# fgvieira/ngsF-HMM

Hardware: AMD Instinct MI355X
Metric: site-ind updates/sec (EM iterations x individuals x sites / s), 1M sites x 1k ind (higher is better)
Workload: dtype f64

## Files before the change

### include/nghmm_debug.h

```cpp
#ifndef NGHMM_DEBUG_H
#define NGHMM_DEBUG_H

#include "nghmm.h"

#ifdef __cplusplus
extern "C" {
#endif

int nghmm_set_switch(nghmm_t* h, const char* name, long value);

int nghmm_fast_layout(nghmm_t* h, uint32_t* waves_per_individual, uint64_t* sites_per_lane);

int nghmm_get_emissions(nghmm_t* h, double* e_prob);

int nghmm_kernel_ms(nghmm_t* h, int slot, double* ms, uint32_t* launches);

typedef struct {
  uint32_t mode;
  uint64_t ind_rounds;
} nghmm_mode_count;
int nghmm_debug_mode_counts(nghmm_t* h, nghmm_mode_count* out, uint32_t cap, uint32_t* n, int reset);
int nghmm_debug_estmaf_counts(nghmm_t* h, uint64_t out[5], int reset);

#ifdef __cplusplus
}
#endif
#endif
```

### ngsf-hmm_amd/csrc/capi_internal.hpp

```cpp
#pragma once
#include <hip/hip_runtime.h>

#include <atomic>
#include <cmath>
#include <cstdarg>
#include <cstdio>
#include <cstdlib>
#include <chrono>
#include <cstring>
#include <new>
#include <functional>
#include <condition_variable>
#include <map>
#include <mutex>
#include <string>
#include <thread>
#include <vector>

#include "../../include/nghmm.h"
#include "../../include/nghmm_debug.h"
#include "bfgs_batch.hpp"
#include "capi_owners.hpp"
#include "kernels.hpp"
#include "kernels_fast.hpp"
#include "kernels_summary.hpp"

using namespace nghmm;

namespace capi {

extern thread_local std::string g_last_error;

#define HIP_TRY(expr)                                                              \
  do {                                                                             \
    hipError_t e__ = (expr);                                                       \
    if (e__ != hipSuccess) {                                                       \
      set_error("%s failed: %s (%s:%d)", #expr, hipGetErrorString(e__), __FILE__,  \
                __LINE__);                                                         \
      return NGHMM_ERR_HIP;                                                        \
    }                                                                              \
  } while (0)

enum Slot { SLOT_EMISSION = 0, SLOT_FORWARD = 1, SLOT_BACKWARD = 2, SLOT_LKL = 3, SLOT_ESTMAF = 4,
            SLOT_VITERBI = 5, SLOT_LKL_FIRST = 6, SLOT_BFGS = 7, NSLOTS = 8 };

}

using namespace capi;

struct ChainCtx;
struct nghmm_handle {
  ~nghmm_handle();
  uint64_t I = 0, S = 0;
  int device = 0, mode = NGHMM_MODE_EXACT;
  Stream stream;
  Event ev0, ev1, ev_sync;
  Stream aux_stream;
  Stream g_xstream;
  Event aux_ev0, aux_ev1, aux_go, aux_done;
  static constexpr uint32_t kAuxPieces = 16;
  Event aux_piece_ev[kAuxPieces];
  Event aux_estep_ev[3];
  DevBuf<double> d_aux_params;
  PinBuf<int> h_flags_pin;
  PinBuf<double> h_lkl_pin;
  hipEvent_t param_snapshot_ev = nullptr;
  bool blocking_sync = false;
  bool loaded = false;
  bool warmed = false;

  DevBuf<double> d_gl, d_pos;
  DevBuf<double> d_freq, d_eprob, d_fw, d_marg, d_indF, d_alpha, d_ind_lkl;
  DevBuf<int> d_flags;

  DevScratch<uint32_t> d_pt_ind;
  DevScratch<double> d_pt_F, d_pt_A, d_pt_lkl;

  DevBuf<uint8_t> d_bp, d_path_sites, d_path;
  DevBuf<double> d_vit;
  DevBuf<double> d_tmp;
  DevScratch<double> d_geno;
  DevScratch<char> d_text;
  bool tmp_is_posteriors = false;
  bool path_decoded = false;
  DevScratch<uint8_t> d_tseg, d_trec;
  DevScratch<uint8_t> d_samp;
  DevScratch<uint8_t> d_info;
  DevScratch<uint8_t> d_summ;
  DevBuf<double> d_freq_new, d_hap;

  uint64_t I_tot = 0, ind_begin = 0, site_begin = 0, S_own = 0;
  DevBuf<double> d_gl_shard;

  bool packed = false;
  DevBuf<uint32_t> d_codes;
  DevBuf<uint32_t> d_codes_shard;
  DevBuf<double> d_cls_log;
  double h_cls_proto[12] = {0};
  DevBuf<unsigned long long> d_uniform;
  uint64_t lkl_redone = 0;
  struct LklAsync {
    Event ev0, ev1, ev_done;
    DevScratch<double> d_lkl;
    PinScratch<double> h_lkl;
    DevBuf<int> d_flags;
    PinBuf<int> h_flags;
    std::vector<uint32_t> ind;
    std::vector<double> F, A;
    uint64_t lo = 0, hi = 0;
    bool pending = false;
  } lane[2];
  struct BgSpan {
    Event ev0, ev1;
    int slot = 0;
  };
  DevBuf<int> d_flags_bg;
  bool flags_bg_clear = false;
  std::vector<BgSpan> bg_spans;
  size_t bg_used = 0;
  nghmm_handle* parent = nullptr;
  std::atomic<int> n_replicas{0};
  int g_n = 0, g_rank = 0;
  DevBuf<double> g_send, g_recv, g_freq_own, g_freq_all;
  struct ChainCtx* chain = nullptr;
  DevBuf<double> c_send, c_recv;
  bool loading = false;
  std::map<uint64_t, uint64_t> load_cover;
  DevScratch<double> d_stage;
  DevScratch<int8_t> d_stage8;

  FastState fast;
  BfgsBatch batch;
  bool marg_valid = false;

  std::vector<double> h_indF, h_alpha;
  double ms[NSLOTS] = {0, 0, 0, 0, 0, 0, 0, 0};
  uint32_t launches[NSLOTS] = {0, 0, 0, 0, 0, 0, 0, 0};
};

namespace capi {

hipError_t sync_stream(nghmm_t* h);
int use_device(nghmm_t* h);
void tic(nghmm_t* h);
int toc(nghmm_t* h, int slot, bool accumulate);
int clear_flags(nghmm_t* h);
int check_flags(nghmm_t* h, const int* d_flags = nullptr);
int ensure_points(nghmm_t* h, size_t n);
GlView own_gl(const nghmm_t* h);
int ensure_tmp(nghmm_t* h);
int ensure_marg(nghmm_t* h);
int viterbi_scratch(nghmm_t* h, uint64_t* chunk, double** state = nullptr);
int fast_estep_impl(nghmm_t* h, double* ind_lkl, bool have_walk);
int redo_nonfinite(nghmm_t* h, uint32_t n_pts, const uint32_t* ind, const double* F,
                   const double* alpha, double* lkl);
int lkl_batch_impl(nghmm_t* h, uint32_t n_pts, const uint32_t* ind, const double* F,
                   const double* alpha, double* lkl, bool accumulate, bool* emit_estep = nullptr);
int lane_setup(nghmm_t* h, int k, size_t n);
int lkl_submit(nghmm_t* h, int k);
int lkl_wait(nghmm_t* h, int k);
int emission_impl(nghmm_t* h);
int bg_begin(nghmm_t* h);
int bg_open(nghmm_t* h, int slot, hipStream_t st = nullptr);
int bg_close(nghmm_t* h, hipStream_t st = nullptr);
int bg_finish(nghmm_t* h);
int ensure_emissions(nghmm_t* h);

int estmaf_and_refresh(nghmm_t* h, bool shard, const double* d_marg_blocks, uint64_t S_own,
                       uint64_t I_tot, uint64_t I_blk, double* d_freq_out);
void chain_release(nghmm_t* h);
int tracts_to_host(nghmm_t* h, int source, double threshold, uint64_t min_sites,
                   std::vector<nghmm_tract>& out);
int tracts_check_args(nghmm_t* h, int source, double threshold, const char* who);
int summary_check_source(nghmm_t* h, int what, double threshold, const char* who);
int summary_check_regions(uint64_t S, uint64_t I, uint64_t n_regions, const uint64_t* begin,
                          const uint64_t* end, const void* regions, const void* sites,
                          const char* who);
struct SummaryRegion {
  uint64_t begin, end;
  bool first;
};
int summary_to_host(nghmm_t* h, int what, double thr, const std::vector<SummaryRegion>& regs,
                    const uint8_t* prev_state, nghmm_region_stat* regions, nghmm_site_stat* sites);
int summary_last_state(nghmm_t* h, uint8_t* out);

}
```

### ngsf-hmm_amd/csrc/capi_multi.hip

```cpp
#include "capi_internal.hpp"


int nghmm_shard_config(nghmm_t* h, uint64_t n_ind_total, uint64_t ind_begin, uint64_t site_begin,
                       uint64_t n_sites_own) {
  g_last_error.clear();
  if (h && h->fast.shard.world > 1) {
    set_error("nghmm_shard_config: the handle is a site shard (one layout at a time)");
    return NGHMM_ERR_ARG;
  }
  if (!h || n_ind_total < h->I || ind_begin + h->I > n_ind_total ||
      site_begin + n_sites_own > h->S || n_ind_total % h->I != 0) {
    set_error("nghmm_shard_config: inconsistent shard (equal individuals per rank required)");
    return NGHMM_ERR_ARG;
  }
  h->I_tot = n_ind_total;
  h->ind_begin = ind_begin;
  h->site_begin = site_begin;
  h->S_own = n_sites_own;
  return NGHMM_OK;
}

uint64_t nghmm_site_shard_bytes(nghmm_t* h) {
  return h ? (uint64_t)(h->I * 30 + 64) * sizeof(double) : 0;
}
// ... 95 lines not shown
  if ((rc = use_device(h))) return rc;
  const size_t n = (size_t)h->S_own * h->I_tot * 3;
  if ((rc = h->d_gl_shard.alloc(n))) return rc;
  HIP_TRY(hipMemcpyAsync(h->d_gl_shard, gl_site_shard, n * sizeof(double), hipMemcpyHostToDevice,
                         h->stream));
  if (h->mode == NGHMM_MODE_FAST) fast_exp(h->stream, h->d_gl_shard, h->d_gl_shard, n);
  HIP_TRY(sync_stream(h));
  return NGHMM_OK;
}

int nghmm_get_geno_codes_dev(nghmm_t* h, uint64_t site_lo, uint64_t site_hi, uint8_t* d_out) {
  g_last_error.clear();
  if (!h || !h->packed || !h->loaded || !d_out || site_lo > site_hi || site_hi > h->S)
    return NGHMM_ERR_ARG;
  int rc;
  if ((rc = use_device(h))) return rc;
  launch_codes_to_bytes(h->stream, h->d_codes, site_lo * h->I, (site_hi - site_lo) * h->I, d_out);
  HIP_TRY(hipGetLastError());
  HIP_TRY(sync_stream(h));
  return NGHMM_OK;
}

int nghmm_load_geno_site_shard_dev(nghmm_t* h, const uint8_t* d_codes_bytes) {
  g_last_error.clear();
  if (!h || !h->packed || !d_codes_bytes) return NGHMM_ERR_ARG;
  int rc;
  if ((rc = use_device(h))) return rc;
  const size_t n = (size_t)h->S_own * h->I_tot;
  if ((rc = h->d_codes_shard.alloc(n / 16 + 2))) return rc;
  HIP_TRY(hipDeviceSynchronize());
  launch_bytes_to_codes(h->stream, d_codes_bytes, n, h->d_codes_shard);
  HIP_TRY(hipGetLastError());
  HIP_TRY(sync_stream(h));
  return NGHMM_OK;
}

int nghmm_load_gl_site_shard_dev(nghmm_t* h, const double* d_gl_site_shard) {
  g_last_error.clear();
  if (!h || !d_gl_site_shard) return NGHMM_ERR_ARG;
  if (h->packed) {
    set_error("packed handle: use nghmm_load_geno_site_shard_dev");
    return NGHMM_ERR_ARG;
  }
  int rc;
  if ((rc = use_device(h))) return rc;
  const size_t n = (size_t)h->S_own * h->I_tot * 3;
  if ((rc = h->d_gl_shard.alloc(n))) return rc;
  HIP_TRY(hipDeviceSynchronize());
  HIP_TRY(hipMemcpyAsync(h->d_gl_shard, d_gl_site_shard, n * sizeof(double),
                         hipMemcpyDeviceToDevice, h->stream));
  if (h->mode == NGHMM_MODE_FAST) fast_exp(h->stream, h->d_gl_shard, h->d_gl_shard, n);
  HIP_TRY(sync_stream(h));
  return NGHMM_OK;
}

int nghmm_pack_posteriors_dev(nghmm_t* h, uint64_t site_lo, uint64_t site_hi, double* d_out) {
  g_last_error.clear();
  if (!h || !d_out || site_lo > site_hi || site_hi > h->S) return NGHMM_ERR_ARG;
  int rc;
  if ((rc = use_device(h))) return rc;
  if (h->mode == NGHMM_MODE_FAST && site_lo == 0 && site_hi == h->S) {
    if (!fast_post_to_site_major(h->fast, h->stream, d_out)) return NGHMM_ERR_HIP;
    HIP_TRY(hipGetLastError());
    HIP_TRY(sync_stream(h));
    return NGHMM_OK;
  }
  if ((rc = ensure_marg(h))) return rc;
  launch_copy_f64(h->stream, h->d_marg + site_lo * h->I, d_out, (site_hi - site_lo) * h->I);
  HIP_TRY(hipGetLastError());
  HIP_TRY(sync_stream(h));
  return NGHMM_OK;
}

int nghmm_mstep_freq_sites_dev(nghmm_t* h, const double* d_marg_blocks, double* d_freq_out) {
  g_last_error.clear();
  if (!h || !d_marg_blocks || !d_freq_out || !(h->packed ? (void*)h->d_codes_shard.p : (void*)h->d_gl_shard.p))
    return NGHMM_ERR_ARG;
  int rc;
  if ((rc = use_device(h))) return rc;
  if (h->mode != NGHMM_MODE_FAST && h->I_tot != h->I) {
    set_error("exact-mode sharded est_maf is not available; use NGHMM_MODE_FAST");
    return NGHMM_ERR_ARG;
  }
  if ((rc = estmaf_and_refresh(h, true, d_marg_blocks, h->S_own, h->I_tot, h->I, d_freq_out)))
    return rc;
  HIP_TRY(sync_stream(h));
  return NGHMM_OK;
}

int nghmm_set_freq_dev(nghmm_t* h, const double* d_freq_all) {
  g_last_error.clear();
  if (!h || !d_freq_all) return NGHMM_ERR_ARG;
  int rc;
  if ((rc = use_device(h))) return rc;
  HIP_TRY(hipMemcpyAsync(h->d_freq, d_freq_all, h->S * sizeof(double), hipMemcpyDeviceToDevice,
                         h->stream));
  return emission_impl(h);
}



namespace {

struct GroupHook {
  nghmm_t** hs;
  int n, r;
  int rc;
};

void group_after_estep(void* user) {
  GroupHook* g = static_cast<GroupHook*>(user);
  nghmm_t* h = g->hs[g->r];
  g->rc = nghmm_pack_posteriors_dev(h, 0, h->S, h->g_send);
  if (g->rc != NGHMM_OK) return;
  const size_t blk = (size_t)h->S_own * h->I;
  for (int q = 0; q < g->n; ++q) {
    if (hipMemcpyAsync(g->hs[q]->g_recv + (size_t)g->r * blk, h->g_send + (size_t)q * blk,
                       blk * sizeof(double), hipMemcpyDeviceToDevice, h->g_xstream) != hipSuccess) {
      g->rc = NGHMM_ERR_HIP;
      return;
    }
  }
}

int for_each_rank(int n, const std::function<int(int)>& fn) {
  std::vector<int> rcs(n, NGHMM_OK);
  std::vector<std::string> msgs(n);
  if (n == 1) {
    rcs[0] = fn(0);
  } else {
    std::vector<std::thread> th;
    for (int r = 0; r < n; ++r)
      th.emplace_back([&, r] {
        rcs[r] = fn(r);
        if (rcs[r] != NGHMM_OK) msgs[r] = g_last_error;
      });
    for (auto& t : th) t.join();
  }
  for (int r = 0; r < n; ++r)
    if (rcs[r] != NGHMM_OK) {
      if (!msgs[r].empty()) g_last_error = msgs[r];
      return rcs[r];
    }
  return NGHMM_OK;
}

int group_freq_phases(nghmm_t** hs, int n) {
  const uint64_t S_own = hs[0]->S / n;
  int rc = for_each_rank(n, [&](int r) -> int {
    nghmm_t* h = hs[r];
    int rr = nghmm_mstep_freq_sites_dev(h, h->g_recv, h->g_freq_own);
    if (rr != NGHMM_OK) return rr;
    for (int q = 0; q < n; ++q)
      if (hipMemcpyAsync(hs[q]->g_freq_all + (size_t)r * S_own, h->g_freq_own, S_own * sizeof(double),
                         hipMemcpyDeviceToDevice, h->g_xstream) != hipSuccess)
        return NGHMM_ERR_HIP;
    return hipStreamSynchronize(h->g_xstream) == hipSuccess ? NGHMM_OK : NGHMM_ERR_HIP;
  });
  if (rc != NGHMM_OK) return rc;
  return for_each_rank(n, [&](int r) -> int { return nghmm_set_freq_dev(hs[r], hs[r]->g_freq_all); });
}

}

int nghmm_group_setup(nghmm_t** hs, int n) {
  g_last_error.clear();
  if (!hs || n < 1) return NGHMM_ERR_ARG;
  for (int r = 0; r < n; ++r)
    if (hs[r]) hs[r]->batch.set_max_threads(n > 1 ? 1 : 64);
  nghmm_t* h0 = hs[0];
  for (int r = 0; r < n; ++r) {
    nghmm_t* h = hs[r];
    if (!h || !h->loaded || (n > 1 && (h->parent || h->n_replicas.load() > 0)) ||
        h->fast.shard.world > 1 || h->I != h0->I ||
        h->S != h0->S || h->mode != h0->mode ||
        h->packed != h0->packed) {
      set_error("nghmm_group_setup: the handles must be loaded and agree in size, mode and packing");
      return NGHMM_ERR_ARG;
    }
// ... 476 lines not shown
```

### ngsf-hmm_amd/csrc/kernels_fast.hip

```cpp
#include <hip/hip_runtime.h>

#include "fast_dev.hpp"

namespace nghmm {

namespace {


__global__ void __launch_bounds__(256)
k_fast_geno_interleave(const uint32_t* __restrict__ codes, uint64_t cell0, uint64_t I, uint64_t S,
                       uint64_t T, uint32_t C, uint32_t* __restrict__ geno_il) {
  const uint64_t TB = T >> 4;
  const uint64_t n = I * C * TB * 64;
  for (uint64_t k = (uint64_t)blockIdx.x * blockDim.x + threadIdx.x; k < n;
       k += (uint64_t)gridDim.x * blockDim.x) {
    const uint64_t lane = k & 63, r = k >> 6;
    const uint64_t tb = r % TB, wv = r / TB;
    const uint64_t c = wv % C, i = wv / C;
    const uint64_t s0 = (c * 64 + lane) * T + tb * 16;
    uint32_t w = 0;
#pragma unroll
    for (int j = 0; j < 16; ++j) {
      const uint64_t s = s0 + j;
      if (s < S) w |= gl_code(codes, cell0 + s * I + i) << (2 * j);
// ... 90 lines not shown
      }
      tq[tx][ll] = q;
    }
  }
  __syncthreads();
  {
    const int tx = threadIdx.x & 63, ty = threadIdx.x >> 6;
    for (int ii = ty; ii < 32; ii += 4) {
      const uint64_t i = i0 + ii;
      if (i < I) glq_il[((i * C + c) * T + t) * 64 + tx] = tq[ii][tx];
    }
  }
}

__global__ void __launch_bounds__(256)
k_fast_gl_scale(const GlView gl_log, uint64_t I, uint64_t S, uint64_t T, uint32_t C,
                double* __restrict__ scale_c) {
  __shared__ double part[8][33];
  const uint64_t n_it = (I + 31) / 32;
  const uint64_t c = blockIdx.x / n_it;
  const uint64_t i0 = (blockIdx.x % n_it) * 32;
  const int tx = threadIdx.x & 31, ty = threadIdx.x >> 5;
  const uint64_t i = i0 + tx;
  double acc = 0;
  if (i < I) {
    for (uint64_t j = c * 64 + ty; j < c * 64 + 64; j += 8) {
      for (uint64_t t = 0; t < T; ++t) {
        const uint64_t s = j * T + t;
        if (s >= S) break;
        double g0, g1, g2;
        gl_fetch(gl_log, s * I + i, g0, g1, g2);
        acc += fmax(g0, fmax(g1, g2));
      }
    }
  }
  part[ty][tx] = acc;
  __syncthreads();
  if (ty == 0 && i < I) {
    double sum = 0;
    for (int k = 0; k < 8; ++k) sum += part[k][tx];
    scale_c[i * C + c] = sum;
  }
}

__global__ void __launch_bounds__(256)
k_fast_export_e(LklArrays arr, bool packed, const double* __restrict__ gl_lin, uint64_t I,
                uint64_t S, uint64_t T, uint32_t C, double* __restrict__ out) {
  const uint64_t n = I * S;
  for (uint64_t k = (uint64_t)blockIdx.x * blockDim.x + threadIdx.x; k < n;
       k += (uint64_t)gridDim.x * blockDim.x) {
    const uint64_t i = k / S, s = k % S;
    const uint64_t j = s / T, t = s % T;
    const uint64_t c = j >> 6, lane = j & 63;
    const uint64_t wv = i * C + c;
    const double maf = arr.freq_il[(c * T + t) * 64 + lane], om = 1 - maf;
    const double bb = om * maf;
    const double h00 = om * om, h02 = maf * maf;
    double e0, e1;
    if (packed) {
      const uint32_t w = arr.geno_il[(wv * (T >> 4) + (t >> 4)) * 64 + lane];
      const uint32_t code = (w >> ((uint32_t)(t & 15) * 2)) & 3u;
      const double u = arr.u_lin;
      const double u0 = fma(u, h00, fma(u, 2 * bb, u * h02));
      const double u1 = fma(u, h00 + bb, u * (h02 + bb));
      e0 = code == 0 ? h00 : code == 1 ? 2 * bb : code == 2 ? h02 : u0;
      e1 = code == 0 ? h00 + bb : code == 1 ? 0.0 : code == 2 ? h02 + bb : u1;
    } else {
      const double* g = gl_lin + (s * I + i) * 3;
      e0 = fma(g[0], h00, fma(g[1], 2 * bb, g[2] * h02));
      e1 = fma(g[0], h00 + bb, g[2] * (h02 + bb));
    }
    out[k * 2] = log(e0);
    out[k * 2 + 1] = log(e1);
  }
}

struct SwitchName {
  const char* name;
  int Switches::*field;
};
const SwitchName kSwitches[] = {
    {"bg_parts", &Switches::bg_parts}, {"estmaf_interp", &Switches::estmaf_interp},
    {"estmaf_no_rows", &Switches::estmaf_no_rows}, {"estmaf_no_called", &Switches::estmaf_no_called},
    {"fast_c", &Switches::fast_c}, {"exact_serial", &Switches::exact_serial},
    {"dbg_abort_round", &Switches::dbg_abort_round}, {"no_dev_bfgs", &Switches::no_dev_bfgs},
    {"no_bg_stream", &Switches::no_bg_stream}, {"spans", &Switches::spans},
    {"viterbi_chunk", &Switches::viterbi_chunk}};

}

Switches Switches::from_env() {
  Switches sw;
  for (const auto& k : kSwitches) {
    std::string env = "NGHMM_";
    for (const char* c = k.name; *c; ++c) env += (char)std::toupper((unsigned char)*c);
    if (const char* v = std::getenv(env.c_str())) {
      char* end = nullptr;
      const long n = std::strtol(v, &end, 10);
      sw.*(k.field) = (end != v) ? (int)n : 1;
    }
  }
  return sw;
}

bool Switches::set(const char* name, long value) {
  for (const auto& k : kSwitches)
    if (std::strcmp(k.name, name) == 0) {
      this->*(k.field) = (int)value;
      return true;
    }
  return false;
}

static bool fast_alloc_run_state(FastState& fs) {
  const size_t cells = (size_t)fs.I * fs.Spad;
  const size_t slack = 8 * 64;
  if (!dalloc(&fs.e_il, cells + slack)) return false;
  if (hipMemset(fs.e_il + cells, 0, slack * sizeof(double)) != hipSuccess) return false;
  if (!dalloc(&fs.base_c, (size_t)fs.I * fs.C)) return false;
  if (!dalloc(&fs.freq_il, (size_t)fs.Spad + slack)) return false;
  if (hipMemset(fs.freq_il + fs.Spad, 0, slack * sizeof(double)) != hipSuccess) return false;
  const size_t post_cells = (size_t)fs.C * fs.T * post_tile_doubles(fs.I);
  if (!dalloc(&fs.post, post_cells)) return false;
  if (hipMemset(fs.post, 0, post_cells * sizeof(double)) != hipSuccess) return false;
  if (!dalloc(&fs.ckpt, cells / CK * 4 + 4 * 64)) return false;
  if (!dalloc(&fs.lane_ops, (size_t)fs.I * fs.J * 5)) return false;
  if (!dalloc(&fs.bound, (size_t)fs.I * fs.J * 4)) return false;
  fs.e_stale = true;
  return true;
}

bool fast_create(FastState& fs, uint64_t I, uint64_t S, bool packed) {
  fs.I = I;
  fs.S = S;
  fs.packed = packed;
  fs.owns_data = true;
  uint64_t C = (49152 + I - 1) / I;
  if (fs.sw.fast_c >= 1) C = (uint64_t)fs.sw.fast_c;
  if (C > 256) C = 256;
  while (C > 1 && (S + 64 * C - 1) / (64 * C) < (C > 64 ? 32u : 16u)) --C;
  if (C < 1) C = 1;
  if (fs.sw.fast_c < 1) {
    const uint64_t c64 = S / (64 * 64);
    if (c64 >= 1 && c64 < C && I * c64 >= 24576) C = c64;
  }
  if (fs.sw.fast_c < 1) {
    const uint64_t q = packed ? 16 : 8;
    auto padded = [&](uint64_t c) { return 64 * c * ((((S + 64 * c - 1) / (64 * c)) + q - 1) / q * q); };
    uint64_t best = C;
    for (uint64_t c = C; c >= 1 && 4 * c >= 3 * C; --c)
      if (padded(c) < padded(best)) best = c;
    C = best;
  }
  fs.C = (uint32_t)C;
  fs.J = 64 * C;
  fs.T = (S + fs.J - 1) / fs.J;
  fs.T = (fs.T + 7) & ~7ull;
  if (packed) fs.T = (fs.T + 15) & ~15ull;
  fs.Spad = fs.J * fs.T;
  const size_t cells = (size_t)I * fs.Spad;
  const size_t slack = 8 * 64;
  if (!dalloc(&fs.pos_il, (size_t)fs.Spad + slack)) return false;
  if (hipMemset(fs.pos_il + fs.Spad, 0, slack * sizeof(double)) != hipSuccess) return false;
  if (!dalloc(&fs.chunk_scale, (size_t)2 * fs.J)) return false;
  if (!dalloc(&fs.gl_scale_c, (size_t)I * C)) return false;
  if (packed) {
    const size_t words = cells / 16 + slack;
    if (!dalloc(&fs.geno_il, words)) return false;
    if (hipMemset(fs.geno_il, 0, words * sizeof(uint32_t)) != hipSuccess) return false;
    if (!dalloc(&fs.cls_lin, (size_t)12)) return false;
  } else {
    if (!dalloc(&fs.glq_il, (cells + slack) * 2)) return false;
    if (hipMemset(fs.glq_il + cells * 2, 0, slack * 2 * sizeof(double)) != hipSuccess) return false;
    if (!dalloc(&fs.gl_lin, (size_t)I * S * 3)) return false;
  }
  return fast_alloc_run_state(fs);
}

bool fast_create_replica(FastState& fs, const FastState& parent) {
  fs = FastState();
  fs.sw = parent.sw;
  fs.I = parent.I;
  fs.S = parent.S;
  fs.T = parent.T;
  fs.C = parent.C;
  fs.J = parent.J;
  fs.Spad = parent.Spad;
  fs.packed = parent.packed;
  fs.owns_data = false;
  fs.gl_log = parent.gl_log;
  fs.d_pos = parent.d_pos;
  fs.geno_il = parent.geno_il;
  fs.cls_lin = parent.cls_lin;
  fs.u_lin = parent.u_lin;
  fs.called_table = parent.called_table;
  fs.gl_lin = parent.gl_lin;
  fs.pos_il = parent.pos_il;
  fs.chunk_scale = parent.chunk_scale;
  fs.glq_il = parent.glq_il;
  fs.gl_scale_c = parent.gl_scale_c;
  fs.dmax_finite = parent.dmax_finite;
  fs.alpha_small_min = parent.alpha_small_min;
  return fast_alloc_run_state(fs);
}

void fast_destroy(FastState& fs) {
  dbfgs_destroy(fs);
  void* run[] = {fs.e_il, fs.base_c, fs.freq_il, fs.post, fs.ckpt, fs.lane_ops, fs.bound, fs.lanes[0].part,
                 fs.lanes[0].grp_dev, fs.lanes[1].part, fs.lanes[1].grp_dev, fs.redo, fs.est_status,
                 fs.est_state, fs.est_counts, fs.shard.edges};
  for (void* p : run)
    if (p) (void)hipFree(p);
  if (fs.owns_data) {
    void* data[] = {fs.pos_il, fs.chunk_scale, fs.glq_il, fs.gl_scale_c, fs.gl_lin, fs.geno_il, fs.cls_lin};
    for (void* p : data)
      if (p) (void)hipFree(p);
  }
  fs = FastState();
}

void fast_exp(hipStream_t st, const double* d_in, double* d_out, uint64_t n) {
  if (n) hipLaunchKernelGGL(k_fast_exp, dim3(16384), dim3(256), 0, st, d_in, d_out, n);
}

GlView fast_gl_lin(const FastState& fs) {
  return fs.packed ? gl_packed(fs.gl_log.codes, fs.cls_lin, fs.gl_log.cell0) : gl_dense(fs.gl_lin);
}

bool fast_load(FastState& fs, hipStream_t st, const GlView& gl_log, const double* d_pos) {
  dbfgs_invalidate(fs);
  fs.gl_log = gl_log;
  fs.d_pos = d_pos;
  fs.e_stale = true;
  if (fs.packed) {
    if (gl_log.dense) return false;
    fast_exp(st, gl_log.table, fs.cls_lin, 12);
    double t[12];
    if (hipMemcpyAsync(t, fs.cls_lin, sizeof t, hipMemcpyDeviceToHost, st) != hipSuccess) return false;
    if (hipStreamSynchronize(st) != hipSuccess) return false;
    fs.u_lin = t[9];
    fs.called_table = t[0] == 1 && t[1] == 0 && t[2] == 0 && t[3] == 0 && t[4] == 1 && t[5] == 0 &&
                      t[6] == 0 && t[7] == 0 && t[8] == 1 && t[9] > 0 && t[10] == t[9] && t[11] == t[9];
    hipLaunchKernelGGL(k_fast_geno_interleave, dim3(8192), dim3(256), 0, st, gl_log.codes,
                       gl_log.cell0, fs.I, fs.S, fs.T, fs.C, fs.geno_il);
  } else {
    if (!gl_log.dense) return false;
    const double* lg = gl_log.dense + gl_log.cell0 * 3;
    fast_exp(st, lg, fs.gl_lin, fs.I * fs.S * 3);
    const uint64_t n_it = (fs.I + 31) / 32;
    hipLaunchKernelGGL(k_fast_gl_interleave, dim3((unsigned)((uint64_t)fs.C * fs.T * n_it)),
                       dim3(256), 0, st, lg, fs.I, fs.S, fs.T, fs.C,
                       reinterpret_cast<double2*>(fs.glq_il));
  }
  hipLaunchKernelGGL(k_fast_gl_scale, dim3((unsigned)((uint64_t)fs.C * ((fs.I + 31) / 32))), dim3(256),
                     0, st, gl_log, fs.I, fs.S, fs.T, fs.C, fs.gl_scale_c);
  hipLaunchKernelGGL(k_fast_pos_interleave, dim3(1024), dim3(256), 0, st, d_pos, fs.S, fs.T, fs.C,
                     fs.pos_il);
  hipLaunchKernelGGL(k_fast_chunk_scale, dim3(fs.C), dim3(64), 0, st, fs.pos_il, fs.T,
                     reinterpret_cast<double2*>(fs.chunk_scale));
  unsigned long long* d_m = reinterpret_cast<unsigned long long*>(fs.bound);
  if (hipMemsetAsync(d_m, 0, sizeof(unsigned long long), st) != hipSuccess) return false;
  hipLaunchKernelGGL(k_fast_max_finite, dim3(256), dim3(256), 0, st, d_pos, fs.S, d_m);
  unsigned long long bits = 0;
  if (hipMemcpyAsync(&bits, d_m, sizeof bits, hipMemcpyDeviceToHost, st) != hipSuccess) return false;
  if (hipStreamSynchronize(st) != hipSuccess) return false;
  std::memcpy(&fs.dmax_finite, &bits, sizeof bits);
  {
    std::vector<double> cs((size_t)2 * fs.J);
    if (hipMemcpy(cs.data(), fs.chunk_scale, cs.size() * sizeof(double), hipMemcpyDeviceToHost) != hipSuccess)
      return false;
    double sum = 0, starts = 0;
    for (size_t k = 0; k < fs.J; ++k) {
      sum += cs[2 * k];
      starts += cs[2 * k + 1];
    }
    const double n_finite = (double)fs.S - starts;
    fs.alpha_small_min = (n_finite > 0 && sum > 0) ? 1e-6 / (sum / n_finite) : HUGE_VAL;
  }
  return hipGetLastError() == hipSuccess;
}

bool fast_refresh_freq_table(FastState& fs, hipStream_t st, const double* d_freq, int* d_flags) {
  hipLaunchKernelGGL(k_fast_freq_interleave, dim3(1024), dim3(256), 0, st, d_freq, fs.S, fs.T, fs.C,
                     fs.freq_il, d_flags);
  fs.e_stale = true;
  return hipGetLastError() == hipSuccess;
}


bool fast_viterbi(FastState& fs, hipStream_t st, const double* d_freq, const double* d_indF,
                  const double* d_alpha, uint8_t* d_bp, uint8_t* d_path_sites, int* d_flags,
                  double* d_scratch, uint64_t chunk_sites) {
  double* eprob_log = nullptr;
  if (!dalloc(&eprob_log, (size_t)fs.I * fs.S * 2)) return false;
  launch_emission_exact(st, fs.gl_log, d_freq, eprob_log, fs.S, fs.I, d_flags);
  launch_viterbi_exact(st, eprob_log, fs.d_pos, fs.S, fs.I, d_indF, d_alpha, d_bp, d_path_sites,
                       d_scratch, chunk_sites, fs.sw.exact_serial != 0);
  const bool ok = hipGetLastError() == hipSuccess && hipStreamSynchronize(st) == hipSuccess;
  (void)hipFree(eprob_log);
  return ok;
}

bool fast_viterbi_forward(FastState& fs, hipStream_t st, const double* d_freq, const double* d_indF,
                          const double* d_alpha, uint8_t* d_bp, int* d_flags, double* d_scratch,
                          uint64_t chunk_sites, bool chain_start) {
  double* eprob_log = nullptr;
  if (!dalloc(&eprob_log, (size_t)fs.I * fs.S * 2)) return false;
  launch_emission_exact(st, fs.gl_log, d_freq, eprob_log, fs.S, fs.I, d_flags);
  launch_viterbi_fwd_exact(st, eprob_log, fs.d_pos, fs.S, fs.I, d_indF, d_alpha, d_bp, d_scratch,
                           chunk_sites, chain_start, fs.sw.exact_serial != 0);
  const bool ok = hipGetLastError() == hipSuccess && hipStreamSynchronize(st) == hipSuccess;
  (void)hipFree(eprob_log);
  return ok;
// ... 10 lines not shown
```

### ngsf-hmm_amd/csrc/kernels_fast.hpp

```cpp
#pragma once

#include <hip/hip_runtime.h>

#include <cstdint>
#include <map>
#include <vector>

#include "glview.hpp"

namespace nghmm {

struct Switches {
  int bg_parts = 2;
  int estmaf_interp = 1;
  int estmaf_no_rows = 0;
  int estmaf_no_called = 0;
  int fast_c = 0;
  int exact_serial = 0;
  int dbg_abort_round = 0;
  int no_dev_bfgs = 0;
  int no_bg_stream = 0;
  int viterbi_chunk = 0;
  int spans = 0;
  static Switches from_env();
  bool set(const char* name, long value);
};

struct SiteShard {
  uint32_t rank = 0, world = 1;
  double* send = nullptr;
  double* recv = nullptr;
  uint64_t cap = 0;
  int (*allgather)(void* user, uint64_t n_bytes) = nullptr;
  void* user = nullptr;
  double* edges = nullptr;
  bool edges_from_round = false;
  uint64_t n_gathers = 0;
};

struct FastState {
  Switches sw;
  SiteShard shard;
  uint64_t I = 0, S = 0;
  uint64_t T = 0;
  uint32_t C = 0;
  uint64_t J = 0;
  uint64_t Spad = 0;
  GlView gl_log;
  const double* d_pos = nullptr;
  bool packed = false;
  bool owns_data = true;
  uint32_t* geno_il = nullptr;
  double* cls_lin = nullptr;
  double u_lin = 0;
  bool called_table = false;
  double* gl_lin = nullptr;
  double* e_il = nullptr;
  double* base_c = nullptr;
  double* pos_il = nullptr;
  double* chunk_scale = nullptr;
  double* glq_il = nullptr;
  double* gl_scale_c = nullptr;
  double* freq_il = nullptr;
  bool e_stale = true;
  double* post = nullptr;
  double* ckpt = nullptr;
  double* lane_ops = nullptr;
  double* bound = nullptr;
  struct ModeRange { uint32_t mode, begin, count; };
  struct LklLane {
    double* part = nullptr;
    size_t part_cap = 0;
    void* grp_dev = nullptr;
    size_t grp_cap = 0;
    std::vector<unsigned char> grp_host;
    uint32_t n_groups = 0;
    uint32_t n_pts = 0;
    std::vector<ModeRange> mode_ranges;
  };
  LklLane lanes[2];
  int cur_lane = 0;

  struct DevBfgs {
    static constexpr uint32_t kRing = 4;
    static constexpr uint32_t kTableWords = 4 + 2 * 129 + 12;
    uint64_t cap_I = 0;
    void* prob = nullptr;
    void* solver = nullptr;
    double* arrays = nullptr;
    void* groups = nullptr;
    uint32_t* last_mode = nullptr;
    uint32_t* worklists = nullptr;
    uint32_t* all = nullptr;
    uint32_t* counts = nullptr;
    double* lkl = nullptr;
    double* part = nullptr;
    double *d_F = nullptr, *d_A = nullptr;
    double *snap_F = nullptr, *snap_A = nullptr;
    uint32_t snap_set = 0;
    volatile uint32_t* h_table = nullptr;
    double *h_F = nullptr, *h_A = nullptr;
    unsigned long long stats_host[6] = {0, 0, 0, 0, 0, 0};
    uint32_t seq_base = 0;
    uint32_t mstep_no = 0;
    bool clean = true;
    bool preplanned = false;
    bool pre_F_fixed = false, pre_alpha_fixed = false;
    double* h_epi_lkl = nullptr;
    volatile uint32_t* h_epi = nullptr;
    uint32_t epi_seq = 0;
  } dev;

  double dmax_finite = 0;
  double alpha_small_min = 0;
  uint8_t* redo = nullptr;
  size_t redo_cap = 0;
  uint8_t* est_status = nullptr;
  double* est_state = nullptr;
  std::map<uint32_t, uint64_t> mode_ind_rounds;
  uint32_t* est_counts = nullptr;
};

enum EstCount {
  EST_CNT_CHECK_FAILED = 0,
  EST_CNT_RESUMED = 1,
  EST_CNT_RESUMED_AGAIN = 2,
  EST_CNT_LOGSPACE = 3,
  EST_CNT_EXACT_TAIL = 4,
  EST_COUNTS = 5
};

bool fast_create(FastState& fs, uint64_t I, uint64_t S, bool packed = false);
bool fast_create_replica(FastState& fs, const FastState& parent);
void fast_destroy(FastState& fs);
bool fast_load(FastState& fs, hipStream_t st, const GlView& gl_log, const double* d_pos);
bool fast_refresh_freq_table(FastState& fs, hipStream_t st, const double* d_freq, int* d_flags);
bool fast_refresh_emissions(FastState& fs, hipStream_t st, const double* d_freq, int* d_flags);
bool fast_lkl_prepare(FastState& fs, hipStream_t st, uint32_t n_pts, const uint32_t* h_ind,
                      const double* h_F, const double* h_A, bool force_general = false);
bool fast_lkl_launch(FastState& fs, hipStream_t st, double* d_lkl, int* d_flags,
                     bool emit_estep = false);
bool fast_lkl_covers_everyone(const FastState& fs);
bool dbfgs_available(const FastState& fs);
bool dbfgs_reserve(FastState& fs);
void dbfgs_destroy(FastState& fs);
void dbfgs_invalidate(FastState& fs);
constexpr uint32_t kEpiFlags = 8;
bool dbfgs_epilogue(FastState& fs, hipStream_t st, int* d_flags, uint32_t n_flags, const double* d_lkl);
bool dbfgs_wait_epilogue(FastState& fs, hipStream_t st, int* flags_out, uint32_t n_flags, bool yield);
bool dbfgs_begin(FastState& fs, hipStream_t st, double* d_indF, double* d_alpha, bool F_fixed,
                 bool alpha_fixed);
const double* dbfgs_start_F(const FastState& fs);
const double* dbfgs_start_A(const FastState& fs);
bool dbfgs_advance(FastState& fs, hipStream_t st, uint32_t round, uint32_t n_in);
bool dbfgs_wait_plan(FastState& fs, hipStream_t st, uint32_t round, uint32_t* n_active,
                     std::vector<FastState::ModeRange>* ranges, bool yield = false);
bool dbfgs_launch_round(FastState& fs, hipStream_t st, uint32_t round, uint32_t n_active,
                        const std::vector<FastState::ModeRange>& ranges, bool emit_estep);
void dbfgs_end(FastState& fs, uint32_t last_round);
bool dbfgs_preplan(FastState& fs, hipStream_t st, bool F_fixed, bool alpha_fixed);
bool fast_lkl_launch_planned(FastState& fs, hipStream_t st, const void* d_groups_by_ind,
                             const std::vector<FastState::ModeRange>& ranges, uint32_t n_active,
                             const uint32_t* d_worklists, const uint32_t* d_all, double* part,
                             double* d_lkl, bool emit_estep);
bool fast_estep(FastState& fs, hipStream_t st, const double* d_indF, const double* d_alpha,
                double* d_ind_lkl, int* d_flags, bool have_forward_walk);
bool fast_forward_ops(FastState& fs, hipStream_t st, const double* d_indF, const double* d_alpha);
bool fast_post_to_site_major(FastState& fs, hipStream_t st, double* d_marg);
void fast_exp(hipStream_t st, const double* d_in, double* d_out, uint64_t n);
GlView fast_gl_lin(const FastState& fs);
bool fast_estmaf_splittable(const FastState& fs, uint64_t I_tot, bool tile_major);
bool fast_estmaf_in_place(const FastState& fs, uint64_t I_tot);
bool fast_estmaf_reserve(FastState& fs, uint64_t S_own);
bool fast_estmaf_called(const FastState& fs, const GlView& gl);
bool fast_estmaf(FastState& fs, hipStream_t st, const GlView& d_gl_lin_sites,
                 const double* d_marg_blocks, uint64_t S_own, uint64_t I_tot, uint64_t I_blk,
                 double* d_freq_out, bool tile_major = false, uint32_t part = 0,
                 uint32_t n_parts = 1);
bool fast_viterbi(FastState& fs, hipStream_t st, const double* d_freq, const double* d_indF,
                  const double* d_alpha, uint8_t* d_bp, uint8_t* d_path_sites, int* d_flags,
                  double* d_scratch, uint64_t chunk_sites);
bool fast_viterbi_forward(FastState& fs, hipStream_t st, const double* d_freq, const double* d_indF,
                          const double* d_alpha, uint8_t* d_bp, int* d_flags, double* d_scratch,
                          uint64_t chunk_sites, bool chain_start);
bool fast_export_emissions(FastState& fs, hipStream_t st, double* d_out);

}
```

### ngsf-hmm_amd/csrc/kernels_fast_estmaf.hip

```cpp
#include "fast_dev.hpp"

#include <mutex>

namespace capi {
void set_error(const char* fmt, ...);
}

namespace nghmm {

namespace {



__device__ double2 estmaf_term_logspace(const double* g, double freq, double F) {
  double h[3];
  h[0] = (1 - freq) * (1 - freq) + (1 - freq) * freq * F;
  h[1] = 2 * (1 - freq) * freq - 2 * (1 - freq) * freq * F;
  h[2] = freq * freq + (1 - freq) * freq * F;
  double pp[3];
  for (int k = 0; k < 3; ++k) {
    double l = log(h[k]);
    if (l == -__builtin_huge_val()) l = -kINF;
    h[k] = l;
  }
  if (F == 1) h[1] = -kINF;
  double M = g[0] + h[0];
  for (int k = 0; k < 3; ++k) {
    pp[k] = g[k] + h[k];
    M = (pp[k] >= M) ? pp[k] : M;
  }
  double sum = 0;
  for (int k = 0; k < 3; ++k) sum += exp(pp[k] - M);
  const double norm = log(sum) + M;
  for (int k = 0; k < 3; ++k) pp[k] = exp(pp[k] - norm);
  return double2{pp[1] + pp[2] * (2 - F), 2 * pp[1] + (pp[0] + pp[2]) * (2 - F)};
}

template <int CTRL>
__device__ __forceinline__ double dpp_move(double v) {
  const uint64_t b = ngh_bits(v);
  const int lo = __builtin_amdgcn_mov_dpp((int)(uint32_t)b, CTRL, 0xf, 0xf, true);
  const int hi = __builtin_amdgcn_mov_dpp((int)(uint32_t)(b >> 32), CTRL, 0xf, 0xf, true);
  return ngh_from_bits(((uint64_t)(uint32_t)hi << 32) | (uint32_t)lo);
}

__device__ __forceinline__ double lane_value(double v, int lane) {
  const uint64_t b = ngh_bits(v);
  const uint32_t lo = __builtin_amdgcn_readlane((int)(uint32_t)b, lane);
  const uint32_t hi = __builtin_amdgcn_readlane((int)(uint32_t)(b >> 32), lane);
  return ngh_from_bits(((uint64_t)hi << 32) | lo);
}

__device__ __forceinline__ double wave_sum_lastrow(double v) {
  v += dpp_move<0xB1>(v);
  v += dpp_move<0x4E>(v);
  v += dpp_move<0x141>(v);
  v += dpp_move<0x140>(v);
  {
    const uint64_t b = ngh_bits(v);
    const int lo = __builtin_amdgcn_update_dpp(0, (int)(uint32_t)b, 0x142, 0xa, 0xf, false);
    const int hi = __builtin_amdgcn_update_dpp(0, (int)(uint32_t)(b >> 32), 0x142, 0xa, 0xf, false);
    v += ngh_from_bits(((uint64_t)(uint32_t)hi << 32) | (uint32_t)lo);
  }
  {
    const uint64_t b = ngh_bits(v);
    const int lo = __builtin_amdgcn_update_dpp(0, (int)(uint32_t)b, 0x143, 0xc, 0xf, false);
    const int hi = __builtin_amdgcn_update_dpp(0, (int)(uint32_t)(b >> 32), 0x143, 0xc, 0xf, false);
    v += ngh_from_bits(((uint64_t)(uint32_t)hi << 32) | (uint32_t)lo);
  }
  return v;
}

__device__ __forceinline__ double wave_sum_uniform(double v) {
  v += dpp_move<0xB1>(v);
  v += dpp_move<0x4E>(v);
  v += dpp_move<0x141>(v);
  v += dpp_move<0x140>(v);
  return ((lane_value(v, 0) + lane_value(v, 16)) + lane_value(v, 32)) + lane_value(v, 48);
}

__device__ __forceinline__ double wave_sum_pair(double pn, double pd) {
  const uint64_t bn = ngh_bits(pn), bd = ngh_bits(pd);
  const auto lo = __builtin_amdgcn_permlane32_swap((unsigned)bn, (unsigned)bd, false, false);
  const auto hi = __builtin_amdgcn_permlane32_swap((unsigned)(bn >> 32), (unsigned)(bd >> 32),
                                                   false, false);
  double v = ngh_from_bits(((uint64_t)hi[0] << 32) | lo[0]) +
             ngh_from_bits(((uint64_t)hi[1] << 32) | lo[1]);
  v += dpp_move<0xB1>(v);
  v += dpp_move<0x4E>(v);
  v += dpp_move<0x141>(v);
  v += dpp_move<0x140>(v);
  {
    const uint64_t b = ngh_bits(v);
    const int l = __builtin_amdgcn_update_dpp(0, (int)(uint32_t)b, 0x142, 0xa, 0xf, false);
    const int h = __builtin_amdgcn_update_dpp(0, (int)(uint32_t)(b >> 32), 0x142, 0xa, 0xf, false);
    v += ngh_from_bits(((uint64_t)(uint32_t)h << 32) | (uint32_t)l);
  }
  return v;
}

constexpr int EN = 12;
constexpr int EST_SCALARS = 8;
constexpr int EST_FIELDS = EST_SCALARS + 2 * EN;
enum : uint8_t { EST_DONE = 0, EST_INTERP = 1, EST_EXACT = 2 };
constexpr int EST_K0 = 2;
constexpr int EST_MIN_GAIN = 24;
constexpr double EST_DMAX = 0.85;
constexpr double EST_BACK = 0.1;
constexpr double EST_MULT = 32.0;
constexpr double EST_FIT = 0.72;
constexpr int EST_KMAX = 32;
constexpr double EST_TOL = 1e-11;
constexpr double EST_GUARD = 1e-9;
__constant__ double kChebC[EN] = {0.9914448613738104, 0.9238795325112867, 0.7933533402912352, 0.6087614290087207, 0.38268343236508984, 0.1305261922200517, -0.1305261922200516, -0.3826834323650895, -0.6087614290087207, -0.793353340291235, -0.9238795325112867, -0.9914448613738104};
__constant__ double kChebW[EN] = {0.13052619222005157, -0.3826834323650898, 0.6087614290087207, -0.7933533402912352, 0.9238795325112867, -0.9914448613738104, 0.9914448613738104, -0.9238795325112868, 0.7933533402912352, -0.6087614290087209, 0.3826834323650899, -0.130526192220052};

constexpr int ESTMAF_MAXW = 16;

__device__ __forceinline__ bool in_tile_rows(uint64_t site, uint64_t tile_T, uint64_t row0,
                                             uint64_t row1) {
  if (tile_T == 0) return true;
  const uint64_t j = site / tile_T, t = site - j * tile_T;
  const uint64_t row = (j >> 6) * tile_T + t;
  return row >= row0 && row < row1;
}
__host__ __device__ constexpr int estmaf_full_slots(int NI, int BLOCK) {
  return BLOCK == 64 ? (NI == 16 ? 12 : NI == 12 ? 8 : NI == 8 ? 4 : NI == 4 ? 2 : NI == 2 ? 1 : 0)
                     : (NI == 16 ? 8 : 0);
}

template <int NI, int BLOCK, bool TILE>
__device__ __forceinline__ void estmaf_site(
    const GlView& gl, const double* __restrict__ marg_blocks, uint64_t S_own, uint64_t I_tot,
    uint64_t I_blk, double* __restrict__ freq_out, uint8_t* __restrict__ redo,
    uint8_t* __restrict__ status, double* __restrict__ state, uint64_t state_stride, int fresh,
    int n_exact, int allow_build, uint64_t site, const double* __restrict__ tile_col,
    uint32_t* __restrict__ cnt, double (&xch)[2][ESTMAF_MAXW][2],
    double2 (&nodebuf)[(BLOCK == 64 && NI >= 8) ? EN : 1][(BLOCK == 64 && NI >= 8) ? 65 : 1],
    double2 (&xnode)[(BLOCK == 64 && NI >= 8) ? 1 : EN][(BLOCK == 64 && NI >= 8) ? 1 : BLOCK / 64],
    double2* park = nullptr) {
  constexpr int W = BLOCK / 64;
  constexpr bool PARK = (W == 1 && NI >= 8);
  const int lane = threadIdx.x & 63;
  const int wv = threadIdx.x >> 6;
  const uint32_t tix = threadIdx.x;
  constexpr uint64_t stride = BLOCK;
  const uint64_t cell_s = site * I_tot;

  double tF_lane_out;
  double sA[NI], sb[NI], sC[NI], u0[NI], nC[NI], fc[NI];
  {
    constexpr int NB = NI < 8 ? NI : (NI % 8 ? NI / 2 : 8);
    static_assert(NI % NB == 0, "whole batches");
    const bool one_block = (I_blk == I_tot);
    const uint32_t ib = (uint32_t)I_blk;
    double tF_acc = 0;
#pragma unroll
    for (int k0 = 0; k0 < NI; k0 += NB) {
      double r0[NB], r1[NB], r2[NB], rF[NB];
      uint64_t ic[NB];
#pragma unroll
      for (int j = 0; j < NB; ++j) {
        const uint64_t i = (uint64_t)tix + stride * (k0 + j);
        ic[j] = (k0 + j < estmaf_full_slots(NI, BLOCK) || i < I_tot) ? i : I_tot - 1;
        gl_fetch(gl, cell_s + ic[j], r0[j], r1[j], r2[j]);
      }
      if constexpr (TILE) {
#pragma unroll
        for (int j = 0; j < NB; ++j)
          rF[j] = tile_col[k0 + j < estmaf_full_slots(NI, BLOCK)
                               ? post_ind_off(tix) + (uint64_t)(k0 + j) * post_ind_off(stride)
                               : post_ind_off(ic[j])];
      } else if (one_block) {
#pragma unroll
        for (int j = 0; j < NB; ++j) rF[j] = marg_blocks[site * I_blk + ic[j]];
      } else {
#pragma unroll
        for (int j = 0; j < NB; ++j) {
          const uint32_t q = (uint32_t)ic[j] / ib;
          rF[j] = marg_blocks[((uint64_t)q * S_own + site) * I_blk + ((uint32_t)ic[j] - q * ib)];
        }
      }
#pragma unroll
      for (int j = 0; j < NB; ++j) {
        const int k = k0 + j;
        const bool valid = k < estmaf_full_slots(NI, BLOCK) || (uint64_t)tix + stride * k < I_tot;
        const double p0 = valid ? r0[j] : 1.0, p1 = valid ? r1[j] : 0.0;
        const double p2 = valid ? r2[j] : 0.0, F = valid ? rF[j] : 0.0;
        const double cc = p1 * fma(-2.0, F, 2.0);
        const double n2 = (2 - F) * p2;
        sA[k] = p0;
        sb[k] = fma(F, p0 + p2, cc);
        sC[k] = p2;
        u0[k] = fma(n2, F, cc);
        nC[k] = n2;
        fc[k] = F * cc;
        tF_acc += valid ? 2 - F : 0.0;
      }
      __builtin_amdgcn_sched_barrier(0);
    }
    tF_lane_out = tF_acc;
  }
  double tF_sum = wave_sum_uniform(tF_lane_out);
  if constexpr (W > 1) {
    if (lane == 0) xch[1][wv][0] = tF_sum;
    __syncthreads();
    tF_sum = xch[1][0][0];
#pragma unroll
    for (int w = 1; w < W; ++w) tF_sum += xch[1][w][0];
    __syncthreads();
  }

  int iters = 0;
  int buf = 0;
  double num = 0, den = 0;
  double pnum = 0.01, pden = 1.0;
  if (!fresh) {
    num = state[0 * state_stride + site];
    den = state[1 * state_stride + site];
    pnum = state[2 * state_stride + site];
    pden = state[3 * state_stride + site];
    iters = (int)state[4 * state_stride + site];
  }
  bool built = !allow_build;
  int n_before = n_exact;
  bool check = false, interp_ok = false;
  double mid = 0, half = 0, my_gn = 0, my_gd = 0, rprev = 0;
  auto lane_sums = [&](double r, double& pn, double& pd) {
    pn = 0;
    pd = 0;
    if constexpr (NI >= 4) {
#pragma unroll
      for (int k0 = 0; k0 + 4 <= NI; k0 += 4) {
        double sm[4];
#pragma unroll
        for (int j = 0; j < 4; ++j) sm[j] = fma(r, fma(r, sC[k0 + j], sb[k0 + j]), sA[k0 + j]);
        const double p01 = sm[0] * sm[1], p23 = sm[2] * sm[3];
        const double R = rcp_nr(p01 * p23);
        const double r01 = R * p23, r23 = R * p01;
        const double inv0 = r01 * sm[1], inv1 = r01 * sm[0];
        const double inv2 = r23 * sm[3], inv3 = r23 * sm[2];
        pn = fma(fma(nC[k0], r, u0[k0]), inv0, pn);
        pd = fma(fc[k0], inv0, pd);
        pn = fma(fma(nC[k0 + 1], r, u0[k0 + 1]), inv1, pn);
        pd = fma(fc[k0 + 1], inv1, pd);
        pn = fma(fma(nC[k0 + 2], r, u0[k0 + 2]), inv2, pn);
        pd = fma(fc[k0 + 2], inv2, pd);
        pn = fma(fma(nC[k0 + 3], r, u0[k0 + 3]), inv3, pn);
        pd = fma(fc[k0 + 3], inv3, pd);
      }
      if constexpr (NI % 4 == 2) {
        constexpr int k0 = NI - 2;
        const double s0 = fma(r, fma(r, sC[k0], sb[k0]), sA[k0]);
        const double s1 = fma(r, fma(r, sC[k0 + 1], sb[k0 + 1]), sA[k0 + 1]);
        const double R = rcp_nr(s0 * s1);
        const double inv0 = R * s1, inv1 = R * s0;
        pn = fma(fma(nC[k0], r, u0[k0]), inv0, pn);
        pd = fma(fc[k0], inv0, pd);
        pn = fma(fma(nC[k0 + 1], r, u0[k0 + 1]), inv1, pn);
        pd = fma(fc[k0 + 1], inv1, pd);
      }
    } else {
#pragma unroll
      for (int k = 0; k < NI; ++k) {
        const double inv = rcp_nr(fma(r, fma(r, sC[k], sb[k]), sA[k]));
        pn = fma(fma(nC[k], r, u0[k]), inv, pn);
        pd = fma(fc[k], inv, pd);
      }
    }
  };
  for (;;) {
    const double r = pnum * rcp_nr2(pden - pnum);
    double pn, pd;
    lane_sums(r, pn, pd);
    const double v = wave_sum_pair(pn, pd);
    double sn = lane_value(v, 31), sd = lane_value(v, 63);
    if constexpr (W > 1) {
      if (lane == 0) {
        xch[buf][wv][0] = sn;
        xch[buf][wv][1] = sd;
      }
      __syncthreads();
      sn = xch[buf][0][0];
      sd = xch[buf][0][1];
#pragma unroll
      for (int w = 1; w < W; ++w) {
        sn += xch[buf][w][0];
        sd += xch[buf][w][1];
      }
      buf ^= 1;
    }
    if (check) {
      const int nj = lane < EN ? lane : 0;
      const double t = (r - mid) / (r + mid) - half * kChebC[nj];
      const double q = (lane < EN) ? kChebW[nj] / t : 0.0;
      const double Sq = wave_sum_uniform(q);
      const double bn = wave_sum_uniform(q * my_gn) / Sq, bd = wave_sum_uniform(q * my_gd) / Sq;
      interp_ok = fabs(bn - sn) <= EST_TOL * fabs(sn) && fabs(bd - sd) <= EST_TOL * fabs(sd);
      check = false;
      if (!interp_ok && tix == 0) atomicAdd(cnt + EST_CNT_CHECK_FAILED, 1u);
    }
    num = fma(r, sn, num);
    den = fma(r, sd, den + tF_sum);
    const double lhs = fabs(fma(pnum, den, -(num * pden))), thr = kEPS * (den * pden);
    const bool again = (lhs > thr) && (iters++ < 100);
    rprev = r;
    pnum = num;
    pden = den;
    if (!again) break;
    if (interp_ok) {
      if (wv == 0) {
        if (lane < EN) {
          state[(EST_SCALARS + lane) * state_stride + site] = my_gn;
          state[(EST_SCALARS + EN + lane) * state_stride + site] = my_gd;
        }
        if (lane == 0) {
          state[0 * state_stride + site] = num;
          state[1 * state_stride + site] = den;
          state[2 * state_stride + site] = pnum;
          state[3 * state_stride + site] = pden;
          state[4 * state_stride + site] = (double)iters;
          state[5 * state_stride + site] = mid;
          state[6 * state_stride + site] = half;
          state[7 * state_stride + site] = tF_sum;
          status[site] = EST_INTERP;
        }
      }
      return;
    }
    if (!built && --n_before <= 0) {
      const double m_est = (double)iters * (sqrt(lhs / thr) - 1.0);
      const double rn = pnum * rcp_nr2(pden - pnum);
      const double step = fabs(rn - rprev);
      const double reach = (rn >= rprev) ? EST_DMAX * rn : EST_DMAX / (1 + EST_DMAX) * rn;
      const bool fits = (double)iters * step <= EST_FIT * reach;
      if (!fits && iters < EST_KMAX && m_est >= EST_MIN_GAIN) {
        n_before = 1;
      } else {
        built = true;
      }
      if (built && m_est >= EST_MIN_GAIN && 100 - iters >= EST_MIN_GAIN) {
        const double g = fmin(EST_DMAX, fmax(EST_MULT * step / rn, 1e-3));
        double lo, hi;
        if (rn >= rprev) {
          lo = rn * (1 - EST_BACK * g);
          hi = rn * (1 + g);
        } else {
          lo = rn / (1 + g);
          hi = rn * (1 + EST_BACK * g);
        }
        mid = sqrt(lo * hi);
        half = (hi - mid) / (hi + mid);
        if (half > 0 && lo > 0 && hi < 1e300) {
          if constexpr (PARK) {
            const double tnl = half * kChebC[lane < EN ? lane : 0];
            const double r_nodes = mid * (1 + tnl) * rcp_nr2(1 - tnl);
#pragma unroll 1
            for (int nd = 0; nd < EN; ++nd) {
              double pn, pd;
              lane_sums(lane_value(r_nodes, nd), pn, pd);
              nodebuf[nd][lane] = double2{pn, pd};
            }
            __syncthreads();
            const int j = lane & 15, q4 = lane >> 4;
            double an = 0, ad = 0;
            if (j < EN) {
#pragma unroll
              for (int l = 0; l < 16; ++l) {
                const double2 t2 = nodebuf[j][q4 * 16 + l];
                an += t2.x;
                ad += t2.y;
              }
            }
            an += __shfl_xor(an, 16);
            ad += __shfl_xor(ad, 16);
            an += __shfl_xor(an, 32);
            ad += __shfl_xor(ad, 32);
            my_gn = an;
            my_gd = ad;
            check = true;
          } else {
            const double tnl = half * kChebC[lane < EN ? lane : 0];
            const double r_nodes = mid * (1 + tnl) * rcp_nr2(1 - tnl);
            double an = 0, ad = 0;
            if constexpr (W > 1) {
#pragma unroll 1
              for (int nd = 0; nd < EN; ++nd) {
                double pn, pd;
                lane_sums(lane_value(r_nodes, nd), pn, pd);
                park[nd * BLOCK + (int)tix] = double2{pn, pd};
              }
              __syncthreads();
              for (int nd = wv; nd < EN; nd += W) {
                double sn = 0, sd = 0;
#pragma unroll
                for (int w = 0; w < W; ++w) {
                  const double2 t2 = park[nd * BLOCK + w * 64 + lane];
                  sn += t2.x;
                  sd += t2.y;
                }
                const double v = wave_sum_pair(sn, sd);
                const double tn = lane_value(v, 31), td = lane_value(v, 63);
                if (lane == 0) xnode[nd][0] = double2{tn, td};
              }
              __syncthreads();
              if (lane < EN) {
                an = xnode[lane][0].x;
                ad = xnode[lane][0].y;
              }
              __syncthreads();
            } else {
#pragma unroll 1
              for (int nd = 0; nd < EN; ++nd) {
                double pn, pd;
                lane_sums(lane_value(r_nodes, nd), pn, pd);
                const double v = wave_sum_pair(pn, pd);
                const double sn = lane_value(v, 31), sd = lane_value(v, 63);
                if (lane == nd) {
                  an = sn;
                  ad = sd;
                }
              }
            }
            my_gn = an;
            my_gd = ad;
            check = true;
          }
        }
      }
    }
  }
  if (tix == 0) {
    const double freq = num / den;
    const bool ok = freq >= 0 && freq < 1;
    freq_out[site] = freq;
    redo[site] = ok ? 0 : 1;
    status[site] = EST_DONE;
  }
}

__device__ __forceinline__ const double* estmaf_tile_col(const double* marg_blocks, uint64_t site,
                                                         uint64_t tile_T, uint64_t I_tot) {
  const uint64_t j = site / tile_T, t = site - j * tile_T;
  return marg_blocks + post_lane_off((j >> 6) * tile_T + t, j & 63, I_tot);
}

#define ESTMAF_SHARED(NI, BLOCK)                                                              \
  constexpr bool PARK_ = ((BLOCK) == 64 && (NI) >= 8);                                         \
  __shared__ double xch[2][ESTMAF_MAXW][2];                       \
  __shared__ double2 nodebuf[PARK_ ? EN : 1][PARK_ ? 65 : 1];                                  \
  __shared__ double2 xnode[PARK_ ? 1 : EN][PARK_ ? 1 : (BLOCK) / 64]

template <int NI, int BLOCK, bool TILE>
__global__ void __launch_bounds__(BLOCK) __attribute__((amdgpu_waves_per_eu(2)))
k_fast_estmaf(const GlView gl, const double* __restrict__ marg_blocks,
              uint64_t S_own, uint64_t I_tot, uint64_t I_blk, uint64_t tile_T,
              double* __restrict__ freq_out, uint8_t* __restrict__ redo,
              uint8_t* __restrict__ status, double* __restrict__ state, uint64_t state_stride,
              int n_exact, int allow_build, uint64_t blk0, uint32_t* __restrict__ cnt) {
  ESTMAF_SHARED(NI, BLOCK);
  uint64_t site;
  const double* tile_col = nullptr;
  if constexpr (TILE) {
    const uint64_t b = blockIdx.x + blk0, x = b & 7, k = b >> 3;
    const uint64_t q = ((k >> 3) << 6) + (x << 3) + (k & 7);
    const uint64_t tile_row = q >> 6, l = q & 63;
    const uint64_t c = tile_row / tile_T, t = tile_row - c * tile_T;
    site = (c * 64 + l) * tile_T + t;
    if (site >= S_own) return;
    tile_col = marg_blocks + post_lane_off(tile_row, l, I_tot);
  } else {
    site = blockIdx.x;
  }
  extern __shared__ double2 park_mem[];
  estmaf_site<NI, BLOCK, TILE>(gl, marg_blocks, S_own, I_tot, I_blk, freq_out, redo, status, state,
                               state_stride, 1, n_exact, allow_build, site, tile_col, cnt, xch, nodebuf,
                               xnode, park_mem);
}

template <int NI, int BLOCK, bool TILE>
__global__ void __launch_bounds__(BLOCK) __attribute__((amdgpu_waves_per_eu(2)))
k_fast_estmaf_resume(const GlView gl, const double* __restrict__ marg_blocks,
                     uint64_t S_own, uint64_t I_tot, uint64_t I_blk, uint64_t tile_T,
                     double* __restrict__ freq_out, uint8_t* __restrict__ redo,
                     uint8_t* __restrict__ status, double* __restrict__ state,
                     uint64_t state_stride, int n_exact, int allow_build, uint64_t row0,
                     uint64_t row1, uint32_t* __restrict__ cnt, int cnt_slot) {
  ESTMAF_SHARED(NI, BLOCK);
  extern __shared__ double2 park_mem[];
  const int lane = threadIdx.x & 63;
  for (uint64_t base = (uint64_t)blockIdx.x * 64; base < S_own; base += (uint64_t)gridDim.x * 64) {
    const uint64_t s = base + lane;
    const bool need = s < S_own && in_tile_rows(s, TILE ? tile_T : 0, row0, row1) &&
                      status[s] == EST_EXACT;
    uint64_t mask = __ballot(need);
    if (mask && threadIdx.x == 0) atomicAdd(cnt + cnt_slot, (uint32_t)__popcll(mask));
    if constexpr (BLOCK > 64) __syncthreads();
    while (mask) {
      const uint64_t site = base + (uint64_t)__builtin_ctzll(mask);
      mask &= mask - 1;
      const double* tile_col = TILE ? estmaf_tile_col(marg_blocks, site, tile_T, I_tot) : nullptr;
      estmaf_site<NI, BLOCK, TILE>(gl, marg_blocks, S_own, I_tot, I_blk, freq_out, redo, status,
                                   state, state_stride, 0, n_exact, allow_build, site, tile_col, cnt,
                                   xch, nodebuf, xnode, park_mem);
      if constexpr (BLOCK > 64) __syncthreads();
    }
  }
}

__device__ __forceinline__ double row_sum(double v) {
  v = __dadd_rn(v, dpp_move<0xB1>(v));
  v = __dadd_rn(v, dpp_move<0x4E>(v));
  v = __dadd_rn(v, dpp_move<0x141>(v));
  v = __dadd_rn(v, dpp_move<0x140>(v));
  return v;
}

template <int NI, bool TILE>
__device__ __forceinline__ void estmaf_rows_sites(
    const GlView& gl, const double* __restrict__ marg_blocks, uint64_t S_own, uint64_t I_tot,
    uint64_t I_blk, double* __restrict__ freq_out, uint8_t* __restrict__ redo,
    uint8_t* __restrict__ status, double* __restrict__ state, uint64_t state_stride, int fresh,
    int n_exact, int allow_build, uint64_t site, const double* __restrict__ tile_col, bool done,
    uint32_t* __restrict__ cnt) {
  static_assert(EN <= 16, "a row's lanes hold the interval's node sums");
  const int lane = threadIdx.x, j = lane & 15;
  const uint64_t cell_s = site * I_tot;

  double sA[NI], sb[NI], sC[NI], u0[NI], nC[NI], fc[NI];
  double tF_acc = 0;
  {
    const bool one_block = (I_blk == I_tot);
    const uint32_t ib = (uint32_t)I_blk;
    double r0[NI], r1[NI], r2[NI], rF[NI];
    uint64_t ic[NI];
#pragma unroll
    for (int k = 0; k < NI; ++k) {
      const uint64_t i = (uint64_t)j + 16 * k;
      ic[k] = i < I_tot ? i : I_tot - 1;
      gl_fetch(gl, cell_s + ic[k], r0[k], r1[k], r2[k]);
    }
#pragma unroll
    for (int k = 0; k < NI; ++k) {
      if constexpr (TILE) {
        rF[k] = tile_col[post_ind_off(ic[k])];
      } else if (one_block) {
        rF[k] = marg_blocks[site * I_blk + ic[k]];
      } else {
        const uint32_t q = (uint32_t)ic[k] / ib;
        rF[k] = marg_blocks[((uint64_t)q * S_own + site) * I_blk + ((uint32_t)ic[k] - q * ib)];
      }
    }
#pragma unroll
    for (int k = 0; k < NI; ++k) {
      const bool valid = (uint64_t)j + 16 * k < I_tot;
      const double p0 = valid ? r0[k] : 1.0, p1 = valid ? r1[k] : 0.0;
      const double p2 = valid ? r2[k] : 0.0, F = valid ? rF[k] : 0.0;
      const double cc = p1 * fma(-2.0, F, 2.0);
      const double n2 = (2 - F) * p2;
      sA[k] = p0;
      sb[k] = fma(F, p0 + p2, cc);
      sC[k] = p2;
      u0[k] = fma(n2, F, cc);
      nC[k] = n2;
      fc[k] = F * cc;
      tF_acc += valid ? 2 - F : 0.0;
    }
  }
  const double tF_sum = row_sum(tF_acc);

  int iters = 0;
  double num = 0, den = 0;
  double pnum = 0.01, pden = 1.0;
  if (!fresh && !done) {
    num = state[0 * state_stride + site];
    den = state[1 * state_stride + site];
    pnum = state[2 * state_stride + site];
    pden = state[3 * state_stride + site];
    iters = (int)state[4 * state_stride + site];
  }
  bool built = !allow_build;
  int n_before = n_exact;
  bool check = false;
  double mid = 1, half = 0.5, my_gn = 0, my_gd = 0, rprev = 0;
  auto lane_sums = [&](double r, double& pn, double& pd) {
    pn = 0;
    pd = 0;
    if constexpr (NI >= 4) {
#pragma unroll
      for (int k0 = 0; k0 < NI; k0 += 4) {
        double sm[4];
#pragma unroll
        for (int k = 0; k < 4; ++k) sm[k] = fma(r, fma(r, sC[k0 + k], sb[k0 + k]), sA[k0 + k]);
        const double p01 = sm[0] * sm[1], p23 = sm[2] * sm[3];
        const double R = rcp_nr(p01 * p23);
        const double r01 = R * p23, r23 = R * p01;
        const double inv0 = r01 * sm[1], inv1 = r01 * sm[0];
        const double inv2 = r23 * sm[3], inv3 = r23 * sm[2];
        pn = fma(fma(nC[k0], r, u0[k0]), inv0, pn);
        pd = fma(fc[k0], inv0, pd);
        pn = fma(fma(nC[k0 + 1], r, u0[k0 + 1]), inv1, pn);
        pd = fma(fc[k0 + 1], inv1, pd);
        pn = fma(fma(nC[k0 + 2], r, u0[k0 + 2]), inv2, pn);
        pd = fma(fc[k0 + 2], inv2, pd);
        pn = fma(fma(nC[k0 + 3], r, u0[k0 + 3]), inv3, pn);
        pd = fma(fc[k0 + 3], inv3, pd);
      }
    } else {
#pragma unroll
      for (int k = 0; k < NI; ++k) {
        const double inv = rcp_nr(fma(r, fma(r, sC[k], sb[k]), sA[k]));
        pn = fma(fma(nC[k], r, u0[k]), inv, pn);
        pd = fma(fc[k], inv, pd);
      }
    }
  };
  for (;;) {
    const double r = pnum * rcp_nr2(pden - pnum);
    double pn, pd;
    lane_sums(r, pn, pd);
    const double sn = row_sum(pn), sd = row_sum(pd);
    bool interp_ok = false;
    if (__builtin_amdgcn_ballot_w64(check && !done) != 0) {
      const int nj = j < EN ? j : 0;
      const double t = (r - mid) / (r + mid) - half * kChebC[nj];
      const double q = (j < EN) ? kChebW[nj] / t : 0.0;
      const double Sq = row_sum(q);
      const double bn = row_sum(q * my_gn) / Sq, bd = row_sum(q * my_gd) / Sq;
      if (check && !done) {
        interp_ok = fabs(bn - sn) <= EST_TOL * fabs(sn) && fabs(bd - sd) <= EST_TOL * fabs(sd);
        if (!interp_ok && j == 0) atomicAdd(cnt + EST_CNT_CHECK_FAILED, 1u);
      }
      check = false;
    }
    bool want_build = false;
    if (!done) {
      num = fma(r, sn, num);
      den = fma(r, sd, den + tF_sum);
      const double lhs = fabs(fma(pnum, den, -(num * pden))), thr = kEPS * (den * pden);
      const bool again = (lhs > thr) && (iters++ < 100);
      rprev = r;
      pnum = num;
      pden = den;
      if (!again) {
        if (j == 0) {
          const double freq = num / den;
          const bool ok = freq >= 0 && freq < 1;
          freq_out[site] = freq;
          redo[site] = ok ? 0 : 1;
          status[site] = EST_DONE;
        }
        done = true;
      } else if (interp_ok) {
        if (j < EN) {
          state[(EST_SCALARS + j) * state_stride + site] = my_gn;
          state[(EST_SCALARS + EN + j) * state_stride + site] = my_gd;
        }
        if (j == 0) {
          state[0 * state_stride + site] = num;
          state[1 * state_stride + site] = den;
          state[2 * state_stride + site] = pnum;
          state[3 * state_stride + site] = pden;
          state[4 * state_stride + site] = (double)iters;
          state[5 * state_stride + site] = mid;
          state[6 * state_stride + site] = half;
          state[7 * state_stride + site] = tF_sum;
          status[site] = EST_INTERP;
        }
        done = true;
      } else if (!built && --n_before <= 0) {
        const double m_est = (double)iters * (sqrt(lhs / thr) - 1.0);
        const double rn = pnum * rcp_nr2(pden - pnum);
        const double step = fabs(rn - rprev);
        const double reach = (rn >= rprev) ? EST_DMAX * rn : EST_DMAX / (1 + EST_DMAX) * rn;
        const bool fits = (double)iters * step <= EST_FIT * reach;
        if (!fits && iters < EST_KMAX && m_est >= EST_MIN_GAIN) {
          n_before = 1;
        } else {
          built = true;
        }
        if (built && m_est >= EST_MIN_GAIN && 100 - iters >= EST_MIN_GAIN) {
          const double g = fmin(EST_DMAX, fmax(EST_MULT * step / rn, 1e-3));
          double lo, hi;
          if (rn >= rprev) {
            lo = rn * (1 - EST_BACK * g);
            hi = rn * (1 + g);
          } else {
            lo = rn / (1 + g);
            hi = rn * (1 + EST_BACK * g);
          }
          const double a = sqrt(lo * hi), h = (hi - a) / (hi + a);
          if (h > 0 && lo > 0 && hi < 1e300) {
            mid = a;
            half = h;
            want_build = true;
          }
        }
      }
    }
    if (__builtin_amdgcn_ballot_w64(want_build) != 0) {
#pragma unroll 1
      for (int nd = 0; nd < EN; ++nd) {
        const double tn = half * kChebC[nd];
        double qn, qd;
        lane_sums(mid * (1 + tn) * rcp_nr2(1 - tn), qn, qd);
        const double gn = row_sum(qn), gd = row_sum(qd);
        if (want_build && j == nd) {
          my_gn = gn;
          my_gd = gd;
        }
      }
      if (want_build) check = true;
    }
    if (__builtin_amdgcn_ballot_w64(!done) == 0) break;
  }
}

template <int NI, bool TILE>
__global__ void __launch_bounds__(64)
k_fast_estmaf_rows(const GlView gl, const double* __restrict__ marg_blocks, uint64_t S_own,
                   uint64_t I_tot, uint64_t I_blk, uint64_t tile_T, double* __restrict__ freq_out,
                   uint8_t* __restrict__ redo, uint8_t* __restrict__ status,
                   double* __restrict__ state, uint64_t state_stride, int n_exact,
                   int allow_build, uint32_t* __restrict__ cnt) {
  const int lane = threadIdx.x, row = lane >> 4;
  uint64_t site;
  const double* tile_col = nullptr;
  if constexpr (TILE) {
    const uint64_t b = blockIdx.x, x = b & 7, k = b >> 3;
    const uint64_t q = ((k >> 1) << 6) + (x << 3) + ((k & 1) << 2) + row;
    const uint64_t tile_row = q >> 6, l = q & 63;
    const uint64_t c = tile_row / tile_T, t = tile_row - c * tile_T;
    site = (c * 64 + l) * tile_T + t;
    tile_col = marg_blocks + post_lane_off(tile_row, l, I_tot);
  } else {
    site = (uint64_t)blockIdx.x * 4 + row;
  }
  bool done = site >= S_own;
  if (done) {
    site = 0;
    if constexpr (TILE) tile_col = marg_blocks;
  }
  if (__builtin_amdgcn_ballot_w64(!done) == 0) return;
  estmaf_rows_sites<NI, TILE>(gl, marg_blocks, S_own, I_tot, I_blk, freq_out, redo, status, state,
                              state_stride, 1, n_exact, allow_build, site, tile_col, done, cnt);
}

template <int NI, bool TILE>
__global__ void __launch_bounds__(64)
k_fast_estmaf_rows_resume(const GlView gl, const double* __restrict__ marg_blocks, uint64_t S_own,
                          uint64_t I_tot, uint64_t I_blk, uint64_t tile_T,
                          double* __restrict__ freq_out, uint8_t* __restrict__ redo,
                          uint8_t* __restrict__ status, double* __restrict__ state,
                          uint64_t state_stride, int n_exact, int allow_build,
                          uint32_t* __restrict__ cnt, int cnt_slot) {
  const int lane = threadIdx.x, row = lane >> 4;
  for (uint64_t base = (uint64_t)blockIdx.x * 64; base < S_own; base += (uint64_t)gridDim.x * 64) {
    const uint64_t s = base + lane;
    uint64_t mask = __ballot(s < S_own && status[s] == EST_EXACT);
    if (mask && lane == 0) atomicAdd(cnt + cnt_slot, (uint32_t)__popcll(mask));
    while (mask) {
      uint64_t site = 0;
      bool done = true;
#pragma unroll
      for (int r = 0; r < 4; ++r) {
        if (mask) {
          const uint64_t cand = base + (uint64_t)__builtin_ctzll(mask);
          mask &= mask - 1;
          if (r == row) {
            site = cand;
            done = false;
          }
        }
      }
      const double* tile_col =
          TILE ? (done ? marg_blocks : estmaf_tile_col(marg_blocks, site, tile_T, I_tot)) : nullptr;
      estmaf_rows_sites<NI, TILE>(gl, marg_blocks, S_own, I_tot, I_blk, freq_out, redo, status,
                                  state, state_stride, 0, n_exact, allow_build, site, tile_col, done,
                                  cnt);
    }
  }
}

__global__ void __launch_bounds__(256)
k_fast_estmaf_interp(uint64_t S_own, double* __restrict__ freq_out, uint8_t* __restrict__ redo,
                     uint8_t* __restrict__ status, double* __restrict__ state,
                     uint64_t state_stride, uint64_t tile_T, uint64_t row0, uint64_t row1) {
  const uint64_t site = (uint64_t)blockIdx.x * blockDim.x + threadIdx.x;
  if (site >= S_own || !in_tile_rows(site, tile_T, row0, row1) || status[site] != EST_INTERP)
    return;
  double num = state[0 * state_stride + site], den = state[1 * state_stride + site];
  double pnum = state[2 * state_stride + site], pden = state[3 * state_stride + site];
  int iters = (int)state[4 * state_stride + site];
  const double mid = state[5 * state_stride + site], half = state[6 * state_stride + site];
  const double tF_sum = state[7 * state_stride + site];
  double gn[EN], gd[EN];
#pragma unroll
  for (int j = 0; j < EN; ++j) {
    gn[j] = state[(EST_SCALARS + j) * state_stride + site];
    gd[j] = state[(EST_SCALARS + EN + j) * state_stride + site];
  }
  double cn[EN], cd[EN];
#pragma unroll
  for (int k = 0; k < EN; ++k) cn[k] = cd[k] = 0;
#pragma unroll
  for (int j = 0; j < EN; ++j) {
    const double x = kChebC[j], fn = gn[j] * (2.0 / EN), fd = gd[j] * (2.0 / EN);
    double t0 = 1.0, t1 = x;
    cn[0] += fn;
    cd[0] += fd;
#pragma unroll
    for (int k = 1; k < EN; ++k) {
      cn[k] = fma(fn, t1, cn[k]);
      cd[k] = fma(fd, t1, cd[k]);
      const double t2 = fma(2 * x, t1, -t0);
      t0 = t1;
      t1 = t2;
    }
  }
  const double inv_half = 1.0 / half;
  uint8_t st = EST_EXACT;
  for (;;) {
    const double r = pnum * rcp_nr2(pden - pnum);
    const double tt = (r - mid) * rcp_nr2(r + mid);
    if (!(fabs(tt) <= half)) break;
    const double x2 = 2 * (tt * inv_half);
    double bn1 = 0, bn2 = 0, bd1 = 0, bd2 = 0;
#pragma unroll
    for (int k = EN - 1; k >= 1; --k) {
      const double bn0 = fma(x2, bn1, cn[k] - bn2), bd0 = fma(x2, bd1, cd[k] - bd2);
      bn2 = bn1;
      bn1 = bn0;
      bd2 = bd1;
      bd1 = bd0;
    }
    const double sn = fma(0.5 * x2, bn1, 0.5 * cn[0] - bn2);
    const double sd = fma(0.5 * x2, bd1, 0.5 * cd[0] - bd2);
    const double num2 = fma(r, sn, num), den2 = fma(r, sd, den + tF_sum);
    const double lhs = fabs(fma(pnum, den2, -(num2 * pden))), thr = kEPS * (den2 * pden);
    if (!(fabs(lhs - thr) >= EST_GUARD * thr)) break;
    num = num2;
    den = den2;
    const bool again = (lhs > thr) && (iters++ < 100);
    pnum = num;
    pden = den;
    if (!again) {
      st = EST_DONE;
      break;
    }
  }
  if (st == EST_DONE) {
    const double freq = num / den;
    const bool ok = freq >= 0 && freq < 1;
    freq_out[site] = freq;
    redo[site] = ok ? 0 : 1;
  } else {
    state[0 * state_stride + site] = num;
    state[1 * state_stride + site] = den;
    state[2 * state_stride + site] = pnum;
    state[3 * state_stride + site] = pden;
    state[4 * state_stride + site] = (double)iters;
  }
  status[site] = st;
}

constexpr int ESTC_A0 = 0, ESTC_B0 = 1, ESTC_M0 = 2, ESTC_M1 = 3, ESTC_M2 = 4;

template <bool TILE>
__global__ void __launch_bounds__(64)
k_fast_estmaf_called_sums(const GlView gl, const double* __restrict__ marg_blocks, uint64_t S_own,
                          uint64_t I_tot, uint64_t I_blk, uint64_t tile_T,
                          uint8_t* __restrict__ redo, double* __restrict__ state,
                          uint64_t state_stride, uint64_t blk0) {
  const int lane = threadIdx.x;
  uint64_t site;
  const double* tile_col = nullptr;
  if constexpr (TILE) {
    const uint64_t b = blockIdx.x + blk0, x = b & 7, k = b >> 3;
    const uint64_t q = ((k >> 3) << 6) + (x << 3) + (k & 7);
    const uint64_t tile_row = q >> 6, l = q & 63;
    const uint64_t c = tile_row / tile_T, t = tile_row - c * tile_T;
    site = (c * 64 + l) * tile_T + t;
    if (site >= S_own) return;
    tile_col = marg_blocks + post_lane_off(tile_row, l, I_tot);
  } else {
    site = blockIdx.x;
  }
  const uint64_t cell_s = gl.cell0 + site * I_tot;
  const bool one_block = (I_blk == I_tot);
  double n1 = 0, s2 = 0, s02 = 0, m0 = 0, m1 = 0, m2 = 0;
  bool bad = false;
  auto posterior = [&](uint64_t i) -> double {
    if constexpr (TILE) return tile_col[post_ind_off(i)];
    if (one_block) return marg_blocks[site * I_blk + i];
    const uint64_t q = i / I_blk;
    return marg_blocks[(q * S_own + site) * I_blk + (i - q * I_blk)];
  };
  auto take = [&](uint32_t code, double F) {
    const double tF = 2 - F;
    const bool g1 = code == 1, g2 = code == 2, g3 = code == 3;
    n1 += g1 ? 1.0 : 0.0;
    bad |= g1 && !(F < 1);
    s2 += g2 ? tF : 0.0;
    s02 += (code == 0 || g2) ? tF : 0.0;
    m0 += g3 ? 1 - F : 0.0;
    m1 += g3 ? tF : 0.0;
    m2 += g3 ? F * tF : 0.0;
  };
  uint64_t i = lane;
  for (; i + 192 < I_tot; i += 256) {
    double F[4];
    uint32_t cd[4];
#pragma unroll
    for (int j = 0; j < 4; ++j) {
      F[j] = posterior(i + 64 * j);
      cd[j] = gl_code(gl.codes, cell_s + i + 64 * j);
    }
#pragma unroll
    for (int j = 0; j < 4; ++j) take(cd[j], F[j]);
  }
  for (; i < I_tot; i += 64) take(gl_code(gl.codes, cell_s + i), posterior(i));
  const double A0 = wave_sum(n1 + s2), B0 = wave_sum(2 * n1 + s02);
  m0 = wave_sum(m0);
  m1 = wave_sum(m1);
  m2 = wave_sum(m2);
  const bool any_bad = __ballot(bad) != 0;
  if (lane == 0) {
    state[ESTC_A0 * state_stride + site] = A0;
    state[ESTC_B0 * state_stride + site] = B0;
    state[ESTC_M0 * state_stride + site] = m0;
    state[ESTC_M1 * state_stride + site] = m1;
    state[ESTC_M2 * state_stride + site] = m2;
    redo[site] = any_bad ? 1 : 0;
  }
}

__global__ void __launch_bounds__(256)
k_fast_estmaf_called_passes(uint64_t S_own, double* __restrict__ freq_out, uint8_t* __restrict__ redo,
                            uint8_t* __restrict__ status, const double* __restrict__ state,
                            uint64_t state_stride, uint64_t tile_T, uint64_t row0, uint64_t row1) {
  const uint64_t site = (uint64_t)blockIdx.x * blockDim.x + threadIdx.x;
  if (site >= S_own || !in_tile_rows(site, tile_T, row0, row1)) return;
  status[site] = EST_DONE;
  if (redo[site]) return;
  const double A0 = state[ESTC_A0 * state_stride + site], B0 = state[ESTC_B0 * state_stride + site];
  const double m0 = state[ESTC_M0 * state_stride + site], m1 = state[ESTC_M1 * state_stride + site];
  const double m2 = state[ESTC_M2 * state_stride + site];
  int iters = 0;
  double num = 0, den = 0, pnum = 0.01, pden = 1.0;
  for (;;) {
    const double f = pnum / pden, om = 1 - f;
    const double b = f * om, ff = f * f;
    const double miss_n = fma(2 * b, m0, fma(ff, m1, b * m2));
    const double miss_d = fma(4 * b, m0, fma(fma(om, om, ff), m1, 2 * b * m2));
    num += A0 + miss_n;
    den += B0 + miss_d;
    const double lhs = fabs(fma(pnum, den, -(num * pden))), thr = kEPS * (den * pden);
    const bool again = (lhs > thr) && (iters++ < 100);
    pnum = num;
    pden = den;
    if (!again) break;
  }
  const double freq = num / den;
  const bool ok = freq >= 0 && freq < 1;
  freq_out[site] = freq;
  redo[site] = ok ? 0 : 1;
}

__device__ void estmaf_stream_site(const GlView& gl, const double* __restrict__ marg_blocks,
                                   uint64_t S_own, uint64_t I_tot, uint64_t I_blk, uint64_t tile_T,
                                   double* __restrict__ freq_out, uint64_t site, int lane) {
  const uint64_t cell_s = site * I_tot;
  const uint64_t tj = tile_T ? site / tile_T : 0;
  const double* trow =
      tile_T ? marg_blocks + post_lane_off((tj >> 6) * tile_T + (site - tj * tile_T), tj & 63, I_tot)
             : nullptr;
  int iters = 0;
  double num = 0, den = 0, freq = 0.01, prev;
  bool again;
  do {
    prev = freq;
    const double om = 1 - freq;
    const double b = om * freq;
    const double A = om * om, Cq = freq * freq;
    double pn = 0, pd = 0;
    for (uint64_t i = lane; i < I_tot; i += 64) {
      const double F = trow ? trow[post_ind_off(i)]
                            : marg_blocks[((i / I_blk) * S_own + site) * I_blk + (i % I_blk)];
      const double bF = b * F;
      const double h0 = A + bF, h2 = Cq + bF;
      const double h1 = (F == 1) ? 0.0 : (2 * b) * (1 - F);
      double p0, p1, p2;
      gl_fetch(gl, cell_s + i, p0, p1, p2);
      const double w0 = p0 * h0, w1 = p1 * h1, w2 = p2 * h2;
      const double sum = w0 + w1 + w2;
      const double tF = 2 - F;
      if (sum > 0) {
        const double inv = 1.0 / sum;
        pn += fma(w2, tF, w1) * inv;
        pd += fma(w0 + w2, tF, 2 * w1) * inv;
      } else {
        double lg[3] = {log(p0), log(p1), log(p2)};
        for (int k = 0; k < 3; ++k)
          if (lg[k] == -__builtin_huge_val()) lg[k] = -kINF;
        const double2 tt = estmaf_term_logspace(lg, freq, F);
        pn += tt.x;
        pd += tt.y;
      }
    }
    num += wave_sum(pn);
    den += wave_sum(pd);
    freq = num / den;
    again = (fabs(prev - freq) > kEPS) && (iters++ < 100);
  } while (again);
  if (lane == 0) freq_out[site] = freq;
}

__global__ void __launch_bounds__(256)
k_fast_estmaf_stream(const GlView gl, const double* __restrict__ marg_blocks,
                     uint64_t S_own, uint64_t I_tot, uint64_t I_blk, uint64_t tile_T,
                     double* __restrict__ freq_out, const uint8_t* __restrict__ redo,
                     uint64_t row0, uint64_t row1, uint32_t* __restrict__ cnt) {
  const int lane = threadIdx.x & 63;
  const uint64_t wave = (uint64_t)blockIdx.x * (blockDim.x >> 6) + (threadIdx.x >> 6);
  const uint64_t n_waves = (uint64_t)gridDim.x * (blockDim.x >> 6);
  if (!redo) {
    for (uint64_t site = wave; site < S_own; site += n_waves)
      if (in_tile_rows(site, tile_T, row0, row1))
        estmaf_stream_site(gl, marg_blocks, S_own, I_tot, I_blk, tile_T, freq_out, site, lane);
    return;
  }
  for (uint64_t base = wave * 64; base < S_own; base += n_waves * 64) {
    const uint64_t s = base + lane;
    const bool need = s < S_own && in_tile_rows(s, tile_T, row0, row1) && redo[s];
    uint64_t mask = __ballot(need);
    if (mask && lane == 0) atomicAdd(cnt + EST_CNT_LOGSPACE, (uint32_t)__popcll(mask));
    while (mask) {
      const int b = __builtin_ctzll(mask);
      mask &= mask - 1;
      estmaf_stream_site(gl, marg_blocks, S_own, I_tot, I_blk, tile_T, freq_out, base + b, lane);
    }
  }
}

}


bool fast_estmaf_called(const FastState& fs, const GlView& gl) {
  return !gl.dense && gl.codes && fs.called_table && !fs.sw.estmaf_no_called;
}

bool fast_estmaf_in_place(const FastState& fs, uint64_t I_tot) {
  return I_tot <= 8192 || (fs.packed && fs.called_table && !fs.sw.estmaf_no_called);
}

bool fast_estmaf_splittable(const FastState& fs, uint64_t I_tot, bool tile_major) {
  if (tile_major && fs.packed && fs.called_table && !fs.sw.estmaf_no_called) return true;
  return tile_major && I_tot > 128 && I_tot <= 8192;
}

bool fast_estmaf_reserve(FastState& fs, uint64_t S_own) {
  if (!fs.est_counts) {
    if (hipMalloc((void**)&fs.est_counts, EST_COUNTS * sizeof(uint32_t)) != hipSuccess) return false;
    if (hipMemset(fs.est_counts, 0, EST_COUNTS * sizeof(uint32_t)) != hipSuccess) return false;
    if (hipDeviceSynchronize() != hipSuccess) return false;
  }
  if (S_own <= fs.redo_cap) return true;
  if (fs.redo) (void)hipFree(fs.redo);
  if (fs.est_status) (void)hipFree(fs.est_status);
  if (fs.est_state) (void)hipFree(fs.est_state);
  fs.redo = fs.est_status = nullptr;
  fs.est_state = nullptr;
  fs.redo_cap = 0;
  if (hipMalloc((void**)&fs.redo, S_own) != hipSuccess) return false;
  if (hipMalloc((void**)&fs.est_status, S_own) != hipSuccess) return false;
  if (hipMalloc((void**)&fs.est_state, S_own * EST_FIELDS * sizeof(double)) != hipSuccess) return false;
  fs.redo_cap = S_own;
  return true;
}

static bool estmaf_dyn_lds(const void* kernel, size_t bytes) {
  if (bytes <= 65536) return true;
  static std::vector<std::pair<const void*, int>> told;
  static std::mutex mu;
  int dev = 0;
  (void)hipGetDevice(&dev);
  std::lock_guard<std::mutex> lock(mu);
  const std::pair<const void*, int> key{kernel, dev};
  if (std::find(told.begin(), told.end(), key) != told.end()) return true;
  const hipError_t e =
      hipFuncSetAttribute(kernel, hipFuncAttributeMaxDynamicSharedMemorySize, (int)bytes);
  if (e != hipSuccess) {
    (void)hipGetLastError();
    capi::set_error("est_maf: the kernel needs %zu bytes of dynamic LDS per workgroup and the "
                    "device refuses them (hipFuncSetAttribute: %s)", bytes, hipGetErrorString(e));
    return false;
  }
  told.push_back(key);
  return true;
}

bool fast_estmaf(FastState& fs, hipStream_t st, const GlView& d_gl_sites,
                 const double* d_marg_blocks, uint64_t S_own, uint64_t I_tot, uint64_t I_blk,
                 double* d_freq_out, bool tile_major, uint32_t part, uint32_t n_parts) {
  if (S_own == 0) return true;
  if (n_parts == 0 || part >= n_parts) return false;
  if (n_parts > 1 && !fast_estmaf_splittable(fs, I_tot, tile_major)) return false;
  const uint64_t n_rows = (uint64_t)fs.C * fs.T;
  const uint64_t row0 = n_parts > 1 ? n_rows * part / n_parts : 0;
  const uint64_t row1 = n_parts > 1 ? n_rows * (part + 1) / n_parts : n_rows;
  const uint64_t blk0 = row0 * 64, nblk = (row1 - row0) * 64;
  if (nblk == 0) return true;
  if (tile_major && !((I_tot <= 8192 || fast_estmaf_called(fs, d_gl_sites)) && I_blk == I_tot &&
                      S_own == fs.S))
    return false;
  const uint64_t tile_T = tile_major ? fs.T : 0;
  const bool stream_all = I_tot > 8192 && !tile_major;
  const uint64_t stream_wgs = stream_all ? (S_own + 3) / 4 : (S_own + 255) / 256;
  const dim3 grid((unsigned)(stream_wgs < 65536 ? stream_wgs : 65536)), block(256);
  if (!fast_estmaf_reserve(fs, S_own)) return false;
  if (fast_estmaf_called(fs, d_gl_sites)) {
    if (tile_major)
      hipLaunchKernelGGL((k_fast_estmaf_called_sums<true>), dim3((unsigned)nblk), dim3(64), 0, st,
                         d_gl_sites, d_marg_blocks, S_own, I_tot, I_blk, tile_T, fs.redo, fs.est_state,
                         fs.redo_cap, blk0);
    else
      hipLaunchKernelGGL((k_fast_estmaf_called_sums<false>), dim3((unsigned)S_own), dim3(64), 0, st,
                         d_gl_sites, d_marg_blocks, S_own, I_tot, I_blk, tile_T, fs.redo, fs.est_state,
                         fs.redo_cap, (uint64_t)0);
    hipLaunchKernelGGL(k_fast_estmaf_called_passes, dim3((unsigned)((S_own + 255) / 256)), dim3(256), 0,
                       st, S_own, d_freq_out, fs.redo, fs.est_status, fs.est_state, fs.redo_cap, tile_T,
                       row0, row1);
    hipLaunchKernelGGL(k_fast_estmaf_stream, grid, block, 0, st, d_gl_sites, d_marg_blocks, S_own,
                       I_tot, I_blk, tile_T, d_freq_out, fs.redo, row0, row1, fs.est_counts);
    return hipGetLastError() == hipSuccess;
  }
  bool interp = true;
  interp = fs.sw.estmaf_interp != 0;
  const uint64_t scan_wgs_all = (S_own + 63) / 64;
  const unsigned scan_wgs = (unsigned)(scan_wgs_all < 16384 ? scan_wgs_all : 16384);
#define ESTMAF_DYN(B) ((B) > 64 ? (size_t)EN * (B) * sizeof(double2) : (size_t)0)
#define ESTMAF_TELL(K, B) estmaf_dyn_lds(reinterpret_cast<const void*>(K), ESTMAF_DYN(B))
#define LAUNCH_NI(N, B)                                                                         \
  do {                                                                                          \
    if (fresh) {                                                                                \
      if (!ESTMAF_TELL((k_fast_estmaf<N, B, false>), B)) return false;                          \
      hipLaunchKernelGGL((k_fast_estmaf<N, B, false>), dim3((unsigned)S_own), dim3(B),          \
                         ESTMAF_DYN(B), st, d_gl_sites, d_marg_blocks, S_own, I_tot, I_blk,     \
                         (uint64_t)0, d_freq_out, fs.redo, fs.est_status, fs.est_state,         \
                         fs.redo_cap, n_exact, allow_build, (uint64_t)0, fs.est_counts);        \
    } else {                                                                                    \
      if (!ESTMAF_TELL((k_fast_estmaf_resume<N, B, false>), B)) return false;                   \
      hipLaunchKernelGGL((k_fast_estmaf_resume<N, B, false>), dim3(scan_wgs), dim3(B),          \
                         ESTMAF_DYN(B), st, d_gl_sites, d_marg_blocks, S_own, I_tot, I_blk,     \
                         (uint64_t)0, d_freq_out, fs.redo, fs.est_status, fs.est_state,         \
                         fs.redo_cap, n_exact, allow_build, row0, row1, fs.est_counts,          \
                         cnt_slot);                                                             \
    }                                                                                           \
  } while (0)
#define LAUNCH_TILE(N, B)                                                                       \
  do {                                                                                          \
    if (fresh) {                                                                                \
      if (!ESTMAF_TELL((k_fast_estmaf<N, B, true>), B)) return false;                           \
      hipLaunchKernelGGL((k_fast_estmaf<N, B, true>), dim3((unsigned)nblk), dim3(B),            \
                         ESTMAF_DYN(B), st, d_gl_sites, d_marg_blocks, S_own, I_tot, I_blk,     \
                         tile_T, d_freq_out, fs.redo, fs.est_status, fs.est_state, fs.redo_cap, \
                         n_exact, allow_build, blk0, fs.est_counts);                            \
    } else {                                                                                    \
      if (!ESTMAF_TELL((k_fast_estmaf_resume<N, B, true>), B)) return false;                    \
      hipLaunchKernelGGL((k_fast_estmaf_resume<N, B, true>), dim3(scan_wgs), dim3(B),           \
                         ESTMAF_DYN(B), st, d_gl_sites, d_marg_blocks, S_own, I_tot, I_blk,     \
                         tile_T, d_freq_out, fs.redo, fs.est_status, fs.est_state, fs.redo_cap, \
                         n_exact, allow_build, row0, row1, fs.est_counts, cnt_slot);            \
    }                                                                                           \
  } while (0)
#define LAUNCH_ROWS(N, TL)                                                                      \
  do {                                                                                          \
    if (fresh)                                                                                  \
      hipLaunchKernelGGL((k_fast_estmaf_rows<N, TL>),                                            \
                         dim3((unsigned)((TL) ? fs.Spad / 4 : (S_own + 3) / 4)), dim3(64), 0,   \
                         st, d_gl_sites, d_marg_blocks, S_own, I_tot, I_blk, tile_T, d_freq_out, \
                         fs.redo, fs.est_status, fs.est_state, fs.redo_cap, n_exact,            \
                         allow_build, fs.est_counts);                                           \
    else                                                                                        \
      hipLaunchKernelGGL((k_fast_estmaf_rows_resume<N, TL>), dim3(scan_wgs), dim3(64), 0, st,    \
                         d_gl_sites, d_marg_blocks, S_own, I_tot, I_blk, tile_T, d_freq_out,    \
                         fs.redo, fs.est_status, fs.est_state, fs.redo_cap, n_exact,            \
                         allow_build, fs.est_counts, cnt_slot);                                 \
  } while (0)
  const bool rows = I_tot <= 128 && !fs.sw.estmaf_no_rows;
  auto launch = [&](int fresh, int n_exact, int allow_build, int cnt_slot = 0) -> bool {
    if (rows) {
      if (tile_major) {
        if (I_tot <= 16) LAUNCH_ROWS(1, true);
        else if (I_tot <= 32) LAUNCH_ROWS(2, true);
        else if (I_tot <= 64) LAUNCH_ROWS(4, true);
        else LAUNCH_ROWS(8, true);
      } else {
        if (I_tot <= 16) LAUNCH_ROWS(1, false);
        else if (I_tot <= 32) LAUNCH_ROWS(2, false);
        else if (I_tot <= 64) LAUNCH_ROWS(4, false);
        else LAUNCH_ROWS(8, false);
      }
      return true;
    }
    if (tile_major) {
      if (I_tot <= 64) LAUNCH_TILE(1, 64);
      else if (I_tot <= 128) LAUNCH_TILE(2, 64);
      else if (I_tot <= 256) LAUNCH_TILE(4, 64);
      else if (I_tot <= 512) LAUNCH_TILE(8, 64);
      else if (I_tot <= 768) LAUNCH_TILE(12, 64);
      else if (I_tot <= 1024) LAUNCH_TILE(16, 64);
      else if (I_tot <= 1536) LAUNCH_TILE(12, 128);
      else if (I_tot <= 2048) LAUNCH_TILE(16, 128);
      else if (I_tot <= 3072) LAUNCH_TILE(12, 256);
      else if (I_tot <= 4096) LAUNCH_TILE(16, 256);
      else if (I_tot <= 5120) LAUNCH_TILE(10, 512);
      else if (I_tot <= 6144) LAUNCH_TILE(12, 512);
      else if (I_tot <= 7168) LAUNCH_TILE(14, 512);
      else LAUNCH_TILE(16, 512);
    } else if (I_tot <= 64) LAUNCH_NI(1, 64);
    else if (I_tot <= 128) LAUNCH_NI(2, 64);
    else if (I_tot <= 256) LAUNCH_NI(4, 64);
    else if (I_tot <= 512) LAUNCH_NI(8, 64);
    else if (I_tot <= 768) LAUNCH_NI(12, 64);
    else if (I_tot <= 1024) LAUNCH_NI(16, 64);
    else if (I_tot <= 1536) LAUNCH_NI(12, 128);
    else if (I_tot <= 2048) LAUNCH_NI(16, 128);
    else if (I_tot <= 3072) LAUNCH_NI(12, 256);
    else if (I_tot <= 4096) LAUNCH_NI(16, 256);
    else if (I_tot <= 5120) LAUNCH_NI(10, 512);
    else if (I_tot <= 6144) LAUNCH_NI(12, 512);
    else if (I_tot <= 7168) LAUNCH_NI(14, 512);
    else LAUNCH_NI(16, 512);
    return true;
  };
  const uint8_t* redo = fs.redo;
  if (I_tot > 8192 && !tile_major) {
    redo = nullptr;
  } else if (!interp) {
    if (!launch(1, 0, 0)) return false;
  } else {
    const dim3 igrid((unsigned)((S_own + 255) / 256));
    if (!launch(1, EST_K0, 1)) return false;
    hipLaunchKernelGGL(k_fast_estmaf_interp, igrid, dim3(256), 0, st, S_own, d_freq_out, fs.redo,
                       fs.est_status, fs.est_state, fs.redo_cap, tile_T, row0, row1);
    for (int again = 0; again < 2; ++again) {
      if (!launch(0, 1, 1, again ? EST_CNT_RESUMED_AGAIN : EST_CNT_RESUMED)) return false;
      hipLaunchKernelGGL(k_fast_estmaf_interp, igrid, dim3(256), 0, st, S_own, d_freq_out, fs.redo,
                         fs.est_status, fs.est_state, fs.redo_cap, tile_T, row0, row1);
    }
    if (!launch(0, 0, 0, EST_CNT_EXACT_TAIL)) return false;
  }
  hipLaunchKernelGGL(k_fast_estmaf_stream, grid, block, 0, st, d_gl_sites, d_marg_blocks, S_own,
                     I_tot, I_blk, tile_T, d_freq_out, redo, row0, row1, fs.est_counts);
#undef LAUNCH_NI
#undef ESTMAF_DYN
#undef ESTMAF_TELL
#undef LAUNCH_TILE
#undef LAUNCH_ROWS
  return hipGetLastError() == hipSuccess;
}

}
```

### ngsf-hmm_amd/csrc/nghmm_capi.hip

```cpp
#include "capi_internal.hpp"

namespace capi {

thread_local std::string g_last_error;

void set_error(const char* fmt, ...) {
  char buf[512];
  va_list ap;
  va_start(ap, fmt);
  vsnprintf(buf, sizeof buf, fmt, ap);
  va_end(ap);
  g_last_error = buf;
}


hipError_t sync_stream(nghmm_t* h) {
  if (!h->blocking_sync) return hipStreamSynchronize(h->stream);
  hipError_t e = hipEventRecord(h->ev_sync, h->stream);
  return e != hipSuccess ? e : hipEventSynchronize(h->ev_sync);
}

int use_device(nghmm_t* h) {
  HIP_TRY(hipSetDevice(h->device));
  return NGHMM_OK;
// ... 448 lines not shown
      launch_prepare_gl(h->stream, h->d_cls_log, 4, NGHMM_GL_LOG, 0, h->d_flags);
      if (hipMemcpyAsync(h->h_cls_proto, h->d_cls_log, sizeof h->h_cls_proto, hipMemcpyDeviceToHost,
                         h->stream) != hipSuccess ||
          sync_stream(h) != hipSuccess) { rc = NGHMM_ERR_HIP; break; }
    } else {
      if ((rc = h->d_gl.alloc(cells * 3))) break;
    }
    if ((rc = h->d_pos.alloc(n_sites))) break;
    if (mode == NGHMM_MODE_FAST && !fast_create(h->fast, n_ind, n_sites, packed)) { rc = NGHMM_ERR_NOMEM; break; }
  } while (0);
  if (rc != NGHMM_OK) {
    if (g_last_error.empty()) set_error("nghmm_create failed (%d)", rc);
    delete h;
    return rc;
  }
  *out = h;
  return NGHMM_OK;
}

int nghmm_destroy(nghmm_t* h) {
  if (!h) return NGHMM_OK;
  if (h->n_replicas.load() > 0) {
    set_error("nghmm_destroy: %d replica(s) of this handle are still alive", h->n_replicas.load());
    return NGHMM_ERR_ARG;
  }
  (void)hipSetDevice(h->device);
  if (h->stream) (void)hipStreamSynchronize(h->stream);
  chain_release(h);
  if (h->parent) h->parent->n_replicas.fetch_sub(1);
  delete h;
  return NGHMM_OK;
}

int nghmm_create_replica(nghmm_t** out, nghmm_t* parent) {
  g_last_error.clear();
  if (!out || !parent || !parent->loaded || parent->parent) {
    set_error("nghmm_create_replica: the parent must be a loaded handle that is not itself a replica");
    return NGHMM_ERR_ARG;
  }
  if (parent->I_tot != parent->I || parent->fast.shard.world > 1) {
    set_error("nghmm_create_replica: sharded handles have no replicas");
    return NGHMM_ERR_ARG;
  }
  int rc;
  if ((rc = use_device(parent))) return rc;
  nghmm_t* h = new (std::nothrow) nghmm_handle;
  if (!h) return NGHMM_ERR_NOMEM;
  h->I = parent->I;
  h->S = parent->S;
  h->device = parent->device;
  h->mode = parent->mode;
  h->packed = parent->packed;
  h->fast.sw = parent->fast.sw;
  h->I_tot = h->I;
  h->S_own = h->S;
  h->parent = parent;
  parent->batch.set_max_threads(1);
  h->batch.set_max_threads(1);
  h->d_gl.borrow(parent->d_gl);
  h->d_pos.borrow(parent->d_pos);
  h->d_codes.borrow(parent->d_codes);
  h->d_cls_log.borrow(parent->d_cls_log);
  h->blocking_sync = true;
  if ((rc = alloc_own_state(h)) == NGHMM_OK && h->mode == NGHMM_MODE_FAST &&
      !fast_create_replica(h->fast, parent->fast))
    rc = NGHMM_ERR_NOMEM;
  if (rc != NGHMM_OK) {
    if (g_last_error.empty()) set_error("nghmm_create_replica failed (%d)", rc);
    delete h;
    return rc;
  }
  h->loaded = true;
  parent->n_replicas.fetch_add(1);
  *out = h;
  return NGHMM_OK;
}

int nghmm_set_params(nghmm_t* h, const double* indF, const double* alpha, const double* freq) {
  g_last_error.clear();
  if (!h) return NGHMM_ERR_ARG;
  int rc;
  if ((rc = use_device(h))) return rc;
  if (indF || alpha) dbfgs_invalidate(h->fast);
  if (indF) {
    std::memcpy(h->h_indF.data(), indF, h->I * sizeof(double));
    HIP_TRY(hipMemcpyAsync(h->d_indF, indF, h->I * sizeof(double), hipMemcpyHostToDevice, h->stream));
  }
  if (alpha) {
    std::memcpy(h->h_alpha.data(), alpha, h->I * sizeof(double));
    HIP_TRY(hipMemcpyAsync(h->d_alpha, alpha, h->I * sizeof(double), hipMemcpyHostToDevice,
                           h->stream));
  }
  if (freq)
    HIP_TRY(hipMemcpyAsync(h->d_freq, freq, h->S * sizeof(double), hipMemcpyHostToDevice, h->stream));
  HIP_TRY(sync_stream(h));
  return NGHMM_OK;
}

int nghmm_get_params(nghmm_t* h, double* indF, double* alpha, double* freq) {
  g_last_error.clear();
  if (!h) return NGHMM_ERR_ARG;
  int rc;
  if ((rc = use_device(h))) return rc;
  if (indF) std::memcpy(indF, h->h_indF.data(), h->I * sizeof(double));
  if (alpha) std::memcpy(alpha, h->h_alpha.data(), h->I * sizeof(double));
  if (freq) {
    HIP_TRY(hipMemcpyAsync(freq, h->d_freq, h->S * sizeof(double), hipMemcpyDeviceToHost, h->stream));
    HIP_TRY(sync_stream(h));
  }
  return NGHMM_OK;
}

int nghmm_emission(nghmm_t* h) {
  g_last_error.clear();
  if (!h || !h->loaded) return NGHMM_ERR_ARG;
  int rc;
  if ((rc = use_device(h))) return rc;
  if (!h->warmed) {
    h->warmed = true;
    h->batch.reserve(h->I);
    if (h->mode == NGHMM_MODE_FAST) {
      if ((rc = lane_setup(h, 0, (size_t)h->I * 5)) || (rc = lane_setup(h, 1, (size_t)h->I * 5))) return rc;
      if (h->I_tot == h->I && !fast_estmaf_reserve(h->fast, h->S)) return NGHMM_ERR_NOMEM;
      if (!h->fast.sw.no_dev_bfgs && dbfgs_available(h->fast) && !dbfgs_reserve(h->fast)) return NGHMM_ERR_NOMEM;
    }
  }
  return emission_impl(h);
}

int nghmm_estep(nghmm_t* h, double* ind_lkl) {
  g_last_error.clear();
  if (!h || !h->loaded) return NGHMM_ERR_ARG;
  int rc;
  if ((rc = use_device(h))) return rc;
  if (h->mode == NGHMM_MODE_FAST) return fast_estep_impl(h, ind_lkl, false);
  if ((rc = clear_flags(h))) return rc;
  {
    tic(h);
    (h->fast.sw.exact_serial ? launch_forward_exact : launch_forward_exact_pc)(
        h->stream, h->d_eprob, h->d_pos, h->S, h->I, (uint32_t)h->I, nullptr, h->d_indF,
        h->d_alpha, h->d_ind_lkl, h->d_fw, h->d_flags);
    if ((rc = toc(h, SLOT_FORWARD, false))) return rc;
    tic(h);
    h->tmp_is_posteriors = false;
    (h->fast.sw.exact_serial ? launch_backward_exact : launch_backward_exact_pc)(
        h->stream, h->d_eprob, h->d_pos, h->d_fw, h->S, h->I, h->d_indF, h->d_alpha,
        h->d_ind_lkl, h->d_marg, h->d_flags);
    if ((rc = toc(h, SLOT_BACKWARD, false))) return rc;
  }
  HIP_TRY(hipGetLastError());
  if (ind_lkl)
    HIP_TRY(hipMemcpyAsync(ind_lkl, h->d_ind_lkl, h->I * sizeof(double), hipMemcpyDeviceToHost,
                           h->stream));
  return check_flags(h);
}

int nghmm_lkl_batch(nghmm_t* h, uint32_t n_pts, const uint32_t* ind, const double* F,
                    const double* alpha, double* lkl) {
  g_last_error.clear();
  if (!h || !h->loaded || (n_pts && (!ind || !F || !alpha || !lkl))) return NGHMM_ERR_ARG;
  int rc;
  if ((rc = use_device(h))) return rc;
  return lkl_batch_impl(h, n_pts, ind, F, alpha, lkl, false);
}

namespace {

struct MstepRun {
  nghmm_t* h;
  int indF_fixed, alpha_fixed;
  bool fuse_estep, fuse_freq;
  double* ind_lkl;
  nghmm_hook_fn after_estep;
  void* user;

  BfgsBatch& batch;
  std::function<int()> before_round;
  bool estep_pending = false;
  bool bg_active = false;
  bool bg_begun = false;
  hipStream_t bg_stream = nullptr;
  const double *estep_F = nullptr, *estep_A = nullptr;
  bool tile_major = false;
  uint32_t bg_parts = 0, bg_next = 0;
  double t_gather = 0, t_lkl = 0, t_estep = 0, t_scatter = 0;
  std::vector<uint32_t> ind;
  std::vector<double> F, A, lkl;

  using clock = std::chrono::steady_clock;
  static double since(clock::time_point t0) {
    return std::chrono::duration<double, std::milli>(clock::now() - t0).count();
  }

  MstepRun(nghmm_t* h_, int f, int a, bool fe, double* il, nghmm_hook_fn hook, void* u, bool ff)
      : h(h_), indF_fixed(f), alpha_fixed(a), fuse_estep(fe), fuse_freq(ff), ind_lkl(il),
        after_estep(hook), user(u), batch(h_->batch) {}

  int estep_then_hook(bool have_walk) {
    const int r = fast_estep_impl(h, ind_lkl, have_walk);
    if (r == NGHMM_OK && after_estep) after_estep(user);
    return r;
  }

  bool wants_background() const {
    return fuse_freq && fuse_estep && !after_estep && h->mode == NGHMM_MODE_FAST &&
           h->I_tot == h->I && h->fast.sw.bg_parts != 0;
  }

  bool wants_two_lanes() const {
    if (h->fast.shard.world > 1) return false;
    return h->mode == NGHMM_MODE_FAST && h->I >= 2 && (uint64_t)h->I * h->fast.C < 16384;
  }

  int start_background(bool have_walk) {
    int r;
    if (!have_walk && (r = ensure_emissions(h))) return r;
    if (!bg_begun && (r = bg_begin(h))) return r;
    bg_begun = true;
    hipStream_t bs = bg_stream ? bg_stream : h->stream;
    if ((r = bg_open(h, SLOT_FORWARD, bs))) return r;
    if (!fast_estep(h->fast, bs, estep_F ? estep_F : h->d_indF, estep_A ? estep_A : h->d_alpha,
                    h->d_ind_lkl, h->d_flags_bg, have_walk))
      return NGHMM_ERR_HIP;
    if ((r = bg_close(h, bs))) return r;
    h->ms[SLOT_BACKWARD] = 0;
    h->launches[SLOT_BACKWARD] = 0;
    h->marg_valid = false;
    h->tmp_is_posteriors = false;
    tile_major = fast_estmaf_in_place(h->fast, h->I);
    bg_parts = 1;
    if (fast_estmaf_splittable(h->fast, h->I, tile_major)) {
      bg_parts = h->fast.sw.bg_parts >= 1 ? (uint32_t)h->fast.sw.bg_parts : 1;
    }
    bg_next = 0;
    bg_active = true;
    return NGHMM_OK;
  }

  int push_background_piece() {
    if (bg_next >= bg_parts) return NGHMM_OK;
    const uint32_t part = bg_next++;
    int q;
    hipStream_t bs = bg_stream ? bg_stream : h->stream;
    if ((q = bg_open(h, SLOT_ESTMAF, bs))) return q;
    if (!tile_major && (q = ensure_marg(h))) return q;
    if (!fast_estmaf(h->fast, bs, fast_gl_lin(h->fast),
                     tile_major ? h->fast.post : h->d_marg, h->S, h->I, h->I, h->d_freq,
                     tile_major, part, bg_parts))
      return NGHMM_ERR_HIP;
    return bg_close(h, bs);
  }

  int first_or_plain_round() {
    int rc;
    if (before_round && (rc = before_round())) return rc;
    auto t0 = clock::now();
    const size_t n = batch.gather(ind, F, A);
    lkl.resize(n);
    t_gather += since(t0);
    bool emit = estep_pending;
    t0 = clock::now();
    if (n) {
      if ((rc = lkl_batch_impl(h, (uint32_t)n, ind.data(), F.data(), A.data(), lkl.data(), true,
                               &emit)))
        return rc;
    } else {
      emit = false;
    }
    t_lkl += since(t0);
    if (estep_pending) {
      t0 = clock::now();
      if ((rc = wants_background() ? start_background(emit) : estep_then_hook(emit))) return rc;
      estep_pending = false;
      t_estep += since(t0);
    }
    t0 = clock::now();
    batch.scatter(lkl.data());
    t_scatter += since(t0);
    return NGHMM_OK;
  }

  int round_with_background() {
    int rc;
    auto& L = h->lane[0];
    auto t0 = clock::now();
    const size_t n = batch.gather(L.ind, L.F, L.A, 0, h->I);
    t_gather += since(t0);
    if (n) {
      t0 = clock::now();
      if ((rc = lkl_submit(h, 0))) return rc;
      if ((rc = push_background_piece())) return rc;
      if ((rc = lkl_wait(h, 0))) return rc;
      t_lkl += since(t0);
    }
    t0 = clock::now();
    batch.scatter(L.h_lkl, 0, h->I);
    t_scatter += since(t0);
    return NGHMM_OK;
  }

  int feed_lane(int k) {
    auto& L = h->lane[k];
    for (;;) {
      auto t1 = clock::now();
      const size_t n = batch.gather(L.ind, L.F, L.A, L.lo, L.hi);
      t_gather += since(t1);
      if (n) {
        t1 = clock::now();
        const int r = lkl_submit(h, k);
        t_lkl += since(t1);
        return r;
      }
      if (batch.active_in(L.lo, L.hi) == 0) return NGHMM_OK;
      batch.scatter(L.h_lkl, L.lo, L.hi);
    }
  }

  int two_lane_rounds() {
    int rc;
    const uint64_t half = (h->I + 1) / 2;
    h->lane[0].lo = 0;
    h->lane[0].hi = half;
    h->lane[1].lo = half;
    h->lane[1].hi = h->I;
    if ((rc = ensure_emissions(h))) return rc;
    for (int k = 0; k < 2; ++k)
      if ((rc = feed_lane(k))) return rc;
    while (bg_active && bg_next < bg_parts)
// ... 294 lines not shown
    for (size_t p = 0; p < n; ++p) lkl[p] = fn(ind[p], F[p], A[p], user);
    batch.scatter(lkl.data());
  }
  batch.result(indF, alpha);
  if (stats) {
    stats->rounds = batch.rounds();
    stats->points = batch.points();
    stats->ref_forward_calls = batch.ref_forward_calls();
    stats->ind_rounds = batch.ind_rounds();
  }
  return NGHMM_OK;
}

int nghmm_bfgs_batch_host2(uint64_t n_ind, double* indF, double* alpha, int indF_fixed,
                           int alpha_fixed, nghmm_objective_fn fn, void* user,
                           nghmm_mstep_stats* stats, int flags) {
  g_last_error.clear();
  if (!indF || !alpha || !fn) return NGHMM_ERR_ARG;
  if (stats) std::memset(stats, 0, sizeof *stats);
  if (indF_fixed && alpha_fixed) return NGHMM_OK;
  const bool det = (flags & 1) != 0;
  if (!(flags & 2)) {
    BfgsBatch batch;
    batch.set_det_pow(det);
    batch.set_max_threads(1);
    batch.begin(n_ind, indF, alpha, indF_fixed != 0, alpha_fixed != 0);
    std::vector<uint32_t> ind;
    std::vector<double> F, A, lkl;
    while (!batch.done()) {
      const size_t n = batch.gather(ind, F, A);
      lkl.resize(n);
      for (size_t p = 0; p < n; ++p) lkl[p] = fn(ind[p], F[p], A[p], user);
      batch.scatter(lkl.data());
    }
    batch.result(indF, alpha);
    if (stats) {
      stats->rounds = batch.rounds();
      stats->points = batch.points();
      stats->ref_forward_calls = batch.ref_forward_calls();
      stats->ind_rounds = batch.ind_rounds();
    }
    return NGHMM_OK;
  }
  std::vector<double> block(LbfgsbPtrs::doubles(2, 10));
  uint64_t points = 0, ref_calls = 0, ind_rounds = 0;
  uint32_t rounds = 0;
  for (uint64_t i = 0; i < n_ind; ++i) {
    BfgsProblem p;
    bfgs_problem_begin(p, indF[i], alpha[i], indF_fixed != 0, alpha_fixed != 0);
    LbfgsbT<PtrStore> solver;
    solver.st_.bind(block.data(), 2, 10);
    for (;;) {
      if (det) bfgs_plan<DetPow>(p);
      else bfgs_plan<LibmPow>(p);
      ++p.n_rounds;
      ++ind_rounds;
      double lklv[5] = {0, 0, 0, 0, 0};
      for (int k = 0; k < 5; ++k)
        if (p.slot_used[k] && !p.slot_nonfinite[k]) {
          lklv[k] = fn((uint32_t)i, p.pt[k][0], p.pt[k][1], user);
          ++points;
        }
      const bool again = bfgs_consume(p, solver, lklv, ref_calls, [&](BfgsProblem& q) {
        const int nbd[2] = {2, 2};
        solver.start_bound(2, 10, q.x, q.lb, q.ub, nbd, 1.0e6, 1.0e-3);
      });
      if (!again) break;
    }
    if (p.n_rounds > rounds) rounds = p.n_rounds;
    indF[i] = p.x[0];
    alpha[i] = p.x[1];
  }
  if (stats) {
    stats->rounds = rounds;
    stats->points = points;
    stats->ref_forward_calls = ref_calls;
    stats->ind_rounds = ind_rounds;
  }
  return NGHMM_OK;
}

}

int capi::estmaf_and_refresh(nghmm_t* h, bool shard, const double* d_marg_blocks, uint64_t S_own,
                              uint64_t I_tot, uint64_t I_blk, double* d_freq_out) {
  int rc;
  tic(h);
  if (h->mode == NGHMM_MODE_FAST) {
    const GlView lin = !shard ? fast_gl_lin(h->fast)
                       : h->packed ? gl_packed(h->d_codes_shard, h->fast.cls_lin)
                                   : gl_dense(h->d_gl_shard);
    bool tile_major = false;
    if (!d_marg_blocks) {
      tile_major = fast_estmaf_in_place(h->fast, I_tot);
      if (tile_major) {
        d_marg_blocks = h->fast.post;
      } else {
        if ((rc = ensure_marg(h))) return rc;
        d_marg_blocks = h->d_marg;
      }
    }
    if (!fast_estmaf(h->fast, h->stream, lin, d_marg_blocks, S_own, I_tot, I_blk, d_freq_out,
                     tile_major))
      return NGHMM_ERR_HIP;
  } else {
    if (I_blk != I_tot) {
      set_error("exact-mode est_maf expects one posterior block");
      return NGHMM_ERR_ARG;
    }
    const GlView lg = !shard ? own_gl(h)
                      : h->packed ? gl_packed(h->d_codes_shard, h->d_cls_log)
                                  : gl_dense(h->d_gl_shard);
    launch_estmaf_exact(h->stream, lg, d_marg_blocks, S_own, I_tot, d_freq_out, nullptr, 0);
  }
  if ((rc = toc(h, SLOT_ESTMAF, false))) return rc;
  HIP_TRY(hipGetLastError());
  return NGHMM_OK;
}

extern "C" {

static int mstep_freq_ld_impl(nghmm_t* h, int freq_est, int e_prob) {
  const bool exact = h->mode == NGHMM_MODE_EXACT;
  if (h->I_tot != h->I || h->fast.shard.world > 1 || h->chain || h->g_n > 1) {
    set_error("the intended --freq_est 2 walks the sites in order on ONE handle: not available "
              "for a sharded cohort");
    return NGHMM_ERR_ARG;
  }
  if (e_prob == 2 && !exact) {
    set_error("the intended --e_prob 2 needs materialised emissions: NGHMM_MODE_EXACT only");
    return NGHMM_ERR_ARG;
  }
  if (h->I > 8192) {
    set_error("the intended --freq_est 2 holds a site pair's cohort in one workgroup: at most "
              "8192 individuals");
    return NGHMM_ERR_ARG;
  }
  int rc;
  if (!h->d_freq_new && (rc = h->d_freq_new.alloc(h->S))) return rc;
  if (!h->d_hap && (rc = h->d_hap.alloc((size_t)h->S * 4))) return rc;
  if ((rc = clear_flags(h))) return rc;
  if (!exact && (rc = ensure_marg(h))) return rc;
  const uint64_t n_est = freq_est == 1 ? h->S : 1;
  tic(h);
  if (exact) {
    launch_estmaf_exact(h->stream, own_gl(h), h->d_marg, n_est, h->I, h->d_freq_new, nullptr, 0);
  } else if (!fast_estmaf(h->fast, h->stream, fast_gl_lin(h->fast), h->d_marg, n_est, h->I, h->I,
                          h->d_freq_new, false)) {
    return NGHMM_ERR_HIP;
  }
  if (!launch_freq_ld_chain(h->stream, exact, exact ? own_gl(h) : fast_gl_lin(h->fast), h->d_marg,
                            h->d_freq, h->d_freq_new, h->d_hap, h->S, h->I, freq_est, h->d_flags))
    return NGHMM_ERR_ARG;
  HIP_TRY(hipMemcpyAsync(h->d_freq, h->d_freq_new, h->S * sizeof(double), hipMemcpyDeviceToDevice,
                         h->stream));
  if ((rc = toc(h, SLOT_ESTMAF, false))) return rc;
  HIP_TRY(hipGetLastError());
  int f[NFLAGS];
  HIP_TRY(hipMemcpyAsync(f, h->d_flags, sizeof f, hipMemcpyDeviceToHost, h->stream));
  HIP_TRY(sync_stream(h));
  if (f[FLAG_LD_FREQ]) {
    set_error("invalid allele frequencies");
    return NGHMM_ERR_FREQ_EST2;
  }
  if ((rc = emission_impl(h))) return rc;
  if (e_prob == 2) {
    if ((rc = clear_flags(h))) return rc;
    launch_emission_ld_exact(h->stream, own_gl(h), h->d_freq, h->d_hap, h->d_eprob, h->S, h->I,
                             h->d_flags);
    HIP_TRY(hipGetLastError());
    if ((rc = check_flags(h))) return rc;
  }
  return NGHMM_OK;
}

int nghmm_mstep_freq(nghmm_t* h, int freq_est) {
  g_last_error.clear();
  if (!h || !h->loaded) return NGHMM_ERR_ARG;
  int rc;
  if ((rc = use_device(h))) return rc;
  if (freq_est & NGHMM_LD_INTENDED) {
    const int fe = freq_est & 3, ep = (freq_est & NGHMM_EPROB_LD) ? 2 : 1;
    if ((freq_est & ~(NGHMM_LD_INTENDED | NGHMM_EPROB_LD | 3)) || (fe != 1 && fe != 2)) {
      set_error("wrong MAF estimation method!");
      return NGHMM_ERR_ARG;
    }
    if (fe == 1 && ep == 1) freq_est = 1;
    else return mstep_freq_ld_impl(h, fe, ep);
  }
  if (freq_est == 0) return NGHMM_OK;
  if (freq_est == 2) {
    set_error("invalid allele frequencies");
    return NGHMM_ERR_FREQ_EST2;
  }
  if (freq_est != 1) {
    set_error("wrong MAF estimation method!");
    return NGHMM_ERR_ARG;
  }
  if (h->I_tot != h->I) {
    set_error("sharded handle: use nghmm_mstep_freq_sites_dev");
    return NGHMM_ERR_ARG;
  }
  if ((rc = estmaf_and_refresh(h, false, h->mode == NGHMM_MODE_FAST ? nullptr : h->d_marg, h->S,
                               h->I, h->I, h->d_freq)))
    return rc;
  return emission_impl(h);
}

int nghmm_estep_mstep(nghmm_t* h, int indF_fixed, int alpha_fixed, double* ind_lkl,
                      nghmm_mstep_stats* stats, nghmm_hook_fn after_estep, void* user) {
  g_last_error.clear();
  if (!h || !h->loaded) return NGHMM_ERR_ARG;
  int rc;
  if ((rc = use_device(h))) return rc;
  if (h->mode == NGHMM_MODE_FAST)
    return mstep_indf_impl(h, indF_fixed, alpha_fixed, stats, true, ind_lkl, after_estep, user);
  if ((rc = nghmm_estep(h, ind_lkl))) return rc;
  if (after_estep) after_estep(user);
  return nghmm_mstep_indf(h, indF_fixed, alpha_fixed, stats);
}

int nghmm_iter_em(nghmm_t* h, int freq_est, int indF_fixed, int alpha_fixed, double* ind_lkl,
                  nghmm_mstep_stats* stats) {
  g_last_error.clear();
  if (!h || !h->loaded) return NGHMM_ERR_ARG;
  int rc;
  if ((rc = use_device(h))) return rc;
  if (h->mode == NGHMM_MODE_FAST) {
    bool freq_done = false;
    if ((rc = mstep_indf_impl(h, indF_fixed, alpha_fixed, stats, true, ind_lkl, nullptr, nullptr,
                              freq_est == 1, &freq_done)))
      return rc;
// ... 125 lines not shown
  PinBuf<uint8_t> b;
  if (bytes == 0 || b.alloc(bytes) != NGHMM_OK) {
    (void)hipGetLastError();
    return nullptr;
  }
  return b.release();
}

void nghmm_free_host(void* p) {
  PinBuf<uint8_t> b;
  b.adopt(static_cast<uint8_t*>(p));
}

int nghmm_set_switch(nghmm_t* h, const char* name, long value) {
  g_last_error.clear();
  if (!h || !name) return NGHMM_ERR_ARG;
  if (std::strcmp(name, "fast_c") == 0) {
    set_error("nghmm_set_switch: fast_c is fixed when the handle is created (NGHMM_FAST_C in the environment)");
    return NGHMM_ERR_ARG;
  }
  if (!h->fast.sw.set(name, value)) {
    set_error("nghmm_set_switch: no switch named %s", name);
    return NGHMM_ERR_ARG;
  }
  return NGHMM_OK;
}

int nghmm_fast_layout(nghmm_t* h, uint32_t* waves_per_individual, uint64_t* sites_per_lane) {
  if (!h) return NGHMM_ERR_ARG;
  const bool fast = h->mode == NGHMM_MODE_FAST;
  if (waves_per_individual) *waves_per_individual = fast ? h->fast.C : 0;
  if (sites_per_lane) *sites_per_lane = fast ? h->fast.T : 0;
  return NGHMM_OK;
}

void* nghmm_stream(nghmm_t* h) { return h ? (void*)h->stream : nullptr; }

int nghmm_synchronize(nghmm_t* h) {
  g_last_error.clear();
  if (!h) return NGHMM_ERR_ARG;
  HIP_TRY(hipSetDevice(h->device));
  HIP_TRY(sync_stream(h));
  return NGHMM_OK;
}

int nghmm_kernel_ms(nghmm_t* h, int slot, double* ms, uint32_t* launches) {
  if (!h || slot < 0 || slot >= NSLOTS) return NGHMM_ERR_ARG;
  if (ms) *ms = h->ms[slot];
  if (launches) *launches = h->launches[slot];
  return NGHMM_OK;
}

int nghmm_debug_mode_counts(nghmm_t* h, nghmm_mode_count* out, uint32_t cap, uint32_t* n, int reset) {
  g_last_error.clear();
  if (!h || (!out && cap)) return NGHMM_ERR_ARG;
  uint32_t k = 0;
  for (const auto& kv : h->fast.mode_ind_rounds) {
    if (k < cap) out[k] = nghmm_mode_count{kv.first, kv.second};
    ++k;
  }
  if (n) *n = k;
  if (reset) h->fast.mode_ind_rounds.clear();
  return NGHMM_OK;
}

int nghmm_debug_estmaf_counts(nghmm_t* h, uint64_t out[5], int reset) {
  g_last_error.clear();
  if (!h || !out) return NGHMM_ERR_ARG;
  for (int k = 0; k < 5; ++k) out[k] = 0;
  if (!h->fast.est_counts) return NGHMM_OK;
  int rc;
  if ((rc = use_device(h))) return rc;
  uint32_t v[EST_COUNTS];
  HIP_TRY(sync_stream(h));
  HIP_TRY(hipMemcpy(v, h->fast.est_counts, sizeof v, hipMemcpyDeviceToHost));
  for (int k = 0; k < 5; ++k) out[k] = v[k];
  if (reset) {
    HIP_TRY(hipMemset(h->fast.est_counts, 0, sizeof v));
    HIP_TRY(hipDeviceSynchronize());
  }
  return NGHMM_OK;
}

}
```

### ngsf-hmm_amd/hmm.py

```python
from __future__ import annotations

import ctypes as C
import weakref
import math
import os
import subprocess

import numpy as np

MODE_EXACT = 0
MODE_FAST = 1
GENO_PACKED = 0x10
LD_INTENDED = 0x20
EPROB_LD = 0x40

_HERE = os.path.dirname(os.path.abspath(__file__))
_LIB = None

c_double_p = C.POINTER(C.c_double)
HOOK_FN = C.CFUNCTYPE(None, C.c_void_p)
ALLGATHER_FN = C.CFUNCTYPE(C.c_int, C.c_void_p, C.c_uint64)


class NgsFHMMError(RuntimeError):
# ... 7 lines not shown
class ModeCount(C.Structure):
    _fields_ = [("mode", C.c_uint32), ("ind_rounds", C.c_uint64)]


class MstepStats(C.Structure):
    _fields_ = [("rounds", C.c_uint32), ("points", C.c_uint64),
                ("ref_forward_calls", C.c_uint64), ("ind_rounds", C.c_uint64)]


def library_path():
    return os.environ.get("NGHMM_LIB") or os.path.join(_HERE, "libnghmm.so")


def build_library(verbose=False):
    out = None if verbose else subprocess.DEVNULL
    subprocess.run(["make", "-C", os.path.join(_HERE, "csrc"), "-j4"], check=True, stdout=out)
    return library_path()


def load_library():
    global _LIB
    if _LIB is not None:
        return _LIB
    path = library_path()
    if not os.path.exists(path):
        raise NgsFHMMError(-11, f"{path} is missing: build it with "
                                "`python -c 'import __graft_entry__ as g; g.build()'` "
                                "(the hot path has no CPU fallback)")
    L = C.CDLL(path)
    vp, u64, u32, i32, d = C.c_void_p, C.c_uint64, C.c_uint32, C.c_int, C.c_double
    dp = c_double_p
    sig = {
        "nghmm_last_error": (C.c_char_p, []),
        "nghmm_strerror": (C.c_char_p, [i32]),
        "nghmm_has_hip": (i32, []),
        "nghmm_create": (i32, [C.POINTER(vp), u64, u64, i32, i32]),
        "nghmm_destroy": (i32, [vp]),
        "nghmm_create_replica": (i32, [C.POINTER(vp), vp]),
        "nghmm_load_gl": (i32, [vp, dp, dp]),
        "nghmm_load_gl_raw": (i32, [vp, dp, i32, i32, i32, dp]),
        "nghmm_get_gl": (i32, [vp, dp]),
        "nghmm_geno_posteriors": (i32, [vp, u64, u64, dp]),
        "nghmm_format_posteriors": (i32, [vp, u64, u64, C.c_char_p]),
        "nghmm_format_fixed6": (i32, [vp, dp, u64, u64, C.c_char_p]),
        "nghmm_load_gl_device": (i32, [vp, vp, vp]),
        "nghmm_load_begin": (i32, [vp, dp]),
        "nghmm_load_begin_dev": (i32, [vp, vp]),
        "nghmm_load_gl_raw_sites": (i32, [vp, u64, u64, dp, i32, i32, i32]),
        "nghmm_load_gl_raw_sites_dev": (i32, [vp, u64, u64, vp, i32, i32, i32]),
        "nghmm_load_geno_sites": (i32, [vp, u64, u64, C.POINTER(C.c_int8)]),
        "nghmm_load_end": (i32, [vp]),
        "nghmm_get_geno_codes_dev": (i32, [vp, u64, u64, vp]),
        "nghmm_load_geno_site_shard_dev": (i32, [vp, vp]),
        "nghmm_set_params": (i32, [vp, dp, dp, dp]),
        "nghmm_get_params": (i32, [vp, dp, dp, dp]),
        "nghmm_emission": (i32, [vp]),
        "nghmm_estep": (i32, [vp, dp]),
        "nghmm_lkl_batch": (i32, [vp, u32, C.POINTER(u32), dp, dp, dp]),
        "nghmm_mstep_indf": (i32, [vp, i32, i32, C.POINTER(MstepStats)]),
        "nghmm_bfgs_batch_host": (i32, [u64, dp, dp, i32, i32, vp, vp, C.POINTER(MstepStats)]),
        "nghmm_bfgs_batch_host2": (i32, [u64, dp, dp, i32, i32, vp, vp, C.POINTER(MstepStats), i32]),
        "nghmm_mstep_freq": (i32, [vp, i32]),
        "nghmm_estep_mstep": (i32, [vp, i32, i32, dp, C.POINTER(MstepStats), HOOK_FN, vp]),
        "nghmm_iter_em": (i32, [vp, i32, i32, i32, dp, C.POINTER(MstepStats)]),
        "nghmm_viterbi": (i32, [vp, C.POINTER(C.c_uint8)]),
        "nghmm_get_posteriors": (i32, [vp, dp]),
        "nghmm_get_emissions": (i32, [vp, dp]),
        "nghmm_shard_config": (i32, [vp, u64, u64, u64, u64]),
        "nghmm_load_gl_site_shard": (i32, [vp, dp]),
        "nghmm_load_gl_site_shard_dev": (i32, [vp, vp]),
        "nghmm_pack_posteriors_dev": (i32, [vp, u64, u64, vp]),
        "nghmm_mstep_freq_sites_dev": (i32, [vp, vp, vp]),
        "nghmm_set_freq_dev": (i32, [vp, vp]),
        "nghmm_group_setup": (i32, [C.POINTER(vp), i32]),
        "nghmm_group_iter_em": (i32, [C.POINTER(vp), i32, i32, i32, i32, dp, C.POINTER(MstepStats)]),
        "nghmm_group_mstep_freq": (i32, [C.POINTER(vp), i32, i32]),
        "nghmm_fast_layout": (i32, [vp, C.POINTER(u32), C.POINTER(u64)]),
        "nghmm_stream": (vp, [vp]),
        "nghmm_synchronize": (i32, [vp]),
        "nghmm_kernel_ms": (i32, [vp, i32, dp, C.POINTER(u32)]),
        "nghmm_set_switch": (i32, [vp, C.c_char_p, C.c_long]),
        "nghmm_debug_mode_counts": (i32, [vp, C.POINTER(ModeCount), u32, C.POINTER(u32), i32]),
        "nghmm_debug_estmaf_counts": (i32, [vp, C.POINTER(u64), i32]),
        "nghmm_alloc_host": (vp, [u64]),
        "nghmm_free_host": (None, [vp]),
        "nghmm_site_shard_bytes": (u64, [vp]),
        "nghmm_site_shard_setup": (i32, [vp, i32, i32, vp, vp, u64, ALLGATHER_FN, vp]),
        "nghmm_chain_setup": (i32, [C.POINTER(vp), i32]),
        "nghmm_chain_iter_em": (i32, [C.POINTER(vp), i32, i32, i32, i32, dp, C.POINTER(MstepStats)]),
        "nghmm_chain_mstep_freq": (i32, [C.POINTER(vp), i32, i32]),
        "nghmm_chain_viterbi": (i32, [C.POINTER(vp), i32, C.POINTER(C.c_uint8)]),
        "nghmm_viterbi_shard_forward": (i32, [vp, dp, dp]),
        "nghmm_viterbi_shard_back": (i32, [vp, C.POINTER(C.c_uint8), C.POINTER(C.c_uint8),
                                           C.POINTER(C.c_uint8)]),
        "nghmm_ibd_tracts": (i32, [vp, i32, d, u64, vp, u64, C.POINTER(u64)]),
        "nghmm_chain_ibd_tracts": (i32, [C.POINTER(vp), i32, i32, d, u64, vp, u64, C.POINTER(u64)]),
        "nghmm_sample_paths": (i32, [vp, u64, u32, vp, u32, C.POINTER(C.c_uint8)]),
        "nghmm_chain_sample_paths": (i32, [C.POINTER(vp), i32, u64, u32, vp, u32,
                                           C.POINTER(C.c_uint8)]),
        "nghmm_obs_info": (i32, [vp, dp, dp, vp]),
        "nghmm_chain_obs_info": (i32, [C.POINTER(vp), i32, dp, dp, vp]),
        "nghmm_ibd_summary": (i32, [vp, i32, d, u64, C.POINTER(u64), C.POINTER(u64), vp, vp]),
        "nghmm_chain_ibd_summary": (i32, [C.POINTER(vp), i32, i32, d, u64, C.POINTER(u64),
                                          C.POINTER(u64), vp, vp]),
    }
    for name, (res, args) in sig.items():
        fn = getattr(L, name)
        fn.restype = res
        fn.argtypes = args
    _LIB = L
    return L


def _dp(a):
    return a.ctypes.data_as(c_double_p)


EXPORTED_SYMBOLS = [
    "nghmm_last_error", "nghmm_strerror", "nghmm_has_hip", "nghmm_create", "nghmm_destroy",
    "nghmm_create_replica",
    "nghmm_load_gl", "nghmm_load_gl_raw", "nghmm_get_gl", "nghmm_geno_posteriors",
    "nghmm_format_posteriors", "nghmm_format_fixed6",
    "nghmm_load_gl_device", "nghmm_load_begin", "nghmm_load_begin_dev", "nghmm_load_gl_raw_sites",
    "nghmm_load_gl_raw_sites_dev", "nghmm_load_geno_sites", "nghmm_load_end",
    "nghmm_get_geno_codes_dev", "nghmm_load_geno_site_shard_dev",
    "nghmm_set_params", "nghmm_get_params",
    "nghmm_emission", "nghmm_estep", "nghmm_lkl_batch", "nghmm_mstep_indf",
    "nghmm_bfgs_batch_host", "nghmm_bfgs_batch_host2", "nghmm_mstep_freq", "nghmm_estep_mstep",
    "nghmm_iter_em", "nghmm_viterbi", "nghmm_get_posteriors", "nghmm_get_emissions",
    "nghmm_shard_config", "nghmm_load_gl_site_shard", "nghmm_load_gl_site_shard_dev",
    "nghmm_pack_posteriors_dev",
    "nghmm_mstep_freq_sites_dev", "nghmm_set_freq_dev", "nghmm_group_setup", "nghmm_group_iter_em",
    "nghmm_group_mstep_freq",
    "nghmm_fast_layout", "nghmm_stream",
    "nghmm_synchronize",
    "nghmm_kernel_ms", "nghmm_set_switch", "nghmm_debug_mode_counts", "nghmm_debug_estmaf_counts",
    "nghmm_site_shard_bytes", "nghmm_site_shard_setup", "nghmm_viterbi_shard_forward",
    "nghmm_viterbi_shard_back", "nghmm_chain_setup", "nghmm_chain_iter_em", "nghmm_chain_mstep_freq",
    "nghmm_chain_viterbi", "nghmm_alloc_host", "nghmm_free_host",
    "nghmm_ibd_tracts", "nghmm_chain_ibd_tracts",
    "nghmm_sample_paths", "nghmm_chain_sample_paths",
    "nghmm_obs_info", "nghmm_chain_obs_info",
    "nghmm_ibd_summary", "nghmm_chain_ibd_summary",
]

OBJECTIVE_FN = C.CFUNCTYPE(C.c_double, C.c_uint32, C.c_double, C.c_double, C.c_void_p)


def bfgs_batch_host(indF, alpha, objective, indF_fixed=False, alpha_fixed=False, det_pow=None,
                    device_solver=False):
    L = load_library()
    F = np.array(indF, dtype=np.float64)
    A = np.array(alpha, dtype=np.float64)
    st = MstepStats()
    cb = OBJECTIVE_FN(lambda i, f, a, _u: float(objective(i, f, a)))
    if det_pow is None and not device_solver:
        rc = L.nghmm_bfgs_batch_host(len(F), _dp(F), _dp(A), int(indF_fixed), int(alpha_fixed),
                                     C.cast(cb, C.c_void_p), None, C.byref(st))
    else:
        rc = L.nghmm_bfgs_batch_host2(len(F), _dp(F), _dp(A), int(indF_fixed), int(alpha_fixed),
                                      C.cast(cb, C.c_void_p), None, C.byref(st),
                                      (1 if det_pow else 0) | (2 if device_solver else 0))
    if rc != 0:
        raise NgsFHMMError(rc, L.nghmm_strerror(rc).decode())
    return F, A, st


TRACTS_VITERBI = 0
TRACTS_POSTERIOR = 1


class Tract(C.Structure):
    _fields_ = [("first_site", C.c_uint64), ("n_sites", C.c_uint64), ("ind", C.c_uint32),
                ("reserved", C.c_uint32), ("post_sum", C.c_double)]


TRACT_DTYPE = np.dtype([("ind", np.uint32), ("first_site", np.uint64), ("n_sites", np.uint64),
                        ("post_sum", np.float64), ("post_mean", np.float64)])


def _tract_source(source):
    src = {"viterbi": TRACTS_VITERBI, "posterior": TRACTS_POSTERIOR}.get(source, source)
    if src not in (TRACTS_VITERBI, TRACTS_POSTERIOR):
        raise NgsFHMMError(-10, f"ibd_tracts: unknown source {source!r} ('viterbi' or 'posterior')")
    return src


def _tracts(call, check, source, threshold, min_sites):
    src = _tract_source(source)
    n = C.c_uint64(0)
    check(call(src, float(threshold), int(min_sites), None, 0, C.byref(n)))
    buf = (Tract * max(n.value, 1))()
    if n.value:
        got = C.c_uint64(0)
        check(call(src, float(threshold), int(min_sites), C.cast(buf, C.c_void_p), n.value,
                   C.byref(got)))
        assert got.value == n.value
    raw = np.frombuffer(buf, dtype=np.dtype([("first_site", np.uint64), ("n_sites", np.uint64),
                                             ("ind", np.uint32), ("reserved", np.uint32),
                                             ("post_sum", np.float64)]), count=n.value)
    out = np.empty(n.value, dtype=TRACT_DTYPE)
    for f in ("ind", "first_site", "n_sites", "post_sum"):
        out[f] = raw[f]
    out["post_mean"] = out["post_sum"] / np.maximum(out["n_sites"], 1)
    return out


def bed_lines(tracts, chrom_names, positions, ind_names):
    lines = []
    for t in tracts:
        a = int(t["first_site"])
        b = a + int(t["n_sites"]) - 1
        start, end = int(positions[a]) - 1, int(positions[b])
        lines.append(f"{chrom_names[a]}\t{start}\t{end}\t{ind_names[int(t['ind'])]}\t{end - start}\n")
    return "".join(lines)


PATH_STATS_DTYPE = np.dtype([("ibd_sites", np.uint64), ("n_tracts", np.uint64),
                             ("longest_sites", np.uint64), ("ibd_mb", np.float64)])
# ... 406 lines not shown
        def _cb(_user, n):
            try:
                allgather(int(n))
                return 0
            except BaseException as e:
                self._shard_err.append(e)
                return 1

        self._shard_cb = ALLGATHER_FN(_cb) if world > 1 else C.cast(None, ALLGATHER_FN)
        self._check(self.lib.nghmm_site_shard_setup(self._h, int(rank), int(world), C.c_void_p(send_ptr),
                                                    C.c_void_p(recv_ptr), int(nbytes), self._shard_cb,
                                                    None))

    def viterbi_shard_forward(self, scores_in=None):
        out = np.empty((self.n_ind, 2))
        if scores_in is not None:
            scores_in = np.ascontiguousarray(scores_in, dtype=np.float64).reshape(self.n_ind, 2)
        self._check(self.lib.nghmm_viterbi_shard_forward(
            self._h, _dp(scores_in) if scores_in is not None else None, _dp(out)))
        return out

    def viterbi_shard_back(self, state_after=None):
        u8p = C.POINTER(C.c_uint8)
        before = np.empty(self.n_ind, dtype=np.uint8)
        path = np.empty((self.n_ind, self.n_sites), dtype=np.uint8)
        if state_after is not None:
            state_after = np.ascontiguousarray(state_after, dtype=np.uint8).reshape(self.n_ind)
        self._check(self.lib.nghmm_viterbi_shard_back(
            self._h, state_after.ctypes.data_as(u8p) if state_after is not None else None,
            before.ctypes.data_as(u8p), path.ctypes.data_as(u8p)))
        return before, path

    def viterbi(self):
        path = np.empty((self.n_ind, self.n_sites), dtype=np.uint8)
        self._check(self.lib.nghmm_viterbi(self._h, path.ctypes.data_as(C.POINTER(C.c_uint8))))
        return path

    def ibd_tracts(self, source="viterbi", threshold=0.5, min_sites=1):
        return _tracts(lambda *a: self.lib.nghmm_ibd_tracts(self._h, *a), self._check, source,
                       threshold, min_sites)

    def sample_paths(self, n_draws, seed=0, keep=0):
        return _sample_paths(lambda *a: self.lib.nghmm_sample_paths(self._h, *a), self._check,
                             self.n_ind, self.n_sites, n_draws, seed, keep)

    def obs_info(self, indF=None, alpha=None):
        return _obs_info(lambda *a: self.lib.nghmm_obs_info(self._h, *a), self._check, self.n_ind,
                         indF, alpha)

    def ibd_summary(self, regions=None, what=("viterbi", "posterior"), threshold=0.5, sites=True):
        return _ibd_summary(lambda *a: self.lib.nghmm_ibd_summary(self._h, *a), self._check,
                            self.n_ind, self.n_sites, regions, what, threshold, sites)

    def kernel_ms(self, name):
        ms = C.c_double(0)
        n = C.c_uint32(0)
        self._check(self.lib.nghmm_kernel_ms(self._h, KERNEL_SLOTS[name], C.byref(ms), C.byref(n)))
        return ms.value, n.value

    def synchronize(self):
        self._check(self.lib.nghmm_synchronize(self._h))

    @staticmethod
    def mode_name(mode):
        if mode == 0xffffffff:
            return "rounds_of_mixed_versions"
        if mode == 0:
            return "general"
        return (f"{(mode >> 2) & 3}F{mode & 3}A" + ("s" if mode & 0x200 else "") +
                ("2" if mode & 0x400 else "") + ("e" if mode & 0x800 else ""))

    def mode_counts(self, reset=False):
        buf = (ModeCount * 160)()
        n = C.c_uint32(0)
        self._check(self.lib.nghmm_debug_mode_counts(self._h, buf, 160, C.byref(n), int(reset)))
        return {self.mode_name(buf[k].mode): int(buf[k].ind_rounds) for k in range(min(n.value, 160))}

    def estmaf_counts(self, reset=False):
        v = (C.c_uint64 * 5)()
        self._check(self.lib.nghmm_debug_estmaf_counts(self._h, v, int(reset)))
        return {"check_failed": int(v[0]), "second_interval": int(v[1]), "third_interval": int(v[2]),
                "log_space": int(v[3]), "exact_tail": int(v[4])}


class Group:

    def __init__(self, handles):
        self.handles = list(handles)
        self.lib = self.handles[0].lib
        n = len(self.handles)
        self._arr = (C.c_void_p * n)(*[h._h for h in self.handles])
        self.handles[0]._check(self.lib.nghmm_group_setup(self._arr, n))
        self.ind_lkl = np.full(n * self.handles[0].n_ind, -math.inf)

    def _members_open(self):
        if any(h.closed for h in self.handles):
            raise NgsFHMMError(-10, "a member of this group has been closed")

    def mstep_freq(self, freq_est=1):
        self._members_open()
        self.handles[0]._check(self.lib.nghmm_group_mstep_freq(self._arr, len(self.handles),
                                                               int(freq_est)))

    def iter_EM(self, freq_est=1, indF_fixed=False, alpha_fixed=False):
        self._members_open()
        st = MstepStats()
        self.handles[0]._check(self.lib.nghmm_group_iter_em(
            self._arr, len(self.handles), int(freq_est), int(indF_fixed), int(alpha_fixed),
            _dp(self.ind_lkl), C.byref(st)))
        return st


class Chain:

    def __init__(self, handles):
        self.handles = list(handles)
        self.lib = self.handles[0].lib
        n = len(self.handles)
        self._arr = (C.c_void_p * n)(*[h._h for h in self.handles])
        self.handles[0]._check(self.lib.nghmm_chain_setup(self._arr, n))
        self.n_ind = self.handles[0].n_ind
        self.n_sites = sum(h.n_sites for h in self.handles)
        self.ind_lkl = np.full(self.n_ind, -math.inf)

    def _members_open(self):
        if any(h.closed for h in self.handles):
            raise NgsFHMMError(-10, "a member of this chain has been closed")

    def mstep_freq(self, freq_est=1):
        self._members_open()
        self.handles[0]._check(self.lib.nghmm_chain_mstep_freq(self._arr, len(self.handles),
                                                               int(freq_est)))

    def iter_EM(self, freq_est=1, indF_fixed=False, alpha_fixed=False):
        self._members_open()
        st = MstepStats()
        self.handles[0]._check(self.lib.nghmm_chain_iter_em(
            self._arr, len(self.handles), int(freq_est), int(indF_fixed), int(alpha_fixed),
            _dp(self.ind_lkl), C.byref(st)))
        return st

    def viterbi(self):
        self._members_open()
        path = np.empty((self.n_ind, self.n_sites), dtype=np.uint8)
        self.handles[0]._check(self.lib.nghmm_chain_viterbi(
            self._arr, len(self.handles), path.ctypes.data_as(C.POINTER(C.c_uint8))))
        return path

    def ibd_tracts(self, source="viterbi", threshold=0.5, min_sites=1):
        self._members_open()
        return _tracts(lambda *a: self.lib.nghmm_chain_ibd_tracts(self._arr, len(self.handles), *a),
                       self.handles[0]._check, source, threshold, min_sites)

    def sample_paths(self, n_draws, seed=0, keep=0):
        self._members_open()
        return _sample_paths(
            lambda *a: self.lib.nghmm_chain_sample_paths(self._arr, len(self.handles), *a),
            self.handles[0]._check, self.n_ind, self.n_sites, n_draws, seed, keep)

    def obs_info(self, indF=None, alpha=None):
        self._members_open()
        return _obs_info(lambda *a: self.lib.nghmm_chain_obs_info(self._arr, len(self.handles), *a),
                         self.handles[0]._check, self.n_ind, indF, alpha)

    def ibd_summary(self, regions=None, what=("viterbi", "posterior"), threshold=0.5, sites=True):
        self._members_open()
# ... 12 lines not shown
```

Baseline: 42.81 billion.

## Warm-start est_maf interpolation interval from previous EM iteration's converged ratio

Stores each site's final fixed-point ratio from the frequency M-step and, on the next call, uses it to predict the interpolation interval right after the first iteration instead of waiting for several fixed-point steps. When the predicted interval is narrow it also picks fewer Chebyshev nodes (6, 8 or 10 instead of 12), which cuts the per-site node evaluations over all individuals. It adds a per-site buffer, extra state fields, striped debug counters and cache invalidation on parameter and data changes. The risk is more failed interpolation checks that fall back to exact iteration, plus extra atomics and memory traffic.

```diff
diff --git a/include/nghmm_debug.h b/include/nghmm_debug.h
--- a/include/nghmm_debug.h
+++ b/include/nghmm_debug.h
@@ -22,6 +22,12 @@
 int nghmm_debug_mode_counts(nghmm_t* h, nghmm_mode_count* out, uint32_t cap, uint32_t* n, int reset);
 int nghmm_debug_estmaf_counts(nghmm_t* h, uint64_t out[5], int reset);
 
+int nghmm_debug_estmaf_predict_counts(nghmm_t* h, uint64_t out[7], int reset);
+
+int nghmm_debug_estmaf_r_end(nghmm_t* h, double* r_end, uint64_t n, int set);
+
+int nghmm_debug_estmaf_state(nghmm_t* h, int field, double* out, uint64_t n);
+
 #ifdef __cplusplus
 }
 #endif
diff --git a/ngsf-hmm_amd/csrc/capi_internal.hpp b/ngsf-hmm_amd/csrc/capi_internal.hpp
--- a/ngsf-hmm_amd/csrc/capi_internal.hpp
+++ b/ngsf-hmm_amd/csrc/capi_internal.hpp
@@ -88,6 +88,7 @@
   DevScratch<uint8_t> d_info;
   DevScratch<uint8_t> d_summ;
   DevBuf<double> d_freq_new, d_hap;
+  DevScratch<double> d_est_rend;
 
   uint64_t I_tot = 0, ind_begin = 0, site_begin = 0, S_own = 0;
   DevBuf<double> d_gl_shard;
@@ -166,6 +167,7 @@
 int bg_finish(nghmm_t* h);
 int ensure_emissions(nghmm_t* h);
 
+int estmaf_carry(nghmm_t* h, uint64_t n_sites);
 int estmaf_and_refresh(nghmm_t* h, bool shard, const double* d_marg_blocks, uint64_t S_own,
                        uint64_t I_tot, uint64_t I_blk, double* d_freq_out);
 void chain_release(nghmm_t* h);
diff --git a/ngsf-hmm_amd/csrc/capi_multi.hip b/ngsf-hmm_amd/csrc/capi_multi.hip
--- a/ngsf-hmm_amd/csrc/capi_multi.hip
+++ b/ngsf-hmm_amd/csrc/capi_multi.hip
@@ -201,8 +201,10 @@
     set_error("exact-mode sharded est_maf is not available; use NGHMM_MODE_FAST");
     return NGHMM_ERR_ARG;
   }
-  if ((rc = estmaf_and_refresh(h, true, d_marg_blocks, h->S_own, h->I_tot, h->I, d_freq_out)))
-    return rc;
+  fast_estmaf_forget(h->fast);
+  rc = estmaf_and_refresh(h, true, d_marg_blocks, h->S_own, h->I_tot, h->I, d_freq_out);
+  fast_estmaf_forget(h->fast);
+  if (rc) return rc;
   HIP_TRY(sync_stream(h));
   return NGHMM_OK;
 }
@@ -214,6 +216,7 @@
   if ((rc = use_device(h))) return rc;
   HIP_TRY(hipMemcpyAsync(h->d_freq, d_freq_all, h->S * sizeof(double), hipMemcpyDeviceToDevice,
                          h->stream));
+  fast_estmaf_forget(h->fast);
   return emission_impl(h);
 }
 
diff --git a/ngsf-hmm_amd/csrc/kernels_fast.hip b/ngsf-hmm_amd/csrc/kernels_fast.hip
--- a/ngsf-hmm_amd/csrc/kernels_fast.hip
+++ b/ngsf-hmm_amd/csrc/kernels_fast.hip
@@ -196,6 +196,7 @@
 const SwitchName kSwitches[] = {
     {"bg_parts", &Switches::bg_parts}, {"estmaf_interp", &Switches::estmaf_interp},
     {"estmaf_no_rows", &Switches::estmaf_no_rows}, {"estmaf_no_called", &Switches::estmaf_no_called},
+    {"estmaf_no_predict", &Switches::estmaf_no_predict},
     {"fast_c", &Switches::fast_c}, {"exact_serial", &Switches::exact_serial},
     {"dbg_abort_round", &Switches::dbg_abort_round}, {"no_dev_bfgs", &Switches::no_dev_bfgs},
     {"no_bg_stream", &Switches::no_bg_stream}, {"spans", &Switches::spans},
@@ -343,6 +344,7 @@
 
 bool fast_load(FastState& fs, hipStream_t st, const GlView& gl_log, const double* d_pos) {
   dbfgs_invalidate(fs);
+  fast_estmaf_forget(fs);
   fs.gl_log = gl_log;
   fs.d_pos = d_pos;
   fs.e_stale = true;
diff --git a/ngsf-hmm_amd/csrc/kernels_fast.hpp b/ngsf-hmm_amd/csrc/kernels_fast.hpp
--- a/ngsf-hmm_amd/csrc/kernels_fast.hpp
+++ b/ngsf-hmm_amd/csrc/kernels_fast.hpp
@@ -15,6 +15,7 @@
   int estmaf_interp = 1;
   int estmaf_no_rows = 0;
   int estmaf_no_called = 0;
+  int estmaf_no_predict = 0;
   int fast_c = 0;
   int exact_serial = 0;
   int dbg_abort_round = 0;
@@ -117,6 +118,9 @@
   size_t redo_cap = 0;
   uint8_t* est_status = nullptr;
   double* est_state = nullptr;
+  double* est_rend = nullptr;
+  size_t est_rend_cap = 0;
+  uint64_t est_rend_sites = 0;
   std::map<uint32_t, uint64_t> mode_ind_rounds;
   uint32_t* est_counts = nullptr;
 };
@@ -129,6 +133,17 @@
   EST_CNT_EXACT_TAIL = 4,
   EST_COUNTS = 5
 };
+enum EstStriped {
+  EST_PRED_N6 = 0,
+  EST_PRED_N8 = 1,
+  EST_PRED_N10 = 2,
+  EST_PRED_N12 = 3,
+  EST_PRED_FAILED = 4,
+  EST_PRED_LEFT = 5,
+  EST_STRIPED = 6
+};
+constexpr uint32_t EST_STRIPED_BASE = 32;
+constexpr uint32_t EST_COUNT_WORDS = EST_STRIPED_BASE + EST_STRIPED * 64 * 32;
 
 bool fast_create(FastState& fs, uint64_t I, uint64_t S, bool packed = false);
 bool fast_create_replica(FastState& fs, const FastState& parent);
@@ -172,6 +187,7 @@
 bool fast_estmaf_splittable(const FastState& fs, uint64_t I_tot, bool tile_major);
 bool fast_estmaf_in_place(const FastState& fs, uint64_t I_tot);
 bool fast_estmaf_reserve(FastState& fs, uint64_t S_own);
+void fast_estmaf_forget(FastState& fs);
 bool fast_estmaf_called(const FastState& fs, const GlView& gl);
 bool fast_estmaf(FastState& fs, hipStream_t st, const GlView& d_gl_lin_sites,
                  const double* d_marg_blocks, uint64_t S_own, uint64_t I_tot, uint64_t I_blk,
diff --git a/ngsf-hmm_amd/csrc/kernels_fast_estmaf.hip b/ngsf-hmm_amd/csrc/kernels_fast_estmaf.hip
--- a/ngsf-hmm_amd/csrc/kernels_fast_estmaf.hip
+++ b/ngsf-hmm_amd/csrc/kernels_fast_estmaf.hip
@@ -100,8 +100,9 @@
 }
 
 constexpr int EN = 12;
-constexpr int EST_SCALARS = 8;
+constexpr int EST_SCALARS = 9;
 constexpr int EST_FIELDS = EST_SCALARS + 2 * EN;
+constexpr int EST_NODES = 8;
 enum : uint8_t { EST_DONE = 0, EST_INTERP = 1, EST_EXACT = 2 };
 constexpr int EST_K0 = 2;
 constexpr int EST_MIN_GAIN = 24;
@@ -112,8 +113,76 @@
 constexpr int EST_KMAX = 32;
 constexpr double EST_TOL = 1e-11;
 constexpr double EST_GUARD = 1e-9;
-__constant__ double kChebC[EN] = {0.9914448613738104, 0.9238795325112867, 0.7933533402912352, 0.6087614290087207, 0.38268343236508984, 0.1305261922200517, -0.1305261922200516, -0.3826834323650895, -0.6087614290087207, -0.793353340291235, -0.9238795325112867, -0.9914448613738104};
-__constant__ double kChebW[EN] = {0.13052619222005157, -0.3826834323650898, 0.6087614290087207, -0.7933533402912352, 0.9238795325112867, -0.9914448613738104, 0.9914448613738104, -0.9238795325112868, 0.7933533402912352, -0.6087614290087209, 0.3826834323650899, -0.130526192220052};
+constexpr double EST_PM_REL = 0.25;
+constexpr double EST_PM_MIN = 0.02;
+constexpr double EST_H6 = 0.015408209381223507;
+constexpr double EST_H8 = 0.0519753424562587;
+constexpr double EST_H10 = 0.10760097663823423;
+constexpr int EST_TAB = 12 + 10 + 8 + 6;
+__host__ __device__ constexpr int est_tab(int n) { return n == 12 ? 0 : n == 10 ? 12 : n == 8 ? 22 : 30; }
+__constant__ double kChebC[EST_TAB] = {
+    0.9914448613738104, 0.9238795325112867, 0.7933533402912352, 0.6087614290087207, 0.38268343236508984, 0.1305261922200517, -0.1305261922200516, -0.3826834323650895, -0.6087614290087207, -0.793353340291235, -0.9238795325112867, -0.9914448613738104,
+    0.9876883405951378, 0.8910065241883679, 0.7071067811865476, 0.4539904997395468, 0.15643446504023087, -0.15643446504023087, -0.4539904997395468, -0.7071067811865476, -0.8910065241883679, -0.9876883405951378,
+    0.9807852804032304, 0.8314696123025452, 0.5555702330196022, 0.19509032201612828, -0.19509032201612828, -0.5555702330196022, -0.8314696123025452, -0.9807852804032304,
+    0.9659258262890683, 0.7071067811865476, 0.25881904510252074, -0.25881904510252074, -0.7071067811865476, -0.9659258262890683};
+__constant__ double kChebW[EST_TAB] = {
+    0.13052619222005157, -0.3826834323650898, 0.6087614290087207, -0.7933533402912352, 0.9238795325112867, -0.9914448613738104, 0.9914448613738104, -0.9238795325112868, 0.7933533402912352, -0.6087614290087209, 0.3826834323650899, -0.130526192220052,
+    0.15643446504023087, -0.4539904997395468, 0.7071067811865476, -0.8910065241883679, 0.9876883405951378, -0.9876883405951378, 0.8910065241883679, -0.7071067811865476, 0.4539904997395468, -0.15643446504023087,
+    0.19509032201612828, -0.5555702330196022, 0.8314696123025452, -0.9807852804032304, 0.9807852804032304, -0.8314696123025452, 0.5555702330196022, -0.19509032201612828,
+    0.25881904510252074, -0.7071067811865476, 0.9659258262890683, -0.9659258262890683, 0.7071067811865476, -0.25881904510252074};
+
+__device__ __forceinline__ void est_count(uint32_t* __restrict__ cnt, int slot, uint64_t key) {
+  atomicAdd(cnt + EST_STRIPED_BASE + ((((uint32_t)slot << 6) + ((uint32_t)key & 63u)) << 5), 1u);
+}
+
+__device__ __forceinline__ bool estmaf_interval(int iters, double lhs, double thr, double rn,
+                                                double rprev, double r_pred, bool& built,
+                                                int& n_before, double& mid, double& half, int& n,
+                                                bool& pred) {
+  const double m_est = (double)iters * (sqrt(lhs / thr) - 1.0);
+  const bool worth = m_est >= EST_MIN_GAIN && 100 - iters >= EST_MIN_GAIN;
+  bool up = false;
+  double g = 0;
+  pred = false;
+  if (iters == 1 && worth && rn > 0 && r_pred > 0 && r_pred < 1e300) {
+    up = r_pred >= rn;
+    const double travel = up ? r_pred / rn - 1 : rn / r_pred - 1;
+    g = fma(1 + travel, fmax(EST_PM_REL * travel, EST_PM_MIN), travel);
+    pred = g <= EST_DMAX;
+  }
+  if (!pred) {
+    if (--n_before > 0) return false;
+    const double step = fabs(rn - rprev);
+    const double reach = (rn >= rprev) ? EST_DMAX * rn : EST_DMAX / (1 + EST_DMAX) * rn;
+    const bool fits = (double)iters * step <= EST_FIT * reach;
+    if (!fits && iters < EST_KMAX && m_est >= EST_MIN_GAIN) {
+      n_before = 1;
+      return false;
+    }
+    built = true;
+    if (!worth) return false;
+    g = fmin(EST_DMAX, fmax(EST_MULT * step / rn, 1e-3));
+    up = rn >= rprev;
+  }
+  built = true;
+  double lo, hi;
+  if (up) {
+    lo = rn * (1 - EST_BACK * g);
+    hi = rn * (1 + g);
+  } else {
+    lo = rn / (1 + g);
+    hi = rn * (1 + EST_BACK * g);
+  }
+  const double a = sqrt(lo * hi), h = (hi - a) / (hi + a);
+  if (!(h > 0 && lo > 0 && hi < 1e300)) {
+    pred = false;
+    return false;
+  }
+  mid = a;
+  half = h;
+  n = !pred ? EN : h <= EST_H6 ? 6 : h <= EST_H8 ? 8 : h <= EST_H10 ? 10 : EN;
+  return true;
+}
 
 constexpr int ESTMAF_MAXW = 16;
 
@@ -133,7 +202,8 @@
 __device__ __forceinline__ void estmaf_site(
     const GlView& gl, const double* __restrict__ marg_blocks, uint64_t S_own, uint64_t I_tot,
     uint64_t I_blk, double* __restrict__ freq_out, uint8_t* __restrict__ redo,
-    uint8_t* __restrict__ status, double* __restrict__ state, uint64_t state_stride, int fresh,
+    uint8_t* __restrict__ status, double* __restrict__ state, uint64_t state_stride,
+    double* __restrict__ rend, int predict, int fresh,
     int n_exact, int allow_build, uint64_t site, const double* __restrict__ tile_col,
     uint32_t* __restrict__ cnt, double (&xch)[2][ESTMAF_MAXW][2],
     double2 (&nodebuf)[(BLOCK == 64 && NI >= 8) ? EN : 1][(BLOCK == 64 && NI >= 8) ? 65 : 1],
@@ -146,6 +216,8 @@
   const uint32_t tix = threadIdx.x;
   constexpr uint64_t stride = BLOCK;
   const uint64_t cell_s = site * I_tot;
+  double r_pred = __builtin_nan("");
+  if (fresh && predict) r_pred = rend[site];
 
   double tF_lane_out;
   double sA[NI], sb[NI], sC[NI], u0[NI], nC[NI], fc[NI];
@@ -210,6 +282,7 @@
     for (int w = 1; w < W; ++w) tF_sum += xch[1][w][0];
     __syncthreads();
   }
+  r_pred = lane_value(r_pred, 0);
 
   int iters = 0;
   int buf = 0;
@@ -224,7 +297,8 @@
   }
   bool built = !allow_build;
   int n_before = n_exact;
-  bool check = false, interp_ok = false;
+  bool check = false, interp_ok = false, pred = false;
+  int nn = EN, tab = 0;
   double mid = 0, half = 0, my_gn = 0, my_gd = 0, rprev = 0;
   auto lane_sums = [&](double r, double& pn, double& pd) {
     pn = 0;
@@ -291,14 +365,17 @@
       buf ^= 1;
     }
     if (check) {
-      const int nj = lane < EN ? lane : 0;
+      const int nj = tab + (lane < nn ? lane : 0);
       const double t = (r - mid) / (r + mid) - half * kChebC[nj];
-      const double q = (lane < EN) ? kChebW[nj] / t : 0.0;
+      const double q = (lane < nn) ? kChebW[nj] / t : 0.0;
       const double Sq = wave_sum_uniform(q);
       const double bn = wave_sum_uniform(q * my_gn) / Sq, bd = wave_sum_uniform(q * my_gd) / Sq;
       interp_ok = fabs(bn - sn) <= EST_TOL * fabs(sn) && fabs(bd - sd) <= EST_TOL * fabs(sd);
       check = false;
-      if (!interp_ok && tix == 0) atomicAdd(cnt + EST_CNT_CHECK_FAILED, 1u);
+      if (!interp_ok && tix == 0) {
+        atomicAdd(cnt + EST_CNT_CHECK_FAILED, 1u);
+        if (pred) est_count(cnt, EST_PRED_FAILED, blockIdx.x);
+      }
     }
     num = fma(r, sn, num);
     den = fma(r, sd, den + tF_sum);
@@ -310,7 +387,7 @@
     if (!again) break;
     if (interp_ok) {
       if (wv == 0) {
-        if (lane < EN) {
+        if (lane < nn) {
           state[(EST_SCALARS + lane) * state_stride + site] = my_gn;
           state[(EST_SCALARS + EN + lane) * state_stride + site] = my_gd;
         }
@@ -323,40 +400,27 @@
           state[5 * state_stride + site] = mid;
           state[6 * state_stride + site] = half;
           state[7 * state_stride + site] = tF_sum;
+          state[EST_NODES * state_stride + site] = pred ? -(double)nn : (double)nn;
           status[site] = EST_INTERP;
         }
       }
       return;
     }
-    if (!built && --n_before <= 0) {
-      const double m_est = (double)iters * (sqrt(lhs / thr) - 1.0);
+    if (!built) {
       const double rn = pnum * rcp_nr2(pden - pnum);
-      const double step = fabs(rn - rprev);
-      const double reach = (rn >= rprev) ? EST_DMAX * rn : EST_DMAX / (1 + EST_DMAX) * rn;
-      const bool fits = (double)iters * step <= EST_FIT * reach;
-      if (!fits && iters < EST_KMAX && m_est >= EST_MIN_GAIN) {
-        n_before = 1;
-      } else {
-        built = true;
-      }
-      if (built && m_est >= EST_MIN_GAIN && 100 - iters >= EST_MIN_GAIN) {
-        const double g = fmin(EST_DMAX, fmax(EST_MULT * step / rn, 1e-3));
-        double lo, hi;
-        if (rn >= rprev) {
-          lo = rn * (1 - EST_BACK * g);
-          hi = rn * (1 + g);
-        } else {
-          lo = rn / (1 + g);
-          hi = rn * (1 + EST_BACK * g);
-        }
-        mid = sqrt(lo * hi);
-        half = (hi - mid) / (hi + mid);
-        if (half > 0 && lo > 0 && hi < 1e300) {
+      int n_new = EN;
+      bool by_pred = false;
+      if (estmaf_interval(iters, lhs, thr, rn, rprev, r_pred, built, n_before, mid, half, n_new, by_pred)) {
+        {
+          nn = __builtin_amdgcn_readfirstlane(n_new);
+          tab = est_tab(nn);
+          pred = by_pred;
+          if (pred && tix == 0) est_count(cnt, EST_PRED_N6 + ((nn - 6) >> 1), blockIdx.x);
           if constexpr (PARK) {
-            const double tnl = half * kChebC[lane < EN ? lane : 0];
+            const double tnl = half * kChebC[tab + (lane < nn ? lane : 0)];
             const double r_nodes = mid * (1 + tnl) * rcp_nr2(1 - tnl);
 #pragma unroll 1
-            for (int nd = 0; nd < EN; ++nd) {
+            for (int nd = 0; nd < nn; ++nd) {
               double pn, pd;
               lane_sums(lane_value(r_nodes, nd), pn, pd);
               nodebuf[nd][lane] = double2{pn, pd};
@@ -364,7 +428,7 @@
             __syncthreads();
             const int j = lane & 15, q4 = lane >> 4;
             double an = 0, ad = 0;
-            if (j < EN) {
+            if (j < nn) {
 #pragma unroll
               for (int l = 0; l < 16; ++l) {
                 const double2 t2 = nodebuf[j][q4 * 16 + l];
@@ -380,18 +444,18 @@
             my_gd = ad;
             check = true;
           } else {
-            const double tnl = half * kChebC[lane < EN ? lane : 0];
+            const double tnl = half * kChebC[tab + (lane < nn ? lane : 0)];
             const double r_nodes = mid * (1 + tnl) * rcp_nr2(1 - tnl);
             double an = 0, ad = 0;
             if constexpr (W > 1) {
 #pragma unroll 1
-              for (int nd = 0; nd < EN; ++nd) {
+              for (int nd = 0; nd < nn; ++nd) {
                 double pn, pd;
                 lane_sums(lane_value(r_nodes, nd), pn, pd);
                 park[nd * BLOCK + (int)tix] = double2{pn, pd};
               }
               __syncthreads();
-              for (int nd = wv; nd < EN; nd += W) {
+              for (int nd = wv; nd < nn; nd += W) {
                 double sn = 0, sd = 0;
 #pragma unroll
                 for (int w = 0; w < W; ++w) {
@@ -404,14 +468,14 @@
                 if (lane == 0) xnode[nd][0] = double2{tn, td};
               }
               __syncthreads();
-              if (lane < EN) {
+              if (lane < nn) {
                 an = xnode[lane][0].x;
                 ad = xnode[lane][0].y;
               }
               __syncthreads();
             } else {
 #pragma unroll 1
-              for (int nd = 0; nd < EN; ++nd) {
+              for (int nd = 0; nd < nn; ++nd) {
                 double pn, pd;
                 lane_sums(lane_value(r_nodes, nd), pn, pd);
                 const double v = wave_sum_pair(pn, pd);
@@ -436,6 +500,8 @@
     freq_out[site] = freq;
     redo[site] = ok ? 0 : 1;
     status[site] = EST_DONE;
+    rend[site] = ok ? num / (den - num) : __builtin_nan("");
+    state[4 * state_stride + site] = (double)iters;
   }
 }
 
@@ -457,6 +523,7 @@
               uint64_t S_own, uint64_t I_tot, uint64_t I_blk, uint64_t tile_T,
               double* __restrict__ freq_out, uint8_t* __restrict__ redo,
               uint8_t* __restrict__ status, double* __restrict__ state, uint64_t state_stride,
+              double* __restrict__ rend, int predict,
               int n_exact, int allow_build, uint64_t blk0, uint32_t* __restrict__ cnt) {
   ESTMAF_SHARED(NI, BLOCK);
   uint64_t site;
@@ -474,8 +541,8 @@
   }
   extern __shared__ double2 park_mem[];
   estmaf_site<NI, BLOCK, TILE>(gl, marg_blocks, S_own, I_tot, I_blk, freq_out, redo, status, state,
-                               state_stride, 1, n_exact, allow_build, site, tile_col, cnt, xch, nodebuf,
-                               xnode, park_mem);
+                               state_stride, rend, predict, 1, n_exact, allow_build, site, tile_col, cnt,
+                               xch, nodebuf, xnode, park_mem);
 }
 
 template <int NI, int BLOCK, bool TILE>
@@ -484,8 +551,9 @@
                      uint64_t S_own, uint64_t I_tot, uint64_t I_blk, uint64_t tile_T,
                      double* __restrict__ freq_out, uint8_t* __restrict__ redo,
                      uint8_t* __restrict__ status, double* __restrict__ state,
-                     uint64_t state_stride, int n_exact, int allow_build, uint64_t row0,
-                     uint64_t row1, uint32_t* __restrict__ cnt, int cnt_slot) {
+                     uint64_t state_stride, double* __restrict__ rend, int n_exact,
+                     int allow_build, uint64_t row0, uint64_t row1, uint32_t* __restrict__ cnt,
+                     int cnt_slot) {
   ESTMAF_SHARED(NI, BLOCK);
   extern __shared__ double2 park_mem[];
   const int lane = threadIdx.x & 63;
@@ -501,8 +569,8 @@
       mask &= mask - 1;
       const double* tile_col = TILE ? estmaf_tile_col(marg_blocks, site, tile_T, I_tot) : nullptr;
       estmaf_site<NI, BLOCK, TILE>(gl, marg_blocks, S_own, I_tot, I_blk, freq_out, redo, status,
-                                   state, state_stride, 0, n_exact, allow_build, site, tile_col, cnt,
-                                   xch, nodebuf, xnode, park_mem);
+                                   state, state_stride, rend, 0, 0, n_exact, allow_build, site,
+                                   tile_col, cnt, xch, nodebuf, xnode, park_mem);
       if constexpr (BLOCK > 64) __syncthreads();
     }
   }
@@ -520,12 +588,15 @@
 __device__ __forceinline__ void estmaf_rows_sites(
     const GlView& gl, const double* __restrict__ marg_blocks, uint64_t S_own, uint64_t I_tot,
     uint64_t I_blk, double* __restrict__ freq_out, uint8_t* __restrict__ redo,
-    uint8_t* __restrict__ status, double* __restrict__ state, uint64_t state_stride, int fresh,
+    uint8_t* __restrict__ status, double* __restrict__ state, uint64_t state_stride,
+    double* __restrict__ rend, int predict, int fresh,
     int n_exact, int allow_build, uint64_t site, const double* __restrict__ tile_col, bool done,
     uint32_t* __restrict__ cnt) {
   static_assert(EN <= 16, "a row's lanes hold the interval's node sums");
   const int lane = threadIdx.x, j = lane & 15;
   const uint64_t cell_s = site * I_tot;
+  double r_pred = __builtin_nan("");
+  if (fresh && predict && !done) r_pred = rend[site];
 
   double sA[NI], sb[NI], sC[NI], u0[NI], nC[NI], fc[NI];
   double tF_acc = 0;
@@ -581,7 +652,8 @@
   }
   bool built = !allow_build;
   int n_before = n_exact;
-  bool check = false;
+  bool check = false, pred = false;
+  int nn = EN;
   double mid = 1, half = 0.5, my_gn = 0, my_gd = 0, rprev = 0;
   auto lane_sums = [&](double r, double& pn, double& pd) {
     pn = 0;
@@ -622,14 +694,17 @@
     const double sn = row_sum(pn), sd = row_sum(pd);
     bool interp_ok = false;
     if (__builtin_amdgcn_ballot_w64(check && !done) != 0) {
-      const int nj = j < EN ? j : 0;
+      const int nj = est_tab(nn) + (j < nn ? j : 0);
       const double t = (r - mid) / (r + mid) - half * kChebC[nj];
-      const double q = (j < EN) ? kChebW[nj] / t : 0.0;
+      const double q = (j < nn) ? kChebW[nj] / t : 0.0;
       const double Sq = row_sum(q);
       const double bn = row_sum(q * my_gn) / Sq, bd = row_sum(q * my_gd) / Sq;
       if (check && !done) {
         interp_ok = fabs(bn - sn) <= EST_TOL * fabs(sn) && fabs(bd - sd) <= EST_TOL * fabs(sd);
-        if (!interp_ok && j == 0) atomicAdd(cnt + EST_CNT_CHECK_FAILED, 1u);
+        if (!interp_ok && j == 0) {
+          atomicAdd(cnt + EST_CNT_CHECK_FAILED, 1u);
+          if (pred) est_count(cnt, EST_PRED_FAILED, site);
+        }
       }
       check = false;
     }
@@ -649,10 +724,12 @@
           freq_out[site] = freq;
           redo[site] = ok ? 0 : 1;
           status[site] = EST_DONE;
+          rend[site] = ok ? num / (den - num) : __builtin_nan("");
+          state[4 * state_stride + site] = (double)iters;
         }
         done = true;
       } else if (interp_ok) {
-        if (j < EN) {
+        if (j < nn) {
           state[(EST_SCALARS + j) * state_stride + site] = my_gn;
           state[(EST_SCALARS + EN + j) * state_stride + site] = my_gd;
         }
@@ -665,43 +742,26 @@
           state[5 * state_stride + site] = mid;
           state[6 * state_stride + site] = half;
           state[7 * state_stride + site] = tF_sum;
+          state[EST_NODES * state_stride + site] = pred ? -(double)nn : (double)nn;
           status[site] = EST_INTERP;
         }
         done = true;
-      } else if (!built && --n_before <= 0) {
-        const double m_est = (double)iters * (sqrt(lhs / thr) - 1.0);
+      } else if (!built) {
         const double rn = pnum * rcp_nr2(pden - pnum);
-        const double step = fabs(rn - rprev);
-        const double reach = (rn >= rprev) ? EST_DMAX * rn : EST_DMAX / (1 + EST_DMAX) * rn;
-        const bool fits = (double)iters * step <= EST_FIT * reach;
-        if (!fits && iters < EST_KMAX && m_est >= EST_MIN_GAIN) {
-          n_before = 1;
-        } else {
-          built = true;
+        if (estmaf_interval(iters, lhs, thr, rn, rprev, r_pred, built, n_before, mid, half, nn, pred)) {
+          want_build = true;
+          if (pred && j == 0) est_count(cnt, EST_PRED_N6 + ((nn - 6) >> 1), site);
         }
-        if (built && m_est >= EST_MIN_GAIN && 100 - iters >= EST_MIN_GAIN) {
-          const double g = fmin(EST_DMAX, fmax(EST_MULT * step / rn, 1e-3));
-          double lo, hi;
-          if (rn >= rprev) {
-            lo = rn * (1 - EST_BACK * g);
-            hi = rn * (1 + g);
-          } else {
-            lo = rn / (1 + g);
-            hi = rn * (1 + EST_BACK * g);
-          }
-          const double a = sqrt(lo * hi), h = (hi - a) / (hi + a);
-          if (h > 0 && lo > 0 && hi < 1e300) {
-            mid = a;
-            half = h;
-            want_build = true;
-          }
-        }
       }
     }
     if (__builtin_amdgcn_ballot_w64(want_build) != 0) {
+      const int nb = want_build ? nn : 0, tab = est_tab(nn);
+      const int n01 = max(__builtin_amdgcn_readlane(nb, 0), __builtin_amdgcn_readlane(nb, 16));
+      const int n23 = max(__builtin_amdgcn_readlane(nb, 32), __builtin_amdgcn_readlane(nb, 48));
+      const int n_max = max(n01, n23);
 #pragma unroll 1
-      for (int nd = 0; nd < EN; ++nd) {
-        const double tn = half * kChebC[nd];
+      for (int nd = 0; nd < n_max; ++nd) {
+        const double tn = half * kChebC[tab + (nd < nn ? nd : 0)];
         double qn, qd;
         lane_sums(mid * (1 + tn) * rcp_nr2(1 - tn), qn, qd);
         const double gn = row_sum(qn), gd = row_sum(qd);
@@ -721,7 +781,8 @@
 k_fast_estmaf_rows(const GlView gl, const double* __restrict__ marg_blocks, uint64_t S_own,
                    uint64_t I_tot, uint64_t I_blk, uint64_t tile_T, double* __restrict__ freq_out,
                    uint8_t* __restrict__ redo, uint8_t* __restrict__ status,
-                   double* __restrict__ state, uint64_t state_stride, int n_exact,
+                   double* __restrict__ state, uint64_t state_stride,
+                   double* __restrict__ rend, int predict, int n_exact,
                    int allow_build, uint32_t* __restrict__ cnt) {
   const int lane = threadIdx.x, row = lane >> 4;
   uint64_t site;
@@ -743,7 +804,8 @@
   }
   if (__builtin_amdgcn_ballot_w64(!done) == 0) return;
   estmaf_rows_sites<NI, TILE>(gl, marg_blocks, S_own, I_tot, I_blk, freq_out, redo, status, state,
-                              state_stride, 1, n_exact, allow_build, site, tile_col, done, cnt);
+                              state_stride, rend, predict, 1, n_exact, allow_build, site, tile_col, done,
+                              cnt);
 }
 
 template <int NI, bool TILE>
@@ -752,8 +814,8 @@
                           uint64_t I_tot, uint64_t I_blk, uint64_t tile_T,
                           double* __restrict__ freq_out, uint8_t* __restrict__ redo,
                           uint8_t* __restrict__ status, double* __restrict__ state,
-                          uint64_t state_stride, int n_exact, int allow_build,
-                          uint32_t* __restrict__ cnt, int cnt_slot) {
+                          uint64_t state_stride, double* __restrict__ rend, int n_exact,
+                          int allow_build, uint32_t* __restrict__ cnt, int cnt_slot) {
   const int lane = threadIdx.x, row = lane >> 4;
   for (uint64_t base = (uint64_t)blockIdx.x * 64; base < S_own; base += (uint64_t)gridDim.x * 64) {
     const uint64_t s = base + lane;
@@ -776,41 +838,35 @@
       const double* tile_col =
           TILE ? (done ? marg_blocks : estmaf_tile_col(marg_blocks, site, tile_T, I_tot)) : nullptr;
       estmaf_rows_sites<NI, TILE>(gl, marg_blocks, S_own, I_tot, I_blk, freq_out, redo, status,
-                                  state, state_stride, 0, n_exact, allow_build, site, tile_col, done,
-                                  cnt);
-    }
-  }
-}
-
-__global__ void __launch_bounds__(256)
-k_fast_estmaf_interp(uint64_t S_own, double* __restrict__ freq_out, uint8_t* __restrict__ redo,
-                     uint8_t* __restrict__ status, double* __restrict__ state,
-                     uint64_t state_stride, uint64_t tile_T, uint64_t row0, uint64_t row1) {
-  const uint64_t site = (uint64_t)blockIdx.x * blockDim.x + threadIdx.x;
-  if (site >= S_own || !in_tile_rows(site, tile_T, row0, row1) || status[site] != EST_INTERP)
-    return;
-  double num = state[0 * state_stride + site], den = state[1 * state_stride + site];
-  double pnum = state[2 * state_stride + site], pden = state[3 * state_stride + site];
-  int iters = (int)state[4 * state_stride + site];
-  const double mid = state[5 * state_stride + site], half = state[6 * state_stride + site];
-  const double tF_sum = state[7 * state_stride + site];
-  double gn[EN], gd[EN];
-#pragma unroll
-  for (int j = 0; j < EN; ++j) {
+                                  state, state_stride, rend, 0, 0, n_exact, allow_build, site,
+                                  tile_col, done, cnt);
+    }
+  }
+}
+
+template <int N>
+__device__ __forceinline__ uint8_t estmaf_interp_passes(const double* __restrict__ state,
+                                                        uint64_t state_stride, uint64_t site,
+                                                        double mid, double half, double tF_sum,
+                                                        double& num, double& den, double& pnum,
+                                                        double& pden, int& iters) {
+  double gn[N], gd[N];
+#pragma unroll
+  for (int j = 0; j < N; ++j) {
     gn[j] = state[(EST_SCALARS + j) * state_stride + site];
     gd[j] = state[(EST_SCALARS + EN + j) * state_stride + site];
   }
-  double cn[EN], cd[EN];
-#pragma unroll
-  for (int k = 0; k < EN; ++k) cn[k] = cd[k] = 0;
-#pragma unroll
-  for (int j = 0; j < EN; ++j) {
-    const double x = kChebC[j], fn = gn[j] * (2.0 / EN), fd = gd[j] * (2.0 / EN);
+  double cn[N], cd[N];
+#pragma unroll
+  for (int k = 0; k < N; ++k) cn[k] = cd[k] = 0;
+#pragma unroll
+  for (int j = 0; j < N; ++j) {
+    const double x = kChebC[est_tab(N) + j], fn = gn[j] * (2.0 / N), fd = gd[j] * (2.0 / N);
     double t0 = 1.0, t1 = x;
     cn[0] += fn;
     cd[0] += fd;
 #pragma unroll
-    for (int k = 1; k < EN; ++k) {
+    for (int k = 1; k < N; ++k) {
       cn[k] = fma(fn, t1, cn[k]);
       cd[k] = fma(fd, t1, cd[k]);
       const double t2 = fma(2 * x, t1, -t0);
@@ -819,7 +875,6 @@
     }
   }
   const double inv_half = 1.0 / half;
-  uint8_t st = EST_EXACT;
   for (;;) {
     const double r = pnum * rcp_nr2(pden - pnum);
     const double tt = (r - mid) * rcp_nr2(r + mid);
@@ -827,7 +882,7 @@
     const double x2 = 2 * (tt * inv_half);
     double bn1 = 0, bn2 = 0, bd1 = 0, bd2 = 0;
 #pragma unroll
-    for (int k = EN - 1; k >= 1; --k) {
+    for (int k = N - 1; k >= 1; --k) {
       const double bn0 = fma(x2, bn1, cn[k] - bn2), bd0 = fma(x2, bd1, cd[k] - bd2);
       bn2 = bn1;
       bn1 = bn0;
@@ -844,22 +899,53 @@
     const bool again = (lhs > thr) && (iters++ < 100);
     pnum = num;
     pden = den;
-    if (!again) {
-      st = EST_DONE;
+    if (!again) return EST_DONE;
+  }
+  return EST_EXACT;
+}
+
+__global__ void __launch_bounds__(256)
+k_fast_estmaf_interp(uint64_t S_own, double* __restrict__ freq_out, uint8_t* __restrict__ redo,
+                     uint8_t* __restrict__ status, double* __restrict__ state,
+                     uint64_t state_stride, double* __restrict__ rend, uint64_t tile_T,
+                     uint64_t row0, uint64_t row1, uint32_t* __restrict__ cnt) {
+  const uint64_t site = (uint64_t)blockIdx.x * blockDim.x + threadIdx.x;
+  if (site >= S_own || !in_tile_rows(site, tile_T, row0, row1) || status[site] != EST_INTERP)
+    return;
+  double num = state[0 * state_stride + site], den = state[1 * state_stride + site];
+  double pnum = state[2 * state_stride + site], pden = state[3 * state_stride + site];
+  int iters = (int)state[4 * state_stride + site];
+  const double mid = state[5 * state_stride + site], half = state[6 * state_stride + site];
+  const double tF_sum = state[7 * state_stride + site];
+  const int nodes = (int)state[EST_NODES * state_stride + site];
+  uint8_t st;
+  switch (nodes < 0 ? -nodes : nodes) {
+    case 6:
+      st = estmaf_interp_passes<6>(state, state_stride, site, mid, half, tF_sum, num, den, pnum, pden, iters);
       break;
-    }
+    case 8:
+      st = estmaf_interp_passes<8>(state, state_stride, site, mid, half, tF_sum, num, den, pnum, pden, iters);
+      break;
+    case 10:
+      st = estmaf_interp_passes<10>(state, state_stride, site, mid, half, tF_sum, num, den, pnum, pden, iters);
+      break;
+    default:
+      st = estmaf_interp_passes<EN>(state, state_stride, site, mid, half, tF_sum, num, den, pnum, pden, iters);
   }
   if (st == EST_DONE) {
     const double freq = num / den;
     const bool ok = freq >= 0 && freq < 1;
     freq_out[site] = freq;
     redo[site] = ok ? 0 : 1;
+    rend[site] = ok ? num / (den - num) : __builtin_nan("");
+    state[4 * state_stride + site] = (double)iters;
   } else {
     state[0 * state_stride + site] = num;
     state[1 * state_stride + site] = den;
     state[2 * state_stride + site] = pnum;
     state[3 * state_stride + site] = pden;
     state[4 * state_stride + site] = (double)iters;
+    if (nodes < 0) est_count(cnt, EST_PRED_LEFT, site);
   }
   status[site] = st;
 }
@@ -938,7 +1024,8 @@
 __global__ void __launch_bounds__(256)
 k_fast_estmaf_called_passes(uint64_t S_own, double* __restrict__ freq_out, uint8_t* __restrict__ redo,
                             uint8_t* __restrict__ status, const double* __restrict__ state,
-                            uint64_t state_stride, uint64_t tile_T, uint64_t row0, uint64_t row1) {
+                            uint64_t state_stride, double* __restrict__ rend, uint64_t tile_T,
+                            uint64_t row0, uint64_t row1) {
   const uint64_t site = (uint64_t)blockIdx.x * blockDim.x + threadIdx.x;
   if (site >= S_own || !in_tile_rows(site, tile_T, row0, row1)) return;
   status[site] = EST_DONE;
@@ -965,11 +1052,13 @@
   const bool ok = freq >= 0 && freq < 1;
   freq_out[site] = freq;
   redo[site] = ok ? 0 : 1;
+  rend[site] = ok ? num / (den - num) : __builtin_nan("");
 }
 
 __device__ void estmaf_stream_site(const GlView& gl, const double* __restrict__ marg_blocks,
                                    uint64_t S_own, uint64_t I_tot, uint64_t I_blk, uint64_t tile_T,
-                                   double* __restrict__ freq_out, uint64_t site, int lane) {
+                                   double* __restrict__ freq_out, double* __restrict__ rend,
+                                   bool careful, uint64_t site, int lane) {
   const uint64_t cell_s = site * I_tot;
   const uint64_t tj = tile_T ? site / tile_T : 0;
   const double* trow =
@@ -1013,21 +1102,26 @@
     freq = num / den;
     again = (fabs(prev - freq) > kEPS) && (iters++ < 100);
   } while (again);
-  if (lane == 0) freq_out[site] = freq;
+  if (lane == 0) {
+    freq_out[site] = freq;
+    rend[site] = careful ? __builtin_nan("") : freq / (1 - freq);
+  }
 }
 
 __global__ void __launch_bounds__(256)
 k_fast_estmaf_stream(const GlView gl, const double* __restrict__ marg_blocks,
                      uint64_t S_own, uint64_t I_tot, uint64_t I_blk, uint64_t tile_T,
                      double* __restrict__ freq_out, const uint8_t* __restrict__ redo,
-                     uint64_t row0, uint64_t row1, uint32_t* __restrict__ cnt) {
+                     double* __restrict__ rend, uint64_t row0, uint64_t row1,
+                     uint32_t* __restrict__ cnt) {
   const int lane = threadIdx.x & 63;
   const uint64_t wave = (uint64_t)blockIdx.x * (blockDim.x >> 6) + (threadIdx.x >> 6);
   const uint64_t n_waves = (uint64_t)gridDim.x * (blockDim.x >> 6);
   if (!redo) {
     for (uint64_t site = wave; site < S_own; site += n_waves)
       if (in_tile_rows(site, tile_T, row0, row1))
-        estmaf_stream_site(gl, marg_blocks, S_own, I_tot, I_blk, tile_T, freq_out, site, lane);
+        estmaf_stream_site(gl, marg_blocks, S_own, I_tot, I_blk, tile_T, freq_out, rend, false, site,
+                           lane);
     return;
   }
   for (uint64_t base = wave * 64; base < S_own; base += n_waves * 64) {
@@ -1038,7 +1132,8 @@
     while (mask) {
       const int b = __builtin_ctzll(mask);
       mask &= mask - 1;
-      estmaf_stream_site(gl, marg_blocks, S_own, I_tot, I_blk, tile_T, freq_out, base + b, lane);
+      estmaf_stream_site(gl, marg_blocks, S_own, I_tot, I_blk, tile_T, freq_out, rend, true, base + b,
+                         lane);
     }
   }
 }
@@ -1059,10 +1154,12 @@
   return tile_major && I_tot > 128 && I_tot <= 8192;
 }
 
+void fast_estmaf_forget(FastState& fs) { fs.est_rend_sites = 0; }
+
 bool fast_estmaf_reserve(FastState& fs, uint64_t S_own) {
   if (!fs.est_counts) {
-    if (hipMalloc((void**)&fs.est_counts, EST_COUNTS * sizeof(uint32_t)) != hipSuccess) return false;
-    if (hipMemset(fs.est_counts, 0, EST_COUNTS * sizeof(uint32_t)) != hipSuccess) return false;
+    if (hipMalloc((void**)&fs.est_counts, EST_COUNT_WORDS * sizeof(uint32_t)) != hipSuccess) return false;
+    if (hipMemset(fs.est_counts, 0, EST_COUNT_WORDS * sizeof(uint32_t)) != hipSuccess) return false;
     if (hipDeviceSynchronize() != hipSuccess) return false;
   }
   if (S_own <= fs.redo_cap) return true;
@@ -1119,6 +1216,15 @@
   const uint64_t stream_wgs = stream_all ? (S_own + 3) / 4 : (S_own + 255) / 256;
   const dim3 grid((unsigned)(stream_wgs < 65536 ? stream_wgs : 65536)), block(256);
   if (!fast_estmaf_reserve(fs, S_own)) return false;
+  if (!fs.est_rend || fs.est_rend_cap < S_own) {
+    capi::set_error("est_maf: no buffer for the sites' carried odds");
+    return false;
+  }
+  if (fs.est_rend_sites != S_own) {
+    if (hipMemsetAsync(fs.est_rend, 0xff, S_own * sizeof(double), st) != hipSuccess) return false;
+    fs.est_rend_sites = S_own;
+  }
+  const int predict = fs.sw.estmaf_no_predict ? 0 : 1;
   if (fast_estmaf_called(fs, d_gl_sites)) {
     if (tile_major)
       hipLaunchKernelGGL((k_fast_estmaf_called_sums<true>), dim3((unsigned)nblk), dim3(64), 0, st,
@@ -1129,10 +1235,11 @@
                          d_gl_sites, d_marg_blocks, S_own, I_tot, I_blk, tile_T, fs.redo, fs.est_state,
                          fs.redo_cap, (uint64_t)0);
     hipLaunchKernelGGL(k_fast_estmaf_called_passes, dim3((unsigned)((S_own + 255) / 256)), dim3(256), 0,
-                       st, S_own, d_freq_out, fs.redo, fs.est_status, fs.est_state, fs.redo_cap, tile_T,
-                       row0, row1);
+                       st, S_own, d_freq_out, fs.redo, fs.est_status, fs.est_state, fs.redo_cap,
+                       fs.est_rend, tile_T, row0, row1);
     hipLaunchKernelGGL(k_fast_estmaf_stream, grid, block, 0, st, d_gl_sites, d_marg_blocks, S_own,
-                       I_tot, I_blk, tile_T, d_freq_out, fs.redo, row0, row1, fs.est_counts);
+                       I_tot, I_blk, tile_T, d_freq_out, fs.redo, fs.est_rend, row0, row1,
+                       fs.est_counts);
     return hipGetLastError() == hipSuccess;
   }
   bool interp = true;
@@ -1148,14 +1255,15 @@
       hipLaunchKernelGGL((k_fast_estmaf<N, B, false>), dim3((unsigned)S_own), dim3(B),          \
                          ESTMAF_DYN(B), st, d_gl_sites, d_marg_blocks, S_own, I_tot, I_blk,     \
                          (uint64_t)0, d_freq_out, fs.redo, fs.est_status, fs.est_state,         \
-                         fs.redo_cap, n_exact, allow_build, (uint64_t)0, fs.est_counts);        \
+                         fs.redo_cap, fs.est_rend, predict, n_exact, allow_build, (uint64_t)0,  \
+                         fs.est_counts);                                                        \
     } else {                                                                                    \
       if (!ESTMAF_TELL((k_fast_estmaf_resume<N, B, false>), B)) return false;                   \
       hipLaunchKernelGGL((k_fast_estmaf_resume<N, B, false>), dim3(scan_wgs), dim3(B),          \
                          ESTMAF_DYN(B), st, d_gl_sites, d_marg_blocks, S_own, I_tot, I_blk,     \
                          (uint64_t)0, d_freq_out, fs.redo, fs.est_status, fs.est_state,         \
-                         fs.redo_cap, n_exact, allow_build, row0, row1, fs.est_counts,          \
-                         cnt_slot);                                                             \
+                         fs.redo_cap, fs.est_rend, n_exact, allow_build, row0, row1,            \
+                         fs.est_counts, cnt_slot);                                              \
     }                                                                                           \
   } while (0)
 #define LAUNCH_TILE(N, B)                                                                       \
@@ -1165,13 +1273,14 @@
       hipLaunchKernelGGL((k_fast_estmaf<N, B, true>), dim3((unsigned)nblk), dim3(B),            \
                          ESTMAF_DYN(B), st, d_gl_sites, d_marg_blocks, S_own, I_tot, I_blk,     \
                          tile_T, d_freq_out, fs.redo, fs.est_status, fs.est_state, fs.redo_cap, \
-                         n_exact, allow_build, blk0, fs.est_counts);                            \
+                         fs.est_rend, predict, n_exact, allow_build, blk0, fs.est_counts);      \
     } else {                                                                                    \
       if (!ESTMAF_TELL((k_fast_estmaf_resume<N, B, true>), B)) return false;                    \
       hipLaunchKernelGGL((k_fast_estmaf_resume<N, B, true>), dim3(scan_wgs), dim3(B),           \
                          ESTMAF_DYN(B), st, d_gl_sites, d_marg_blocks, S_own, I_tot, I_blk,     \
                          tile_T, d_freq_out, fs.redo, fs.est_status, fs.est_state, fs.redo_cap, \
-                         n_exact, allow_build, row0, row1, fs.est_counts, cnt_slot);            \
+                         fs.est_rend, n_exact, allow_build, row0, row1, fs.est_counts,          \
+                         cnt_slot);                                                             \
     }                                                                                           \
   } while (0)
 #define LAUNCH_ROWS(N, TL)                                                                      \
@@ -1180,13 +1289,13 @@
       hipLaunchKernelGGL((k_fast_estmaf_rows<N, TL>),                                            \
                          dim3((unsigned)((TL) ? fs.Spad / 4 : (S_own + 3) / 4)), dim3(64), 0,   \
                          st, d_gl_sites, d_marg_blocks, S_own, I_tot, I_blk, tile_T, d_freq_out, \
-                         fs.redo, fs.est_status, fs.est_state, fs.redo_cap, n_exact,            \
-                         allow_build, fs.est_counts);                                           \
+                         fs.redo, fs.est_status, fs.est_state, fs.redo_cap, fs.est_rend,        \
+                         predict, n_exact, allow_build, fs.est_counts);                         \
     else                                                                                        \
       hipLaunchKernelGGL((k_fast_estmaf_rows_resume<N, TL>), dim3(scan_wgs), dim3(64), 0, st,    \
                          d_gl_sites, d_marg_blocks, S_own, I_tot, I_blk, tile_T, d_freq_out,    \
-                         fs.redo, fs.est_status, fs.est_state, fs.redo_cap, n_exact,            \
-                         allow_build, fs.est_counts, cnt_slot);                                 \
+                         fs.redo, fs.est_status, fs.est_state, fs.redo_cap, fs.est_rend,        \
+                         n_exact, allow_build, fs.est_counts, cnt_slot);                        \
   } while (0)
   const bool rows = I_tot <= 128 && !fs.sw.estmaf_no_rows;
   auto launch = [&](int fresh, int n_exact, int allow_build, int cnt_slot = 0) -> bool {
@@ -1244,16 +1353,18 @@
     const dim3 igrid((unsigned)((S_own + 255) / 256));
     if (!launch(1, EST_K0, 1)) return false;
     hipLaunchKernelGGL(k_fast_estmaf_interp, igrid, dim3(256), 0, st, S_own, d_freq_out, fs.redo,
-                       fs.est_status, fs.est_state, fs.redo_cap, tile_T, row0, row1);
+                       fs.est_status, fs.est_state, fs.redo_cap, fs.est_rend, tile_T, row0, row1,
+                       fs.est_counts);
     for (int again = 0; again < 2; ++again) {
       if (!launch(0, 1, 1, again ? EST_CNT_RESUMED_AGAIN : EST_CNT_RESUMED)) return false;
       hipLaunchKernelGGL(k_fast_estmaf_interp, igrid, dim3(256), 0, st, S_own, d_freq_out, fs.redo,
-                         fs.est_status, fs.est_state, fs.redo_cap, tile_T, row0, row1);
+                         fs.est_status, fs.est_state, fs.redo_cap, fs.est_rend, tile_T, row0, row1,
+                         fs.est_counts);
     }
     if (!launch(0, 0, 0, EST_CNT_EXACT_TAIL)) return false;
   }
   hipLaunchKernelGGL(k_fast_estmaf_stream, grid, block, 0, st, d_gl_sites, d_marg_blocks, S_own,
-                     I_tot, I_blk, tile_T, d_freq_out, redo, row0, row1, fs.est_counts);
+                     I_tot, I_blk, tile_T, d_freq_out, redo, fs.est_rend, row0, row1, fs.est_counts);
 #undef LAUNCH_NI
 #undef ESTMAF_DYN
 #undef ESTMAF_TELL
diff --git a/ngsf-hmm_amd/csrc/nghmm_capi.hip b/ngsf-hmm_amd/csrc/nghmm_capi.hip
--- a/ngsf-hmm_amd/csrc/nghmm_capi.hip
+++ b/ngsf-hmm_amd/csrc/nghmm_capi.hip
@@ -554,6 +554,7 @@
   int rc;
   if ((rc = use_device(h))) return rc;
   if (indF || alpha) dbfgs_invalidate(h->fast);
+  fast_estmaf_forget(h->fast);
   if (indF) {
     std::memcpy(h->h_indF.data(), indF, h->I * sizeof(double));
     HIP_TRY(hipMemcpyAsync(h->d_indF, indF, h->I * sizeof(double), hipMemcpyHostToDevice, h->stream));
@@ -716,6 +717,7 @@
     hipStream_t bs = bg_stream ? bg_stream : h->stream;
     if ((q = bg_open(h, SLOT_ESTMAF, bs))) return q;
     if (!tile_major && (q = ensure_marg(h))) return q;
+    if ((q = estmaf_carry(h, h->S))) return q;
     if (!fast_estmaf(h->fast, bs, fast_gl_lin(h->fast),
                      tile_major ? h->fast.post : h->d_marg, h->S, h->I, h->I, h->d_freq,
                      tile_major, part, bg_parts))
@@ -1176,6 +1178,17 @@
 
 }
 
+int capi::estmaf_carry(nghmm_t* h, uint64_t n_sites) {
+  int rc;
+  if (n_sites > h->d_est_rend.cap) {
+    if ((rc = h->d_est_rend.reserve(n_sites))) return rc;
+    fast_estmaf_forget(h->fast);
+  }
+  h->fast.est_rend = h->d_est_rend;
+  h->fast.est_rend_cap = h->d_est_rend.cap;
+  return NGHMM_OK;
+}
+
 int capi::estmaf_and_refresh(nghmm_t* h, bool shard, const double* d_marg_blocks, uint64_t S_own,
                               uint64_t I_tot, uint64_t I_blk, double* d_freq_out) {
   int rc;
@@ -1194,6 +1207,7 @@
         d_marg_blocks = h->d_marg;
       }
     }
+    if ((rc = estmaf_carry(h, S_own))) return rc;
     if (!fast_estmaf(h->fast, h->stream, lin, d_marg_blocks, S_own, I_tot, I_blk, d_freq_out,
                      tile_major))
       return NGHMM_ERR_HIP;
@@ -1239,9 +1253,11 @@
   tic(h);
   if (exact) {
     launch_estmaf_exact(h->stream, own_gl(h), h->d_marg, n_est, h->I, h->d_freq_new, nullptr, 0);
-  } else if (!fast_estmaf(h->fast, h->stream, fast_gl_lin(h->fast), h->d_marg, n_est, h->I, h->I,
-                          h->d_freq_new, false)) {
-    return NGHMM_ERR_HIP;
+  } else {
+    if ((rc = estmaf_carry(h, n_est))) return rc;
+    if (!fast_estmaf(h->fast, h->stream, fast_gl_lin(h->fast), h->d_marg, n_est, h->I, h->I,
+                     h->d_freq_new, false))
+      return NGHMM_ERR_HIP;
   }
   if (!launch_freq_ld_chain(h->stream, exact, exact ? own_gl(h) : fast_gl_lin(h->fast), h->d_marg,
                             h->d_freq, h->d_freq_new, h->d_hap, h->S, h->I, freq_est, h->d_flags))
@@ -1533,4 +1549,60 @@
   return NGHMM_OK;
 }
 
-}
+int nghmm_debug_estmaf_predict_counts(nghmm_t* h, uint64_t out[7], int reset) {
+  g_last_error.clear();
+  if (!h || !out) return NGHMM_ERR_ARG;
+  for (int k = 0; k < 7; ++k) out[k] = 0;
+  if (!h->fast.est_counts) return NGHMM_OK;
+  int rc;
+  if ((rc = use_device(h))) return rc;
+  static_assert(EST_STRIPED == 6, "out[0] the total, then one entry per striped count");
+  std::vector<uint32_t> v(EST_COUNT_WORDS - EST_STRIPED_BASE);
+  HIP_TRY(sync_stream(h));
+  HIP_TRY(hipMemcpy(v.data(), h->fast.est_counts + EST_STRIPED_BASE, v.size() * sizeof(uint32_t),
+                    hipMemcpyDeviceToHost));
+  for (int slot = 0; slot < EST_STRIPED; ++slot)
+    for (int k = 0; k < 64; ++k) out[1 + slot] += v[(size_t)(slot * 64 + k) * 32];
+  out[0] = out[1] + out[2] + out[3] + out[4];
+  if (reset) {
+    HIP_TRY(hipMemset(h->fast.est_counts + EST_STRIPED_BASE, 0, v.size() * sizeof(uint32_t)));
+    HIP_TRY(hipDeviceSynchronize());
+  }
+  return NGHMM_OK;
+}
+
+int nghmm_debug_estmaf_state(nghmm_t* h, int field, double* out, uint64_t n) {
+  g_last_error.clear();
+  if (!h || !out || h->mode != NGHMM_MODE_FAST || (field != 4 && field != 5 && field != 6 && field != 8))
+    return NGHMM_ERR_ARG;
+  if (!h->fast.est_state || n > h->fast.redo_cap) {
+    set_error("nghmm_debug_estmaf_state: no frequency step over %llu sites yet", (unsigned long long)n);
+    return NGHMM_ERR_ARG;
+  }
+  int rc;
+  if ((rc = use_device(h))) return rc;
+  HIP_TRY(sync_stream(h));
+  HIP_TRY(hipMemcpy(out, h->fast.est_state + (size_t)field * h->fast.redo_cap, n * sizeof(double),
+                    hipMemcpyDeviceToHost));
+  return NGHMM_OK;
+}
+
+int nghmm_debug_estmaf_r_end(nghmm_t* h, double* r_end, uint64_t n, int set) {
+  g_last_error.clear();
+  if (!h || !r_end || h->mode != NGHMM_MODE_FAST) return NGHMM_ERR_ARG;
+  int rc;
+  if ((rc = use_device(h))) return rc;
+  HIP_TRY(sync_stream(h));
+  if (set) {
+    if ((rc = estmaf_carry(h, n))) return rc;
+    HIP_TRY(hipMemcpy(h->d_est_rend, r_end, n * sizeof(double), hipMemcpyHostToDevice));
+    h->fast.est_rend_sites = n;
+    return NGHMM_OK;
+  }
+  const uint64_t have = h->d_est_rend ? h->fast.est_rend_sites : 0;
+  for (uint64_t s = 0; s < n; ++s) r_end[s] = std::nan("");
+  if (have) HIP_TRY(hipMemcpy(r_end, h->d_est_rend, (n < have ? n : have) * sizeof(double), hipMemcpyDeviceToHost));
+  return NGHMM_OK;
+}
+
+}
diff --git a/ngsf-hmm_amd/hmm.py b/ngsf-hmm_amd/hmm.py
--- a/ngsf-hmm_amd/hmm.py
+++ b/ngsf-hmm_amd/hmm.py
@@ -113,6 +113,9 @@
         "nghmm_set_switch": (i32, [vp, C.c_char_p, C.c_long]),
         "nghmm_debug_mode_counts": (i32, [vp, C.POINTER(ModeCount), u32, C.POINTER(u32), i32]),
         "nghmm_debug_estmaf_counts": (i32, [vp, C.POINTER(u64), i32]),
+        "nghmm_debug_estmaf_predict_counts": (i32, [vp, C.POINTER(u64), i32]),
+        "nghmm_debug_estmaf_r_end": (i32, [vp, dp, u64, i32]),
+        "nghmm_debug_estmaf_state": (i32, [vp, i32, dp, u64]),
         "nghmm_alloc_host": (vp, [u64]),
         "nghmm_free_host": (None, [vp]),
         "nghmm_site_shard_bytes": (u64, [vp]),
@@ -166,6 +169,7 @@
     "nghmm_fast_layout", "nghmm_stream",
     "nghmm_synchronize",
     "nghmm_kernel_ms", "nghmm_set_switch", "nghmm_debug_mode_counts", "nghmm_debug_estmaf_counts",
+    "nghmm_debug_estmaf_predict_counts", "nghmm_debug_estmaf_r_end", "nghmm_debug_estmaf_state",
     "nghmm_site_shard_bytes", "nghmm_site_shard_setup", "nghmm_viterbi_shard_forward",
     "nghmm_viterbi_shard_back", "nghmm_chain_setup", "nghmm_chain_iter_em", "nghmm_chain_mstep_freq",
     "nghmm_chain_viterbi", "nghmm_alloc_host", "nghmm_free_host",
@@ -738,6 +742,27 @@
         return {"check_failed": int(v[0]), "second_interval": int(v[1]), "third_interval": int(v[2]),
                 "log_space": int(v[3]), "exact_tail": int(v[4])}
 
+    def estmaf_predict_counts(self, reset=False):
+        v = (C.c_uint64 * 7)()
+        self._check(self.lib.nghmm_debug_estmaf_predict_counts(self._h, v, int(reset)))
+        return {"predicted": int(v[0]), "nodes": {6: int(v[1]), 8: int(v[2]), 10: int(v[3]), 12: int(v[4])},
+                "check_failed": int(v[5]), "handed_back": int(v[6])}
+
+    def estmaf_r_end(self, n=None):
+        out = np.empty(self.n_sites if n is None else int(n))
+        self._check(self.lib.nghmm_debug_estmaf_r_end(self._h, _dp(out), out.size, 0))
+        return out
+
+    def estmaf_state(self, field, n=None):
+        out = np.empty(self.n_sites if n is None else int(n))
+        k = {"passes": 4, "mid": 5, "half": 6, "nodes": 8}[field]
+        self._check(self.lib.nghmm_debug_estmaf_state(self._h, k, _dp(out), out.size))
+        return out
+
+    def set_estmaf_r_end(self, r_end):
+        a = np.ascontiguousarray(r_end, dtype=np.float64)
+        self._check(self.lib.nghmm_debug_estmaf_r_end(self._h, _dp(a), a.size, 1))
+
 
 class Group:
 
```

New measurement: 42.42 billion. About the same (-0.9%).
